# torchmd/torchmd-net

Measured on AMD Instinct MI355X. Metric: molecules/sec (64-atom molecules) TensorNet E+F, higher is better.
Workload: dtype f32; 1 GPU; BASELINE configs[1]: TensorNet F=128 L=2 K=32 rc=5.0, S-mol64 256 molecules x 64 atoms per GPU, energies + forces, random-init weights (seed 0); atoms_per_gpu=16384, pairs_per_gpu=193709, directed_edges_per_gpu=403802, parallelism=molecule-sharded x1, RCCL all-reduce of energies, rank_step=eager: tmdnet_build_graph (pair-count read-back) + tmdnet_energy_forces

## Files before the change

torchmd-net_amd/csrc/tn_api.hip:

```cpp
#include <hip/hip_runtime.h>

#include <algorithm>
#include <cmath>
#include <cstdio>
#include <cstdlib>
#include <cstring>
#include <map>
#include <unordered_map>
#include <string>
#include <vector>

#include "tn_chain.h"
#include "tn_heads.h"
#include "tn_model.h"
#include "tn_tlin9.h"
#include "tn_small.h"
#include "tn_interp.h"
#include "tn_virial.h"

using namespace tn;

static const char* kCatNames[CAT_COUNT] = {"graph", "gemm_edge", "gemm_node", "message", "pair_bwd", "embed_scatter", "elementwise", "edge_table"};

int fail(tmdnet_model* m, int code, const std::string& msg) {
// ... 52 lines not shown
  a.bias[0] = bias;
  a.C = C;
  a.C2 = C2;
  a.rowscale = rs;
  a.rowscale2 = rs2;
  a.lda = lda;
  a.ldw = K;
  a.ldc = ldc;
  a.M = M;
  a.N = N;
  a.K = K;
  a.groups = 1;
  a.m_dev = g_mdev;
  a.m_add = g_madd;
  const double bytes = 4.0 * (2.0 * M * K + (double)N * K + 2.0 * M * N);
  char lab[64];
  std::snprintf(lab, sizeof(lab), "gemm_dual<%d> %dx%dx%d", kind, M, N, K);
  ProfScope ps_(s, CAT_GEMM_EDGE, 4.0 * M * N * K, bytes, lab);
  launch_gemm_dual(a, kind, s);
}

namespace {

void build_specs(tmdnet_model* m) {
  const int F = m->hp.hidden_channels, K = m->hp.num_rbf, L = m->hp.num_layers, Z = m->hp.max_z, H = m->hp.head_hidden;
  auto& s = m->specs;
  const std::string R = "representation_model.", T = R + "tensor_embedding.";
  s.push_back({R + "distance_expansion.means", K, 1});
  s.push_back({R + "distance_expansion.betas", K, 1});
  for (int k = 1; k <= 3; ++k) {
    s.push_back({T + "distance_proj" + std::to_string(k) + ".weight", F, K});
    s.push_back({T + "distance_proj" + std::to_string(k) + ".bias", F, 1});
  }
  s.push_back({T + "emb.weight", Z, F});
  s.push_back({T + "emb2.weight", F, 2 * F});
  s.push_back({T + "emb2.bias", F, 1});
  for (int k = 0; k < 3; ++k) s.push_back({T + "linears_tensor." + std::to_string(k) + ".weight", F, F});
  s.push_back({T + "linears_scalar.0.weight", 2 * F, F});
  s.push_back({T + "linears_scalar.0.bias", 2 * F, 1});
  s.push_back({T + "linears_scalar.1.weight", 3 * F, 2 * F});
  s.push_back({T + "linears_scalar.1.bias", 3 * F, 1});
  s.push_back({T + "init_norm.weight", F, 1});
  s.push_back({T + "init_norm.bias", F, 1});
  for (int l = 0; l < L; ++l) {
    const std::string Lp = R + "layers." + std::to_string(l) + ".";
    const int64_t K1 = m->tn2 ? K + 2 * m->tn2->hp.q_dim : K;
    const int64_t dims[3][2] = {{F, K1}, {2 * F, F}, {3 * F, 2 * F}};
    for (int k = 0; k < 3; ++k) {
      s.push_back({Lp + "linears_scalar." + std::to_string(k) + ".weight", dims[k][0], dims[k][1]});
      s.push_back({Lp + "linears_scalar." + std::to_string(k) + ".bias", dims[k][0], 1});
    }
    for (int k = 0; k < 6; ++k) s.push_back({Lp + "linears_tensor." + std::to_string(k) + ".weight", F, F});
  }
  s.push_back({R + "linear.weight", F, 3 * F});
  s.push_back({R + "linear.bias", F, 1});
  s.push_back({R + "out_norm.weight", 3 * F, 1});
  s.push_back({R + "out_norm.bias", 3 * F, 1});
  const std::string O = "output_model.output_network.layers.";
  s.push_back({O + "0.weight", H, F});
  s.push_back({O + "0.bias", H, 1});
  s.push_back({O + "2.weight", 1, H});
  s.push_back({O + "2.bias", 1, 1});
  s.push_back({"mean", 1, 1});
  s.push_back({"std", 1, 1});
  if (m->hp.has_atomref) s.push_back({"atomref", Z, 1});
  if (m->tn2) {
    const int qd = m->tn2->hp.q_dim;
    for (int l = 0; l <= L; ++l) {
      const std::string Cp = R + (l == 0 ? std::string("charge_predict_0.") : "charge_predicts." + std::to_string(l - 1) + ".");
      s.push_back({Cp + "q_norm.weight", 3 * F, 1});
      s.push_back({Cp + "q_norm.bias", 3 * F, 1});
      s.push_back({Cp + "q_mlp.layers.0.weight", F, 3 * F});
      s.push_back({Cp + "q_mlp.layers.0.bias", F, 1});
      s.push_back({Cp + "q_mlp.layers.2.weight", F, F});
      s.push_back({Cp + "q_mlp.layers.2.bias", F, 1});
      s.push_back({Cp + "q_mlp.layers.4.weight", 2 * qd, F});
      s.push_back({Cp + "q_mlp.layers.4.bias", 2 * qd, 1});
    }
    s.push_back({"output_model.qweights", (int64_t)(L + 1) * qd, 1});
  }
}

}

void tensor_linear(hipStream_t s, const float* A, const float* const W3[3], float* C, int N, int F, int flags, float* pre,
                   const float* gates) {
  GemmArgs a{};
  a.A = A;
  a.C = C;
  a.pre = pre;
  a.aux = gates;
  a.lda = a.ldc = a.ldpre = 9 * (int64_t)F;
  a.ldaux = 3 * (int64_t)F;
  a.ldw = F;
  for (int c = 0; c < 9; ++c) {
    const int t = c == 0 ? 0 : (c < 4 ? 1 : 2);
    a.W[c] = W3[t];
    if (g_cur) {
      auto it = g_cur->sb_of.find(W3[t]);
      if (it != g_cur->sb_of.end()) a.Wsbg[c] = it->second;
    }
    a.bias[c] = nullptr;
    a.a_off[c] = a.c_off[c] = a.pre_off[c] = c * F;
    a.aux_off[c] = t * F;
  }
  a.M = N;
  a.N = F;
  a.K = F;
  a.groups = 9;
  a.flags = flags;
  const double bytes = 4.0 * (9.0 * N * F * (2 + (pre ? 1 : 0)) + (gates ? 3.0 * N * F : 0.0) + 3.0 * F * F);
  char lab[64];
  std::snprintf(lab, sizeof(lab), "tensor_linear 9x%dx%dx%d", N, F, F);
  ProfScope ps_(s, CAT_GEMM_NODE, 2.0 * 9 * N * (double)F * F, bytes, lab);
  launch_gemm(a, s);
}


void remember_graph(tmdnet_model* m, const void* graph_ws, int64_t n_atoms, int64_t n_mol) {
  if (m->graph_rec.size() >= 64 && !m->graph_rec.count(graph_ws)) m->graph_rec.clear();
  m->graph_rec[graph_ws] = tmdnet_model::GraphRecord{m->graph_is_cell, m->graph_cell_multi, m->graph_has_z, m->last_nt, m->lastE, m->graph_no_ghost_pairs, n_atoms, n_mol, m->graph_closed_tiles};
}
void recall_graph(tmdnet_model* m, const void* graph_ws) {
  auto it = m->graph_rec.find(graph_ws);
  if (it == m->graph_rec.end()) return;
  m->graph_is_cell = it->second.is_cell;
  m->graph_cell_multi = it->second.cell_multi;
  m->graph_has_z = it->second.has_z;
  m->last_nt = it->second.nt;
  m->lastE = it->second.lastE;
  m->graph_no_ghost_pairs = it->second.no_ghost_pairs;
  m->graph_closed_tiles = it->second.closed_tiles;
}

bool tlin9_images(const float* const W3[3]) {
  if (!g_cur) return false;
  for (int t = 0; t < 3; ++t)
    if (g_cur->fm_of.find(W3[t]) == g_cur->fm_of.end()) return false;
  return true;
}
void tlin9(hipStream_t s, int pro, int epi, const float* const W3[3], Tl9Args a, double tensors, const char* what) {
  for (int t = 0; t < 3; ++t) a.Wfm[t] = g_cur->fm_of.at(W3[t]);
  char lab[64];
  std::snprintf(lab, sizeof(lab), "tlin9 %s 9x%dx%dx%d", what, a.N, a.F, a.F);
  ProfScope ps_(s, CAT_GEMM_NODE, 2.0 * 9 * a.N * (double)a.F * a.F, 4.0 * (tensors * 9.0 * a.N * a.F + 3.0 * a.F * a.F), lab);
  launch_tlin9(a, pro, epi, s);
}

Graph carve_graph(void* ws, int64_t N, int64_t B, int64_t ecap, size_t* total) {
  Carver c(ws);
  Graph g{};
  const int64_t pcap = ecap / 2 + 1;
  g.small_mols = N <= 96 * (B > 0 ? B : 1) ? 1 : 0;
  g.counts = c.take<int>(8);
  g.mstart = c.take<int>(B);
  g.mend = c.take<int>(B);
  g.nlow = c.take<int>(N);
  g.ntot = c.take<int>(N);
  g.rowptr = c.take<int>(N + 1);
  g.pairptr = c.take<int>(N + 1);
  g.col = c.take<int>(ecap);
  g.epair = c.take<int>(ecap);
  g.esign = c.take<float>(ecap);
  g.pair_i = c.take<int>(pcap);
  g.pair_j = c.take<int>(pcap);
  g.pd = c.take<float>(pcap + 1);
  g.pdelta = c.take<float>(pcap * 3);
  g.prhat = c.take<float>(pcap * 3);
  g.ecap = ecap;
  g.pcap = pcap;
  g.perm = c.take<int>(N);
  g.iota = c.take<int>(N);
  g.cell_key = c.take<int>(N);
  g.cell_key_sorted = c.take<int>(N);
  g.cell_start = c.take<int>(8 * N + 2);
  g.pos_s = c.take<float>(3 * N);
  g.z_s = c.take<int64_t>(N);
  g.boxd = c.take<float>(12);
  g.cgrid = c.take<int>(4);
  g.bat_s = c.take<int>(N);
  g.bat_c = c.take<int64_t>(N);
  g.z_c = c.take<int64_t>(N);
  g.tix = c.take<int>(N);
  g.tz = c.take<int>(64);
  g.sort_tmp_bytes = cell_sort_temp_bytes(N);
  g.sort_tmp = c.take<char>((int64_t)g.sort_tmp_bytes);
  if (total) *total = c.off;
  return g;
}

namespace {
bool cell_applicable(const tmdnet_model* m, int64_t n_atoms, int64_t n_mol, int box_mode) {
  const int* n = m->cell_n;
  if (n_mol < 1 || box_mode == 2 || n_atoms < 1) return false;
  if (n[0] < 0) return true;
  if (n[0] < 1 || n[1] < 1 || n[2] < 1) return false;
  return (int64_t)n[0] * n[1] * n[2] <= 8 * n_atoms;
}
void set_cell(Graph& g, const tmdnet_model* m, bool on, int64_t n_mol = 1) {
  g.use_cell = on ? (n_mol > 1 ? 2 : 1) : 0;
  const bool explicit_grid = m->cell_n[0] > 0;
  g.ncx = explicit_grid ? m->cell_n[0] : 0;
  g.ncy = explicit_grid ? m->cell_n[1] : 0;
  g.ncz = explicit_grid ? m->cell_n[2] : 0;
}

}
int rb_ntp(const tmdnet_model* m, int64_t n_atoms, int64_t n_pairs) {
  if (!m->rb_fwd || m->et || m->train || n_pairs < 0 || n_atoms < m->rb_min_atoms) return 0;
  return embed_rb_ntp(m->last_nt);
}
namespace {

FwdBuffers carve_fwd(void* ws, const tmdnet_hparams& hp, int64_t N, int64_t B, int64_t P, bool bwd, size_t* total, int ntp = 0,
                     int lean = 0) {
  Carver c(ws);
  FwdBuffers b{};
  const int64_t F = hp.hidden_channels, K = hp.num_rbf, L = hp.num_layers, Z = hp.max_z, H = hp.head_hidden;
  const int64_t P1 = P + 1, N9 = N * 9 * F;
  b.phi = c.take<float>((lean & 1) ? 0 : P1 * K);
  b.dphi = c.take<float>((lean & 1) ? 0 : P1 * K);
  b.C = c.take<float>(P1);
  b.dC = c.take<float>(P1);
  b.Q = c.take<float>((lean & 2) ? 0 : P1 * 3 * F);
  b.u0 = c.take<float>(N9);
  b.s0n = c.take<float>(N * F);
  b.ln0 = c.take<float>(N * F);
  b.xh0 = c.take<float>(N * F);
  b.rstd0 = c.take<float>(N);
  b.a1 = c.take<float>(N * 2 * F);
  b.h1 = c.take<float>(N * 2 * F);
  b.a2 = c.take<float>(N * 3 * F);
  b.gates = c.take<float>(N * 3 * F);
  b.UX = c.take<float>(N9);
  for (int l = 0; l <= L; ++l) b.X.push_back(c.take<float>(N9));
  for (int l = 0; l < L; ++l) {
    b.w.push_back(c.take<float>((lean & 4) ? 0 : P1 * 3 * F));
    b.dw.push_back(c.take<float>(bwd && !(lean & 4) ? P1 * 3 * F : 0));
    b.Pn.push_back(c.take<float>(N9));
    b.Mi.push_back(c.take<float>(N9));
    b.D.push_back(c.take<float>(N9));
  }
  b.he1 = c.take<float>((lean & 1) ? 0 : P1 * F);
  b.he2 = c.take<float>((lean & 1) ? 0 : P1 * 2 * F);
  b.te1 = c.take<float>(bwd && !(lean & 1) ? P1 * F : 0);
  b.te2 = c.take<float>(bwd && !(lean & 1) ? P1 * 2 * F : 0);
  b.dQ = c.take<float>(bwd && !(lean & 2) ? P1 * 3 * F : 0);
  b.Xh = c.take<float>(N9);
  b.Ch = c.take<float>(N9);
  b.feat = c.take<float>(N * 3 * F);
  b.lnr = c.take<float>(N * 3 * F);
  b.xhr = c.take<float>(N * 3 * F);
  b.rstdr = c.take<float>(N);
  b.al = c.take<float>(N * F);
  b.x = c.take<float>(N * F);
  b.ao = c.take<float>(N * H);
  b.ea = c.take<float>(N);
  b.kap = c.take<float>(N);
  b.skeys_s = c.take<unsigned>(P1);
  b.svals_s = c.take<int>(P1);
  b.shist = c.take<int>(65536 + 2);
  if (bwd) {
    b.g_ao = c.take<float>(N * H);
    b.g_al = c.take<float>(N * F);
    b.g_ln = c.take<float>(N * 3 * F);
    b.g_feat = c.take<float>(N * 3 * F);
    b.G = c.take<float>(N9);
    b.gD = c.take<float>(N9);
    b.gCh = c.take<float>(N9);
    b.gMi = c.take<float>(N9);
    b.gPn = c.take<float>(N9);
    b.gXl = c.take<float>(N9);
    b.gd = c.take<float>(P1);
    b.gd_slots = c.take<float>(2 * P1 * (int64_t)L * ((F + 31) / 32));
    b.gUX = c.take<float>(N9);
    b.g_a2 = c.take<float>(N * 3 * F);
    b.g_a1 = c.take<float>(N * 2 * F);
    b.g_ln0 = c.take<float>(N * F);
    b.g_s0n = c.take<float>(N * F);
    b.g_u0l = c.take<float>(N9);
    b.gA = c.take<float>(N * 10 * F);
    b.g_rhat = c.take<float>(P1 * 3);
    b.g_delta = c.take<float>(P1 * 3);
  }
  b.mom = c.take<float>(ntp ? embed_rb_moment_elems(N, ntp, (int)K) : 0);
  b.gmom = c.take<float>(ntp && bwd ? embed_rb_gmoment_elems(N, ntp, (int)K) : 0);
  b.ps = c.take<float>(ntp ? P1 * 8 : 0);
  if (total) *total = c.off;
  return b;
}

}

void free_radial_tables(EdgeTables& t) {
  for (float* p : t.tab)
    if (p) (void)hipFree(p);
  t = EdgeTables{};
}

int build_radial_tables(tmdnet_model* m, EdgeTables& out, const std::vector<TableSpec>& specs, const float* means, const float* betas,
                        int K, double lo, double up) {
  free_radial_tables(out);
  const char* env = getenv("TMDNET_EDGE_TABLE");
  if (env && atoi(env) == 0) return TMDNET_OK;
  int Rmax = 0, Nmax = 0;
  for (const TableSpec& sp : specs) {
    const int R = sp.chain.back().N;
    if (R % 4 || R / 4 > 256) return TMDNET_OK;
    Rmax = std::max(Rmax, R);
    for (const TableLayer& l : sp.chain) Nmax = std::max(Nmax, l.N);
  }
  if (specs.empty()) return TMDNET_OK;
  const double tol_value = 5e-7, tol_slope = 2e-6;
  hipStream_t s = nullptr;
  const int ntab = (int)specs.size();
  for (int T = 8192; T <= 65536; T *= 2) {
    const int M = T + 2;
    std::vector<void*> tmp;
    bool alloc_ok = true;
    auto D_ = [&](int64_t n) {
      double* p = nullptr;
      alloc_ok = (hipMalloc(reinterpret_cast<void**>(&p), (size_t)n * sizeof(double)) == hipSuccess) && alloc_ok;
      tmp.push_back(p);
      return p;
    };
    auto F_ = [&](int64_t n) {
      float* p = nullptr;
      alloc_ok = (hipMalloc(reinterpret_cast<void**>(&p), (size_t)n * sizeof(float)) == hipSuccess) && alloc_ok;
      tmp.push_back(p);
      return p;
    };
    double *dist = D_(M), *phi = D_((int64_t)M * K), *dphi = D_((int64_t)M * K), *C = D_(M), *dC = D_(M);
    double* hv_[2] = {D_((int64_t)M * Nmax), D_((int64_t)M * Nmax)};
    double* hs_[2] = {D_((int64_t)M * Nmax), D_((int64_t)M * Nmax)};
    float *ip = F_((int64_t)T * Rmax), *dip = F_((int64_t)T * Rmax);
    std::vector<float*> tab(ntab, nullptr);
    for (int t = 0; t < ntab; ++t)
      alloc_ok = (hipMalloc(reinterpret_cast<void**>(&tab[t]), (size_t)M * 3 * specs[t].chain.back().N * sizeof(float)) == hipSuccess) &&
                 alloc_ok;
// ... 628 lines not shown
    }
    Packer pk;
    std::map<std::string, size_t> off;
    pack_tensornet_params(m, tags, pk, off);
    if (pk.buf.size() != m->packed_elems) return fail(m, TMDNET_ERR_STATE, "device-side parameter update: layout mismatch");
    std::vector<int32_t> tid(pk.buf.size(), -1), ofs(pk.buf.size(), 0);
    for (size_t i = 0; i < pk.buf.size(); ++i) {
      uint32_t tag;
      std::memcpy(&tag, &pk.buf[i], 4);
      if (!tag || (int64_t)tag > base[ns]) continue;
      const int64_t g = (int64_t)tag - 1;
      const size_t t = (size_t)(std::upper_bound(base.begin(), base.end(), g) - base.begin()) - 1;
      tid[i] = (int32_t)t;
      ofs[i] = (int32_t)(g - base[t]);
    }
    HIP_TRY(m, hipMalloc(reinterpret_cast<void**>(&m->upd_tid), tid.size() * sizeof(int32_t)));
    HIP_TRY(m, hipMalloc(reinterpret_cast<void**>(&m->upd_ofs), ofs.size() * sizeof(int32_t)));
    HIP_TRY(m, hipMalloc(reinterpret_cast<void**>(&m->upd_ptrs), ns * sizeof(float*)));
    HIP_TRY(m, hipMemcpy(m->upd_tid, tid.data(), tid.size() * sizeof(int32_t), hipMemcpyHostToDevice));
    HIP_TRY(m, hipMemcpy(m->upd_ofs, ofs.data(), ofs.size() * sizeof(int32_t), hipMemcpyHostToDevice));
    m->upd_ready = true;
  }
  std::vector<const float*> ptrs(ns, nullptr);
  for (int32_t c = 0; c < count; ++c) {
    size_t i = 0;
    for (; i < ns; ++i)
      if (m->specs[i].name == names[c]) break;
    if (i == ns) return fail(m, TMDNET_ERR_INVALID, std::string("unknown parameter: ") + names[c]);
    if (m->specs[i].name == "mean" || m->specs[i].name == "std")
      return fail(m, TMDNET_ERR_INVALID, "mean / std are kernel arguments read on the host: update them through tmdnet_set_param");
    ptrs[i] = dev_ptrs[c];
  }
  HIP_TRY(m, hipMemcpyAsync(m->upd_ptrs, ptrs.data(), ns * sizeof(float*), hipMemcpyHostToDevice, s));
  hipLaunchKernelGGL(k_param_gather, dim3((unsigned)((m->packed_elems + 255) / 256)), dim3(256), 0, s, m->dev, m->upd_tid, m->upd_ofs,
                     m->upd_ptrs, (int64_t)m->packed_elems);
  for (const auto& j : m->image_jobs) {
    if (j.fm) launch_split_weight_fm(m->dev + j.src_off, j.n, j.k, m->dev_sb + j.dst_off, s);
    else launch_split_weight_tiles(m->dev + j.src_off, j.n, j.k, m->dev_sb + j.dst_off, s);
  }
  const int F = m->hp.hidden_channels;
  launch_ztables(m->P.emb, m->P.emb2_waT, m->P.emb2_wbT, m->P.emb2_b, m->hp.max_z, F, const_cast<float*>(m->P.Utab),
                 const_cast<float*>(m->P.Vtab), s);
  m->tabs_pending = true;
  if (m->rb_fwd)
    launch_embed_rb_images(m->P.Wdp, m->P.bdp, F, m->hp.num_rbf, m->rb_img, m->rb_img + embed_rb_image_elems(F, m->hp.num_rbf, false), s);
  HIP_TRY(m, hipGetLastError());
  return TMDNET_OK;
}

int tmdnet_set_option(tmdnet_model* m, const char* name, double value) {
  if (!m || !name) return TMDNET_ERR_INVALID;
  const std::string n(name);
  if (n == "edge_table_min_pairs") {
    m->tab_min_pairs = value < 0 ? 0 : (int64_t)value;
    return TMDNET_OK;
  }
  if (n == "embed_rb_min_atoms") {
    m->rb_min_atoms = value < 0 ? 0 : (int64_t)value;
    return TMDNET_OK;
  }
  if (n == "chain_min_atoms") {
    m->chain_min_atoms = value < 0 ? 0 : (value > 9e18 ? INT64_MAX : (int64_t)value);
    return TMDNET_OK;
  }
  if (n == "chain_mask") {
    m->chain_mask = (int)value & 7;
    return TMDNET_OK;
  }
  if (n == "pair_rows_bf16") {
    if (!m->et) return fail(m, TMDNET_ERR_INVALID, "pair_rows_bf16 applies to the Equivariant Transformer handle only");
    m->pair_bf16 = value == 2.0 ? 2 : (value != 0.0 ? 1 : 0);
    return TMDNET_OK;
  }
  if (n == "recompute_pair_rows") {
    if (m->et || m->tn2) return fail(m, TMDNET_ERR_INVALID, "recompute_pair_rows applies to the TensorNet handle only");
    m->recompute_rows = value != 0.0;
    return TMDNET_OK;
  }
  if (n == "fold_node_adjoint") {
    if (m->et || m->tn2) return fail(m, TMDNET_ERR_INVALID, "fold_node_adjoint applies to the TensorNet handle only");
    m->fold_node_adjoint = value != 0.0;
    return TMDNET_OK;
  }
  return fail(m, TMDNET_ERR_INVALID, "unknown option: " + n);
}

int tmdnet_get_info(const tmdnet_model* m, const char* name, double* value) {
  if (!m || !name || !value) return TMDNET_ERR_INVALID;
  const std::string n(name);
  if (m->tabs_pending && n.rfind("edge_table_", 0) == 0 && n != "edge_table_min_pairs")
    if (const int rc = ensure_radial_tables(const_cast<tmdnet_model*>(m), nullptr)) return rc;
  if (n == "edge_table_T") *value = m->tabs.ok ? m->tabs.T : 0;
  else if (n == "edge_table_err_value") *value = m->tabs.err_value;
  else if (n == "edge_table_err_slope") *value = m->tabs.err_slope;
  else if (n == "edge_table_min_pairs") *value = (double)m->tab_min_pairs;
  else if (n == "pair_rows_bf16") *value = (double)m->pair_bf16;
  else if (n == "embed_rb_min_atoms") *value = (double)m->rb_min_atoms;
  else if (n == "chain_min_atoms") *value = (double)m->chain_min_atoms;
  else if (n == "chain_mask") *value = (double)m->chain_mask;
  else if (n == "chain_last") *value = (double)m->chain_last;
  else if (n == "recompute_pair_rows") *value = m->recompute_rows ? 1.0 : 0.0;
  else if (n == "embed_rb") *value = m->rb_fwd ? 1.0 : 0.0;
  else if (n == "species_last_build") *value = (double)m->last_nt;
  else if (n == "halo_active_first") *value = (double)m->halo_active[0];
  else if (n == "halo_active_rows") *value = (double)m->halo_active[1];
  else if (n == "message_route_last") *value = (double)m->msg_route_last[0];
  else if (n == "message_adjoint_route_last") *value = (double)m->msg_route_last[1];
  else if (n == "fold_node_adjoint") *value = m->fold_node_adjoint ? 1.0 : 0.0;
  else if (n == "message_adjoint_fold_last") *value = (double)m->msg_fold_last;
  else return TMDNET_ERR_INVALID;
  return TMDNET_OK;
}

int tmdnet_set_cell_grid(tmdnet_model* m, int32_t ncx, int32_t ncy, int32_t ncz) {
  if (!m) return TMDNET_ERR_INVALID;
  if (ncx < 0 || ncy < 0 || ncz < 0) ncx = ncy = ncz = -1;
  m->cell_n[0] = ncx;
  m->cell_n[1] = ncy;
  m->cell_n[2] = ncz;
  return TMDNET_OK;
}

int tmdnet_graph_workspace_bytes(const tmdnet_model* m, int64_t n_atoms, int64_t n_mol, size_t* bytes) {
  if (!m || !bytes || n_atoms < 0 || n_mol < 0) return TMDNET_ERR_INVALID;
  const int64_t ecap = (int64_t)m->hp.max_num_neighbors * n_atoms;
  carve_graph(nullptr, n_atoms, n_mol, ecap, bytes);
  return TMDNET_OK;
}

int tmdnet_build_graph(tmdnet_model* m, void* stream, void* graph_ws, size_t graph_ws_bytes, int64_t n_atoms, int64_t n_mol,
                       const float* pos, const int64_t* batch, const int64_t* z, const float* box, int32_t box_mode,
                       int64_t counts_host[8]) {
  if (!m || !graph_ws || !counts_host || n_atoms < 0 || n_mol < 0) return TMDNET_ERR_INVALID;
  if (n_atoms >= (int64_t)1 << 30) return fail(m, TMDNET_ERR_INVALID, "n_atoms too large for 32-bit indices");
  hipStream_t s = reinterpret_cast<hipStream_t>(stream);
  const int64_t ecap = (int64_t)m->hp.max_num_neighbors * n_atoms;
  size_t need = 0;
  Graph g = carve_graph(graph_ws, n_atoms, n_mol, ecap, &need);
  if (need > graph_ws_bytes) return fail(m, TMDNET_ERR_WORKSPACE, "graph workspace too small");
  if (box_mode != 0 && !box) return fail(m, TMDNET_ERR_INVALID, "box_mode != 0 needs a box");
  const bool cell = cell_applicable(m, n_atoms, n_mol, box_mode);
  set_cell(g, m, cell, n_mol);
  if (cell && m->halo_fn && m->atom_w && !m->et && !m->tn2) g.ghost_w = m->atom_w;
  m->graph_no_ghost_pairs = g.ghost_w != nullptr;
  m->graph_is_cell = cell;
  m->graph_cell_multi = cell && n_mol > 1;
  m->graph_has_z = z != nullptr;
  m->g_pos = pos;
  m->g_box = box;
  m->g_box_mode = box_mode;
  CurScope cur_(m);
  {
    ProfScope ps_(s, CAT_GRAPH, 0.0, (double)n_atoms * 20);
    if (cell) {
      launch_fill(reinterpret_cast<float*>(g.counts), 0.f, 8, s);
      launch_cell_phase1(g, pos, batch, box_mode == 1 ? box : nullptr, (int)n_atoms, m->hp.cutoff_lower, m->hp.cutoff_upper, true, s,
                         (int)n_mol);
      launch_scan_counts(g, (int)n_atoms, s);
    } else {
      launch_graph_build_phase1(g, pos, batch, box, box_mode, (int)n_atoms, (int)n_mol, m->hp.cutoff_lower, m->hp.cutoff_upper,
                                true, s);
    }
    if (z) launch_prepare_z(g, z, cell ? g.perm : nullptr, (int)n_atoms, m->hp.max_z, s);
    if (z && m->rb_fwd && n_atoms >= m->rb_min_atoms) launch_type_map(g, (int)n_atoms, m->hp.max_z, s);
  }
  int counts[8] = {0, 0, 0, 0, 0, 0, 0, 0};
  HIP_TRY(m, hipMemcpyAsync(counts, g.counts, sizeof(counts), hipMemcpyDeviceToHost, s));
  HIP_TRY(m, hipStreamSynchronize(s));
  for (int k = 0; k < 8; ++k) counts_host[k] = counts[k];
  m->last_nt = (z && m->rb_fwd && n_atoms >= m->rb_min_atoms) ? counts[6] : 0;
  m->lastE = counts[1];
  m->graph_closed_tiles = !cell && counts[3] == 0 && counts[5] == 0 && counts[7] == 0;
  remember_graph(m, graph_ws, n_atoms, n_mol);
  if (counts[5])
    return fail(m, TMDNET_ERR_INVALID, "batch index out of range: every entry must be in [0, " + std::to_string(n_mol) + ")");
  if (counts[4])
    return fail(m, TMDNET_ERR_INVALID, "atomic number out of range: every z must be in [0, max_z = " + std::to_string(m->hp.max_z) + ")");
  if (counts[2])
    return fail(m, TMDNET_ERR_OVERFLOW, "Found num_pairs > max_num_pairs, please increase max_num_pairs (found " +
                                            std::to_string(counts[1]) + " edges, capacity " + std::to_string(ecap) + ")");
  m->lastE = counts[1];
  {
    ProfScope ps_(s, CAT_GRAPH, 0.0, (double)counts[1] * 12 + (double)counts[0] * 40);
    if (cell) {
      launch_cell_phase2(g, (int)n_atoms, m->hp.cutoff_lower, m->hp.cutoff_upper, true, s);
      launch_nbr_link_wave(g, (int)n_atoms, s);
    } else {
      launch_graph_build_phase2(g, pos, batch, box, box_mode, (int)n_atoms, (int)n_mol, m->hp.cutoff_lower, m->hp.cutoff_upper, true,
                                s);
    }
  }
  HIP_TRY(m, hipGetLastError());
  return TMDNET_OK;
}

int tmdnet_build_graph_static(tmdnet_model* m, void* stream, void* graph_ws, size_t graph_ws_bytes, int64_t n_atoms, int64_t n_mol,
                              const float* pos, const int64_t* batch, const int64_t* z, const float* box, int32_t box_mode) {
  if (!m || !graph_ws || n_atoms < 0 || n_mol < 0) return TMDNET_ERR_INVALID;
  hipStream_t s = reinterpret_cast<hipStream_t>(stream);
  const int64_t ecap = (int64_t)m->hp.max_num_neighbors * n_atoms;
  size_t need = 0;
  Graph g = carve_graph(graph_ws, n_atoms, n_mol, ecap, &need);
  if (need > graph_ws_bytes) return fail(m, TMDNET_ERR_WORKSPACE, "graph workspace too small");
  if (box_mode != 0 && !box) return fail(m, TMDNET_ERR_INVALID, "box_mode != 0 needs a box");
  const bool cell = cell_applicable(m, n_atoms, n_mol, box_mode);
  set_cell(g, m, cell, n_mol);
  m->graph_no_ghost_pairs = false;
  m->graph_is_cell = cell;
  m->graph_cell_multi = cell && n_mol > 1;
  m->graph_has_z = z != nullptr;
  m->g_pos = pos;
  m->g_box = box;
  m->g_box_mode = box_mode;
  CurScope cur_(m);
  {
    ProfScope ps_(s, CAT_GRAPH, 0.0, (double)n_atoms * 20);
    if (cell) {
      launch_fill(reinterpret_cast<float*>(g.counts), 0.f, 8, s);
      launch_cell_phase1(g, pos, batch, box_mode == 1 ? box : nullptr, (int)n_atoms, m->hp.cutoff_lower, m->hp.cutoff_upper, true, s,
                         (int)n_mol);
      launch_scan_counts(g, (int)n_atoms, s);
      launch_cell_phase2(g, (int)n_atoms, m->hp.cutoff_lower, m->hp.cutoff_upper, true, s);
      launch_nbr_link_wave(g, (int)n_atoms, s);
    } else if (graph_small_ok((int)n_atoms)) {
      launch_graph_small(g, pos, batch, box, box_mode, (int)n_atoms, (int)n_mol, m->hp.cutoff_lower, m->hp.cutoff_upper, true, z,
                         m->hp.max_z, s);
    } else {
      launch_graph_build_phase1(g, pos, batch, box, box_mode, (int)n_atoms, (int)n_mol, m->hp.cutoff_lower, m->hp.cutoff_upper,
                                true, s);
      launch_graph_build_phase2(g, pos, batch, box, box_mode, (int)n_atoms, (int)n_mol, m->hp.cutoff_lower, m->hp.cutoff_upper, true,
                                s);
    }
    if (z && (cell || !graph_small_ok((int)n_atoms))) launch_prepare_z(g, z, cell ? g.perm : nullptr, (int)n_atoms, m->hp.max_z, s);
  }
  m->lastE = ecap;
  m->last_nt = 0;
  m->graph_closed_tiles = false;
  remember_graph(m, graph_ws, n_atoms, n_mol);
  HIP_TRY(m, hipGetLastError());
  return TMDNET_OK;
}

int tmdnet_graph_counts(tmdnet_model* m, void* stream, void* graph_ws, int64_t n_atoms, int64_t n_mol, int64_t counts_host[8]) {
  if (!m || !graph_ws || !counts_host) return TMDNET_ERR_INVALID;
  hipStream_t s = reinterpret_cast<hipStream_t>(stream);
  Graph g = carve_graph(graph_ws, n_atoms, n_mol, (int64_t)m->hp.max_num_neighbors * n_atoms, nullptr);
  int counts[8] = {0, 0, 0, 0, 0, 0, 0, 0};
  HIP_TRY(m, hipMemcpyAsync(counts, g.counts, sizeof(counts), hipMemcpyDeviceToHost, s));
  HIP_TRY(m, hipStreamSynchronize(s));
  for (int k = 0; k < 8; ++k) counts_host[k] = counts[k];
  if (counts[5]) return fail(m, TMDNET_ERR_INVALID, "batch index out of range: every entry must be in [0, " + std::to_string(n_mol) + ")");
  if (counts[4])
    return fail(m, TMDNET_ERR_INVALID, "atomic number out of range: every z must be in [0, max_z = " + std::to_string(m->hp.max_z) + ")");
  return counts[2] ? TMDNET_ERR_OVERFLOW : TMDNET_OK;
}

int tmdnet_set_atom_weights(tmdnet_model* m, const float* weights_dev) {
  if (!m) return TMDNET_ERR_INVALID;
  m->atom_w = weights_dev;
  return TMDNET_OK;
}

int tmdnet_set_halo_exchange(tmdnet_model* m, tmdnet_halo_exchange_fn fn, void* user) {
  if (!m) return TMDNET_ERR_INVALID;
  m->halo_fn = fn;
  m->halo_user = fn ? user : nullptr;
  if (fn && !m->halo_rng) HIP_TRY(m, hipMalloc(reinterpret_cast<void**>(&m->halo_rng), 4 * sizeof(int)));
  return TMDNET_OK;
}

int tmdnet_graph_cell_grid(tmdnet_model* m, void* stream, void* graph_ws, int64_t n_atoms, int64_t n_mol, int64_t grid_host[4]) {
  if (!m || !graph_ws || !grid_host) return TMDNET_ERR_INVALID;
  recall_graph(m, graph_ws);
  hipStream_t s = reinterpret_cast<hipStream_t>(stream);
  Graph g = carve_graph(graph_ws, n_atoms, n_mol, (int64_t)m->hp.max_num_neighbors * n_atoms, nullptr);
  int grid[4] = {0, 0, 0, 0};
  if (m->graph_is_cell) {
    HIP_TRY(m, hipMemcpyAsync(grid, g.cgrid, sizeof(grid), hipMemcpyDeviceToHost, s));
    HIP_TRY(m, hipStreamSynchronize(s));
  }
  for (int k = 0; k < 3; ++k) grid_host[k] = grid[k];
  grid_host[3] = m->graph_is_cell ? 1 : 0;
  return TMDNET_OK;
}

int tmdnet_forward_workspace_bytes(const tmdnet_model* m, int64_t n_atoms, int64_t n_mol, int64_t n_pairs, int64_t n_edges,
                                   int32_t want_forces, size_t* bytes) {
  if (!m || !bytes) return TMDNET_ERR_INVALID;
  (void)n_edges;
  if (n_pairs < 0) n_pairs = ((int64_t)m->hp.max_num_neighbors * n_atoms) / 2 + 1;
  if (m->et) return et_forward_workspace_bytes(m, n_atoms, n_mol, n_pairs, want_forces, bytes);
  if (m->tn2) return tn2_forward_workspace_bytes(m, n_atoms, n_mol, n_pairs, n_edges, want_forces, bytes);
  const bool rb_possible = m->rb_fwd && !m->et && !m->train && n_pairs >= 0 && n_atoms >= m->rb_min_atoms;
  carve_fwd(nullptr, m->hp, n_atoms, n_mol, n_pairs, want_forces != 0, bytes, rb_possible ? 8 : 0,
            m->recompute_rows ? (rb_possible && rb_ntp(m, n_atoms, n_pairs) > 0 ? 7 : 5) : 0);
  if (m->head_kind) {
    size_t hb = 0;
    carve_heads(nullptr, n_atoms, n_mol, &hb);
    *bytes = ((*bytes + 255) & ~size_t(255)) + hb;
  }
  return TMDNET_OK;
}

int tmdnet_energy_forces(tmdnet_model* m, void* stream, void* graph_ws, void* ws, size_t ws_bytes, int64_t n_atoms,
                         int64_t n_mol, int64_t n_pairs, const int64_t* z, const int64_t* batch, const float* q,
                         int32_t want_forces, float* energy, float* forces) {
  if (!m || !graph_ws || !ws || !energy) return TMDNET_ERR_INVALID;
  if (!m->finalized) return fail(m, TMDNET_ERR_STATE, "parameters not finalised");
  if (want_forces && !forces) return TMDNET_ERR_INVALID;
  recall_graph(m, graph_ws);
  hipStream_t s = reinterpret_cast<hipStream_t>(stream);
  const tmdnet_hparams& hp = m->hp;
  const int F = hp.hidden_channels, K = hp.num_rbf, L = hp.num_layers, Z = hp.max_z, H = hp.head_hidden;
  const int N = (int)n_atoms, B = (int)n_mol;
  const int64_t ecap = (int64_t)hp.max_num_neighbors * n_atoms;
  Graph g = carve_graph(graph_ws, n_atoms, n_mol, ecap, nullptr);
  if (n_pairs > g.pcap) return fail(m, TMDNET_ERR_INVALID, "n_pairs out of range");
  if (!m->train && (n_pairs >= 0 ? n_pairs : g.pcap) + 1 >= m->tab_min_pairs)
    if (const int rc_tab = ensure_radial_tables(m, s)) return rc_tab;
  if (m->graph_is_cell && m->graph_cell_multi) batch = g.bat_c;
  if (m->atom_w && (m->et || m->tn2 || m->train))
    return fail(m, TMDNET_ERR_INVALID, "atom weights (tmdnet_set_atom_weights) are implemented for TensorNet inference only");
  if (m->halo_fn && (m->et || m->tn2 || m->train || n_pairs < 0))
    return fail(m, TMDNET_ERR_INVALID, "the halo exchange (tmdnet_set_halo_exchange) is implemented for TensorNet inference with the "
                                       "exact pair count (tmdnet_build_graph, not the static mode)");
  if (m->et) {
    if (q) return fail(m, TMDNET_ERR_INVALID, "the Equivariant Transformer takes no total charge (reference torchmd_et.py:188-196)");
    CurScope cur_(m);
    if (m->graph_has_z) {
      z = g.z_c;
    } else if (m->graph_is_cell) {
      set_cell(g, m, true, n_mol);
      launch_permute_z(g, z, (int)n_atoms, s);
      z = g.z_s;
    }
    if (!z) return fail(m, TMDNET_ERR_INVALID, "z is required (here or in tmdnet_build_graph)");
    return et_energy_forces(m, s, g, ws, ws_bytes, n_atoms, n_mol, n_pairs, z, batch, want_forces, energy, forces);
  }
  if (m->tn2) {
    CurScope cur_(m);
    if (m->graph_has_z) {
      z = g.z_c;
    } else if (m->graph_is_cell) {
      set_cell(g, m, true, n_mol);
      launch_permute_z(g, z, (int)n_atoms, s);
      z = g.z_s;
    }
    if (!z) return fail(m, TMDNET_ERR_INVALID, "z is required (here or in tmdnet_build_graph)");
    if (m->graph_is_cell) set_cell(g, m, true, n_mol);
    return tn2_energy_forces(m, s, g, ws, ws_bytes, n_atoms, n_mol, n_pairs, z, batch, q, want_forces, energy, forces);
  }
  const int P = n_pairs >= 0 ? (int)n_pairs : (int)g.pcap, P1 = P + 1;
  size_t need = 0;
  const int ntp = rb_ntp(m, n_atoms, n_pairs);
  const bool recompute = m->recompute_rows;
  FwdBuffers b = carve_fwd(ws, hp, n_atoms, n_mol, P, want_forces != 0, &need, ntp, recompute ? (ntp ? 7 : 5) : 0);
  HeadBuffers hbuf{};
  if (m->head_kind) {
    if (m->train) return fail(m, TMDNET_ERR_INVALID, "the property heads (tmdnet_set_output_head) have no parameter-gradient pass");
    if (m->atom_w || m->halo_fn)
      return fail(m, TMDNET_ERR_INVALID, "the property heads (tmdnet_set_output_head) take neither atom weights nor the halo exchange");
    if (!m->g_pos) return fail(m, TMDNET_ERR_STATE, "the property heads read the positions of tmdnet_build_graph: build the graph first");
    need = (need + 255) & ~size_t(255);
    size_t hb = 0;
    hbuf = carve_heads(static_cast<char*>(ws) + need, n_atoms, n_mol, &hb);
    need += hb;
  }
  if (need > ws_bytes) return fail(m, TMDNET_ERR_WORKSPACE, "forward workspace too small: need " + std::to_string(need));
  const DevParams& W = m->P;
  const int o3 = hp.group_o3;

  CurScope cur_(m);
  const int* perm = nullptr;
  if (m->graph_is_cell) {
    set_cell(g, m, true, n_mol);
    if (!m->graph_has_z) {
      launch_permute_z(g, z, N, s);
      z = g.z_s;
    }
    perm = g.perm;
  }
  if (m->graph_has_z) z = g.z_c;
  if (!z) return fail(m, TMDNET_ERR_INVALID, "z is required (here or in tmdnet_build_graph)");
  HeadArgs heads{};
  if (m->head_kind) {
    heads.kind = m->head_kind; heads.N = N; heads.B = B; heads.pos = m->g_pos; heads.perm = perm; heads.z = z; heads.batch = batch;
    heads.mass = W.mass; heads.n_mass = TMDNET_MASS_TABLE_SIZE; heads.q = b.ea; heads.mean = W.mean; heads.y = energy;
  }
  const int64_t* batch_k = batch;
  if (q) {
    launch_kappa(q, batch, N, B, b.kap, s);
    q = b.kap;
    batch_k = nullptr;
  }
  const double E_ = (double)m->lastE, Nd = N, Pd = P, Fd = F;
  const double nodeB = Nd * 9 * Fd * 4;
  const double wB = (Pd + 1) * 12 * Fd, idxB = E_ * 12;
  auto EDGE = [&](int add) { g_gemm_cat = CAT_GEMM_EDGE; g_mdev = g.counts; g_madd = add; };
  auto NODE = [&]() { g_gemm_cat = CAT_GEMM_NODE; g_mdev = nullptr; g_madd = 0; };

  TrainCtx* const tc = m->train;
  const bool use_tab = !tc && m->tabs.ok && (int64_t)P1 >= m->tab_min_pairs && (int)m->tabs.tab.size() == 1 + L && L + 1 <= 8;
  hipStream_t es = s;
  const RadialParams rbp{W.means, W.betas, K, hp.cutoff_lower, hp.cutoff_upper};
  const double momB = (double)embed_rb_moment_elems(N, ntp ? ntp : 4, K) * 4;
  const bool run_fwd = !tc || tc->phase != 2, run_bwd = !tc || tc->phase != 1;
  if (recompute && (!use_tab || (want_forces && !(message_adjoint_gd_ok(N, F) && !getenv("TMDNET_SEPARATE_PAIR_GD")))))
    return fail(m, TMDNET_ERR_STATE, "option recompute_pair_rows needs the radial tables (verified, not switched off) and the merged "
                                     "distance gradient; TensorNet inference only");
  PairRowTable rts[8];
  for (int l = 0; l < L && recompute; ++l) {
    const float h_ = (hp.cutoff_upper - hp.cutoff_lower) / (float)m->tabs.T;
    rts[l] = PairRowTable{m->tabs.tab[1 + l], g.pd, g.counts, hp.cutoff_lower, h_, 1.0f / h_, m->tabs.T};
  }
  const bool use_mid = !small_fused_ok(N, F, H, L);
  auto HALO = [&](int stage, float* rows, int row_floats) -> int {
    if (!m->halo_fn) return 0;
    return m->halo_fn(m->halo_user, stage, rows, (int64_t)N, (int64_t)row_floats, perm, (void*)s);
  };
#define HALO_TRY(stage, rows, row_floats) \
  do { if (HALO(stage, rows, row_floats)) return fail(m, TMDNET_ERR_STATE, "halo exchange callback failed at stage " + std::to_string(stage)); } while (0)
  int a0 = 0, Na = N;
  if (m->halo_fn && m->halo_rng && m->atom_w && m->graph_is_cell && want_forces && !tc && (int64_t)N > 256 * (int64_t)B) {
    int h[4] = {0, 0, 0, 0};
    launch_owned_range(m->atom_w, perm, N, m->halo_rng, s);
    HIP_TRY(m, hipMemcpyAsync(h, m->halo_rng, sizeof(h), hipMemcpyDeviceToHost, s));
    HIP_TRY(m, hipStreamSynchronize(s));
    const bool images = tlin9_images(W.Ue) && tlin9_images(W.UeT) && L > 0 && tlin9_images(W.layer[0].V) && tlin9_images(W.layer[0].VT);
    if (h[2] > 0 && h[2] < N && h[1] - h[0] + 1 == h[2] && images && tlin9_ok(h[2], F, true)) {
      a0 = h[0];
      Na = h[2];
    }
  }
  const bool rng = Na != N;
  const bool t9 = !tc && tlin9_ok(Na, F, rng) && tlin9_images(W.Ue) && tlin9_images(W.UeT) && (L == 0 || tlin9_images(W.layer[0].V));
  const bool t9r = !tc && L > 0 && tlin9_ok(Na, F, rng) && tlin9_images(W.UeT) && tlin9_images(W.layer[0].VT);
  m->halo_active[0] = a0;
  m->halo_active[1] = Na;
  const int64_t o1_ = a0, oF = (int64_t)a0 * F, o2F = 2 * oF, o3F = 3 * oF, o9F = 9 * oF, oH = (int64_t)a0 * H;
  const float* const q_a = q ? q + o1_ : nullptr;
  const int64_t* const batch_a = batch_k ? batch_k + o1_ : nullptr;
  const bool fused_small = !tc && !ntp && !recompute && !m->halo_fn && !m->head_kind && (small_fused_ok(N, F, H, L) || mid_fused_ok(N, F, H, L)) &&
                           (!want_forces || (message_adjoint_gd_ok(N, F) && !getenv("TMDNET_SEPARATE_PAIR_GD")));
  auto fm_image = [&](const float* w) -> const uint16_t* {
    auto it = m->fm_of.find(w);
    return it == m->fm_of.end() ? nullptr : it->second;
  };
  const bool chain_any = !tc && !m->head_kind && !m->halo_fn && Na == N && !fused_small && (int64_t)N >= m->chain_min_atoms;
  const bool chain_ro = chain_any && (m->chain_mask & 1) && want_forces && run_fwd && run_bwd && chain_readout_shape_ok(F, H) &&
                        fm_image(W.Lin) && fm_image(W.LinT) && fm_image(W.O1) && fm_image(W.O1T);
  const bool chain_gate = chain_any && want_forces && run_fwd && run_bwd && chain_gate_shape_ok(F);
  const bool chain_gf = chain_gate && (m->chain_mask & 2) && fm_image(W.L1) && fm_image(W.L2);
  const bool chain_gb = chain_gate && (m->chain_mask & 4) && fm_image(W.L2T) && fm_image(W.L1T);
  m->chain_last = (chain_ro ? 1 : 0) | (chain_gf ? 2 : 0) | (chain_gb ? 4 : 0);
  m->msg_fold_last = 0;
  if (run_fwd) {
    if (use_tab) {
      const float* tabs[8];
      float* outs[8];
      float* douts[8];
      int nt_ = 0;
      if (!ntp) {
        tabs[nt_] = m->tabs.tab[0];
        outs[nt_] = b.Q;
        douts[nt_++] = want_forces ? b.dQ : nullptr;
      }
      for (int l = 0; l < L && !recompute; ++l) {
        tabs[nt_] = m->tabs.tab[1 + l];
        outs[nt_] = b.w[l];
        douts[nt_++] = want_forces ? b.dw[l] : nullptr;
      }
      const double rowB = 12.0 * Fd;
      if (nt_ > 0)
        KR(CAT_EDGE_TABLE, (Pd + 1) * (rowB * nt_ * (want_forces ? 2 : 1) + 24) + (double)(m->tabs.T + 2) * 2 * rowB * nt_,
           (launch_pair_buckets(g, P, hp.cutoff_lower, hp.cutoff_upper, m->tabs.T, b.C, b.dC, b.shist, b.skeys_s, b.svals_s, s),
            launch_edge_interp(g, P, hp.cutoff_lower, hp.cutoff_upper, m->tabs.T, 3 * F, nt_, tabs, outs, douts, b.skeys_s, b.svals_s, s, b.C,
                               b.dC)));
    } else {
      RadialParams rp{W.means, W.betas, K, hp.cutoff_lower, hp.cutoff_upper};
      KR(CAT_ELEMENTWISE, Pd * (2 * K + 3) * 4, launch_radial(g, P, rp, b.phi, b.dphi, b.C, b.dC, s));
      es = (m->side && L > 0 && P >= 16384 && !tc) ? m->side : s;
      if (es != s) {
        HIP_TRY(m, hipEventRecord(m->ev_fork, s));
        HIP_TRY(m, hipStreamWaitEvent(es, m->ev_fork, 0));
      }
      for (int l = 0; l < L; ++l) {
        const LayerP& q_ = W.layer[l];
        EDGE(1);
        if (tc) {
          gemm(es, b.phi, K, q_.M1, K, q_.b1, tc->he1[l], F, P1, F, K, GEMM_ACT_SILU, tc->pre1[l], F);
          gemm(es, tc->he1[l], F, q_.M2, F, q_.b2, tc->he2[l], 2 * F, P1, 2 * F, F, GEMM_ACT_SILU, tc->pre2[l], 2 * F);
          gemm(es, tc->he2[l], 2 * F, q_.M3, 2 * F, q_.b3, b.w[l], 3 * F, P1, 3 * F, 2 * F, GEMM_ACT_SILU | GEMM_ROWSCALE, tc->pre3[l], 3 * F,
               nullptr, 0, b.C);
        } else if (want_forces) {
          gemm_dual(es, 1, b.phi, b.dphi, K, q_.M1, q_.b1, b.he1, b.te1, F, P1, F, K, nullptr, nullptr, q_.M_sb[0]);
          gemm_dual(es, 1, b.he1, b.te1, F, q_.M2, q_.b2, b.he2, b.te2, 2 * F, P1, 2 * F, F, nullptr, nullptr, q_.M_sb[1]);
          gemm_dual(es, 2, b.he2, b.te2, 2 * F, q_.M3, q_.b3, b.w[l], b.dw[l], 3 * F, P1, 3 * F, 2 * F, b.C, b.dC, q_.M_sb[2]);
        } else {
          gemm(es, b.phi, K, q_.M1, K, q_.b1, b.he1, F, P1, F, K, GEMM_ACT_SILU);
          gemm(es, b.he1, F, q_.M2, F, q_.b2, b.he2, 2 * F, P1, 2 * F, F, GEMM_ACT_SILU);
          gemm(es, b.he2, 2 * F, q_.M3, 2 * F, q_.b3, b.w[l], 3 * F, P1, 3 * F, 2 * F, GEMM_ACT_SILU | GEMM_ROWSCALE, nullptr, 0, nullptr, 0,
               b.C);
        }
        if (es != s) HIP_TRY(m, hipEventRecord(m->ev_join[l], es));
      }
      EDGE(1);
      if (ntp) {
      } else if (tc) gemm(s, b.phi, K, W.Wdp, K, W.bdp, b.Q, 3 * F, P1, 3 * F, K);
      else if (want_forces) gemm_dual(s, 0, b.phi, b.dphi, K, W.Wdp, W.bdp, b.Q, b.dQ, 3 * F, P1, 3 * F, K, nullptr, nullptr, W.Wdp_sb);
      else gemm(s, b.phi, K, W.Wdp, K, W.bdp, b.Q, 3 * F, P1, 3 * F, K);
    }
    if (fused_small) {
      SmallEmbedArgs ea{};
      ea.g = g; ea.N = N; ea.F = F; ea.L = L; ea.z = z;
      ea.Utab = W.Utab; ea.Vtab = W.Vtab; ea.Q = b.Q; ea.C = b.C;
      ea.ln0_w = W.ln0_w; ea.ln0_b = W.ln0_b; ea.L1T = W.L1T; ea.bL1 = W.bL1; ea.L2T = W.L2T; ea.bL2 = W.bL2;
      for (int t = 0; t < 3; ++t) {
        ea.UeT[t] = W.UeT[t];
        ea.V0T[t] = W.layer[0].VT[t];
      }
      ea.u0 = b.u0; ea.xh0 = b.xh0; ea.rstd0 = b.rstd0; ea.a1 = b.a1; ea.a2 = b.a2; ea.gates = b.gates; ea.UX = b.UX; ea.X0 = b.X[0];
      ea.Pn0 = b.Pn[0];
      KR(CAT_SCATTER, Pd * 12 * Fd + E_ * 12 + 5 * nodeB, (use_mid ? launch_mid_embed(ea, s) : launch_small_embed(ea, s)));
      for (int l = 0; l < L; ++l) {
        const LayerP& q_ = W.layer[l];
        const bool last = l + 1 == L;
        SmallLayerArgs la{};
        la.g = g; la.N = N; la.F = F; la.H = H; la.o3 = o3; la.want_forces = want_forces ? 1 : 0; la.z = z; la.kap = q; la.atom_w = m->atom_w; la.perm = perm;
        la.w = b.w[l]; la.Pn = b.Pn[l]; la.X = b.X[l]; la.Mi = b.Mi[l]; la.D = b.D[l]; la.Xn = b.X[l + 1];
        for (int t = 0; t < 3; ++t) {
          la.VbT[t] = q_.VT[3 + t];
          la.Vb[t] = q_.V[3 + t];
          if (!last) la.VnT[t] = W.layer[l + 1].VT[t];
        }
        if (!last) la.Pn_next = b.Pn[l + 1];
        la.lnr_w = W.lnr_w; la.lnr_b = W.lnr_b; la.LinT = W.LinT; la.bLin = W.bLin; la.O1T = W.O1T; la.bO1 = W.bO1; la.O2 = W.O2;
        la.bO2 = W.bO2; la.atomref = W.atomref; la.Lin = W.Lin; la.O1 = W.O1; la.std_ = W.std;
        la.xhr = b.xhr; la.rstdr = b.rstdr; la.al = b.al; la.x = b.x; la.ea = b.ea;
        if (want_forces) { la.G = b.G; la.gMi = b.gMi; la.gPn = b.gPn; }
        KR(CAT_MESSAGE, wB + idxB + 6 * nodeB, (use_mid ? launch_mid_layer(la, last, s) : launch_small_layer(la, last, s)));
      }
      if (!want_forces) KR(CAT_ELEMENTWISE, Nd * 4, launch_mol_sum(g, b.ea, batch, N, B, W.mean, energy, s));
    } else {
    if (ntp) {
      KR(CAT_SCATTER, E_ * 12 + Pd * 48 + momB,
         (launch_pair_scalars(g, P, hp.cutoff_lower, hp.cutoff_upper, b.ps, s), launch_embed_moments(g, N, rbp, ntp, b.ps, b.mom, s)));
      KR(CAT_SCATTER, momB + Nd * 10 * Fd * 4, launch_embed_combine(g, N, F, K, ntp, z, W.Utab, W.Vtab, m->rb_fwd, b.mom, b.u0, b.s0n, s));
    } else {
      KR(CAT_SCATTER, Pd * 12 * Fd + E_ * 12 + Nd * 10 * Fd * 4,
         launch_embed_scatter(g, N, F, z, W.Utab, W.Vtab, b.Q, b.C, b.u0, b.s0n, s));
    }
    NODE();
    if (chain_gf) {
      ChainGateFwdArgs ca{};
      ca.s0n = b.s0n; ca.xh0 = b.xh0; ca.rstd0 = b.rstd0; ca.a1 = b.a1; ca.a2 = b.a2; ca.gates = b.gates;
      ca.ln_w = W.ln0_w; ca.ln_b = W.ln0_b; ca.bL1 = W.bL1; ca.bL2 = W.bL2; ca.L1_fm = fm_image(W.L1); ca.L2_fm = fm_image(W.L2); ca.N = N;
      char lab[64];
      std::snprintf(lab, sizeof(lab), "chain gate_fwd %dx%d", N, F);
      ProfScope ps_(s, CAT_GEMM_NODE, 2.0 * Nd * 8.0 * Fd * Fd, Nd * 10 * Fd * 4 + Nd * 4 + 4.0 * 8.0 * Fd * Fd, lab);
      if (launch_chain_gate_fwd(ca, F, s)) return fail(m, TMDNET_ERR_HIP, "launch_chain_gate_fwd");
    } else {
    KR(CAT_ELEMENTWISE, Nd * Fd * 12,
       launch_layernorm_fwd(b.s0n + oF, W.ln0_w, W.ln0_b, Na, F, b.ln0 + oF, b.xh0 + oF, b.rstd0 + o1_, s));
    gemm(s, b.ln0 + oF, F, W.L1, F, W.bL1, b.h1 + o2F, 2 * F, Na, 2 * F, F, GEMM_ACT_SILU, b.a1 + o2F, 2 * F);
    gemm(s, b.h1 + o2F, 2 * F, W.L2, 2 * F, W.bL2, b.gates + o3F, 3 * F, Na, 3 * F, 2 * F, GEMM_ACT_SILU, b.a2 + o3F, 3 * F);
    }
    if (t9) {
      Tl9Args ta{};
      ta.A = b.u0 + o9F; ta.C = b.X[0] + o9F; ta.o1 = b.UX + o9F; ta.e3 = b.gates + o3F; ta.N = Na; ta.F = F;
      tlin9(s, TL9_PRO_PLAIN, TL9_EPI_MULGATE, W.Ue, ta, 3.0 + 1.0 / 3.0, "gate");
    } else
      tensor_linear(s, b.u0, W.Ue, b.X[0], N, F, GEMM_MUL_AUX, b.UX, b.gates);
    for (int l = 0; l < L; ++l) {
      const LayerP& q_ = W.layer[l];
      if (es != s) HIP_TRY(m, hipStreamWaitEvent(s, m->ev_join[l], 0));
      float* const Xh_l = tc ? tc->Xh[l] : b.Xh;
      float* const Ch_l = tc ? tc->Ch[l] : b.Ch;
      float* const Xh_n = tc && l + 1 < L ? tc->Xh[l + 1] : b.Xh;
      if (t9) {
        Tl9Args ta{};
        ta.A = b.X[l] + o9F; ta.C = b.Pn[l] + o9F; ta.N = Na; ta.F = F;
        tlin9(s, TL9_PRO_NORM, TL9_EPI_PLAIN, q_.V, ta, 2.0, "norm");
        HALO_TRY(l, b.Pn[l], 9 * F);
        m->msg_route_last[0] = message_route(g, N, F, recompute, a0, rng ? Na : -1);
        KR(CAT_MESSAGE, wB + idxB + nodeB * (1.0 + 2.0 * Na / Nd),
           launch_message(g, N, F, b.w[l], b.Pn[l], q, batch_k, o3, b.Mi[l], Ch_l, s, recompute ? &rts[l] : nullptr, a0, rng ? Na : -1));
        Tl9Args tb{};
        tb.A = Ch_l + o9F; tb.C = b.D[l] + o9F; tb.e0 = b.X[l] + o9F; tb.o1 = b.X[l + 1] + o9F; tb.o2 = b.feat + o3F;
        tb.want_feat = l + 1 == L; tb.kap = q_a;
        tb.N = Na; tb.F = F;
        tlin9(s, TL9_PRO_PLAIN, TL9_EPI_UPDATE, q_.V + 3, tb, 4.0 + (l + 1 == L ? 1.0 / 3.0 : 0.0), "update");
        continue;
      }
      if (l == 0) KR(CAT_ELEMENTWISE, 2 * nodeB, launch_norm_x(b.X[l], Xh_l, N, F, s));
      tensor_linear(s, Xh_l, q_.V, b.Pn[l], N, F);
      HALO_TRY(l, b.Pn[l], 9 * F);
      m->msg_route_last[0] = message_route(g, N, F, recompute);
      KR(CAT_MESSAGE, wB + idxB + 3 * nodeB, launch_message(g, N, F, b.w[l], b.Pn[l], q, batch_k, o3, b.Mi[l], Ch_l, s, recompute ? &rts[l] : nullptr));
      tensor_linear(s, Ch_l, q_.V + 3, b.D[l], N, F);
      KR(CAT_ELEMENTWISE, 4 * nodeB, launch_layer_update(Xh_l, b.D[l], q, batch_k, N, F, b.X[l + 1], l + 1 < L ? 1 : 2,
                                                         l + 1 < L ? Xh_n : b.feat, s));
    }
    if (L == 0) KR(CAT_ELEMENTWISE, nodeB + Nd * 3 * Fd * 4, launch_readout_feat(b.X[L] + o9F, Na, F, b.feat + o3F, s));
    if (chain_ro) {
      ChainReadoutArgs ca{};
      ca.feat = b.feat; ca.X = b.X[L]; ca.G = b.G; ca.x = b.x; ca.ea = b.ea;
      ca.lnr_w = W.lnr_w; ca.lnr_b = W.lnr_b; ca.bLin = W.bLin; ca.bO1 = W.bO1; ca.O2 = W.O2; ca.bO2 = W.bO2;
      ca.Lin_fm = fm_image(W.Lin); ca.LinT_fm = fm_image(W.LinT); ca.O1_fm = fm_image(W.O1); ca.O1T_fm = fm_image(W.O1T);
      ca.atomref = W.atomref; ca.z = z; ca.aw = m->atom_w; ca.perm = perm; ca.std_ = W.std; ca.N = N;
      {
        char lab[64];
        std::snprintf(lab, sizeof(lab), "chain readout_fb %dx%dx%d", N, F, H);
        ProfScope ps_(s, CAT_GEMM_NODE, 2.0 * Nd * (2.0 * 3 * Fd * Fd + 2.0 * Fd * H),
                      2 * nodeB + Nd * 4 * Fd * 4 + Nd * 4 + 4.0 * (2.0 * 3 * Fd * Fd + 2.0 * Fd * H), lab);
        if (launch_chain_readout_fb(ca, F, H, s)) return fail(m, TMDNET_ERR_HIP, "launch_chain_readout_fb");
      }
      KR(CAT_ELEMENTWISE, Nd * 4, launch_mol_sum(g, b.ea, batch, N, B, W.mean, energy, s));
    } else {
    KR(CAT_ELEMENTWISE, Nd * 3 * Fd * 12,
       launch_layernorm_fwd(b.feat + o3F, W.lnr_w, W.lnr_b, Na, 3 * F, b.lnr + o3F, b.xhr + o3F, b.rstdr + o1_, s));
    NODE();
    gemm(s, b.lnr + o3F, 3 * F, W.Lin, 3 * F, W.bLin, b.x + oF, F, Na, F, 3 * F, GEMM_ACT_SILU, b.al + oF, F);
    gemm(s, b.x + oF, F, W.O1, F, W.bO1, b.ao + oH, H, Na, H, F);
    if (m->head_kind) {
      KR(CAT_ELEMENTWISE, Nd * H * 4,
         launch_head_energy(b.ao, W.O2, W.bO2, N, H, W.std, nullptr, z, b.ea, s, want_forces ? b.g_ao : nullptr));
      heads.state = want_forces ? hbuf.state : nullptr;
      KR(CAT_ELEMENTWISE, Nd * 32, launch_heads_reduce(g, heads, hbuf, s));
    } else if ((int64_t)N <= 256 * (int64_t)B) {
      KR(CAT_ELEMENTWISE, Nd * H * 4, launch_head_mol_sum(g, b.ao, W.O2, W.bO2, N, B, H, W.std, W.atomref, z, batch, W.mean, energy, s,
                                                          want_forces ? b.g_ao : nullptr, m->atom_w, perm));
    } else {
      if (Na != N) launch_fill(b.ea, 0.f, N, s);
      KR(CAT_ELEMENTWISE, Nd * H * 4,
         launch_head_energy(b.ao + oH, W.O2, W.bO2, Na, H, W.std, W.atomref, z + o1_, b.ea + o1_, s, want_forces ? b.g_ao + oH : nullptr,
                            perm ? m->atom_w : (m->atom_w ? m->atom_w + o1_ : nullptr), perm ? perm + o1_ : nullptr));
      KR(CAT_ELEMENTWISE, Nd * 4, launch_mol_sum(g, b.ea, batch, N, B, W.mean, energy, s));
    }
    }
    }
  }
  if (m->head_kind && want_forces && run_bwd)
    KR(CAT_ELEMENTWISE, Nd * (8 * H + 40), launch_heads_seed(heads, H, b.g_ao, hbuf.direct, s));

  if (want_forces && run_bwd && fused_small) {
    const int gd_nw = message_adjoint_gd_waves(g, N, F, recompute);
    const int64_t gd_stride = 2 * (int64_t)P1;
    for (int l = L - 1; l >= 0; --l) {
      const LayerP& q_ = W.layer[l];
      float* const gMi_in = ((L - 1 - l) & 1) ? b.gCh : b.gMi;
      float* const gMi_out = ((L - 1 - l) & 1) ? b.gMi : b.gCh;
      SmallRevArgs ra{};
      ra.g = g; ra.N = N; ra.F = F; ra.B = B; ra.o3 = o3; ra.first = l == 0; ra.kap = q;
      ra.w = b.w[l]; ra.dw = b.dw[l]; ra.gMi_in = gMi_in; ra.Pn = b.Pn[l]; ra.X = b.X[l];
      ra.gPn = b.gPn; ra.G = b.G; ra.slots = b.gd_slots + (int64_t)l * gd_nw * gd_stride; ra.slot_stride = gd_stride;
      for (int t = 0; t < 3; ++t) {
        ra.Va[t] = q_.V[t];
        ra.Ue[t] = W.Ue[t];
        if (l > 0) ra.Vb_prev[t] = W.layer[l - 1].V[3 + t];
      }
      if (l > 0) { ra.D_prev = b.D[l - 1]; ra.Pn_prev = b.Pn[l - 1]; ra.Mi_prev = b.Mi[l - 1]; ra.gMi_out = gMi_out; }
      ra.UX = b.UX; ra.gates = b.gates; ra.a2 = b.a2; ra.a1 = b.a1; ra.L2 = W.L2; ra.L1 = W.L1; ra.xh0 = b.xh0; ra.rstd0 = b.rstd0;
      ra.ln0_w = W.ln0_w; ra.u0 = b.u0; ra.gA = b.gA;
      if (l == L - 1) { ra.ea = b.ea; ra.batch = batch; ra.mean = W.mean; ra.energy = energy; }
      KR(CAT_MESSAGE, 2 * wB + idxB + 6 * nodeB + 8 * (Pd + 1) * gd_nw, (use_mid ? launch_mid_rev(ra, s) : launch_small_rev(ra, s)));
    }
    KR(CAT_PAIR, Pd * (24 * Fd + 24) + Nd * 10 * Fd * 4,
       launch_embed_pair_gd(g, P, F, z, W.Utab, W.Vtab, b.Q, b.dQ, b.C, b.dC, b.gA, b.gd, b.g_rhat, s, b.g_delta, b.gd_slots, L * gd_nw,
                            gd_stride));
    if (m->virial_out)
      KR(CAT_ELEMENTWISE, E_ * 8 + Nd * 84 + Pd * 12, launch_force_virial(g, N, B, b.g_delta, perm, batch, forces, m->virial_out, m->virial_ws, s));
    else
      KR(CAT_ELEMENTWISE, E_ * 8 + Nd * 12, launch_force_gather(g, N, b.g_delta, perm, forces, s));
  } else if (want_forces && run_bwd) {
    NODE();
    const RowMap rH = rows_plain(H), rF = rows_plain(F), r2F = rows_plain(2 * F), r3F = rows_plain(3 * F), rK = rows_plain(K);
    const RowMap rc_[3] = {rows_comp(F, 1), rows_comp(F, 3), rows_comp(F, 5)};
    const int c0_[3] = {0, 1, 4}, nc_[3] = {1, 3, 5};
    auto tensor_linear_grad = [&](const float* gOut, const float* In, const std::string& key) {
      for (int t = 0; t < 3; ++t)
        launch_tn_gemm(s, gOut + (int64_t)c0_[t] * F, rc_[t], In + (int64_t)c0_[t] * F, rc_[t], nullptr, nullptr, N * nc_[t], F, F,
                       tc->at(key + std::to_string(t)), false, tc->part);
    };
    if (tc) {
      launch_train_seed(b.ao, tc->gE, batch, N, H, W.std, b.g_ao, tc->head, s);
      launch_colsum(s, tc->head, rows_plain(H + 1), nullptr, rH, nullptr, nullptr, N, H, tc->at("O2"), false, tc->part);
      launch_colsum(s, tc->head + H, rows_plain(H + 1), nullptr, rH, nullptr, nullptr, N, 1, tc->at("bO2"), false, tc->part);
      launch_tn_gemm(s, b.g_ao, rH, b.x, rF, nullptr, nullptr, N, H, F, tc->at("O1"), false, tc->part);
      launch_colsum(s, b.g_ao, rH, nullptr, rH, nullptr, nullptr, N, H, tc->at("bO1"), false, tc->part);
    }
    if (!chain_ro) gemm(s, b.g_ao + oH, H, W.O1T, H, nullptr, b.g_al + oF, F, Na, F, H, GEMM_MUL_DSILU_AUX, nullptr, 0, b.al + oF, F);
    if (!chain_ro) gemm(s, b.g_al + oF, F, W.LinT, F, nullptr, b.g_ln + o3F, 3 * F, Na, 3 * F, F);
    if (tc) {
      launch_tn_gemm(s, b.g_al, rF, b.lnr, r3F, nullptr, nullptr, N, F, 3 * F, tc->at("Lin"), false, tc->part);
      launch_colsum(s, b.g_al, rF, nullptr, rF, nullptr, nullptr, N, F, tc->at("bLin"), false, tc->part);
      launch_colsum(s, b.g_ln, r3F, b.xhr, r3F, nullptr, nullptr, N, 3 * F, tc->at("lnr_w"), false, tc->part);
      launch_colsum(s, b.g_ln, r3F, nullptr, r3F, nullptr, nullptr, N, 3 * F, tc->at("lnr_b"), false, tc->part);
    }
    if (chain_ro) {
// ... 287 lines not shown
  float* e_out = energy ? energy : tc.forces;
  const int rc = tmdnet_energy_forces(m, stream, graph_ws, ws, ws_bytes, n_atoms, n_mol, n_pairs, z, batch, q, 1, e_out, tc.forces);
  m->train = nullptr;
  return rc;
}

int tmdnet_neighbor_workspace_bytes(int64_t n_atoms, int64_t n_mol, int64_t max_num_pairs, size_t* bytes) {
  if (!bytes || n_atoms < 0 || n_mol < 0 || max_num_pairs < 0) return TMDNET_ERR_INVALID;
  const int64_t ecap = 2 * max_num_pairs + n_atoms + 2;
  carve_graph(nullptr, n_atoms, n_mol, ecap, bytes);
  return TMDNET_OK;
}

int tmdnet_neighbor_pairs(void* stream, void* ws, size_t ws_bytes, int64_t n_atoms, int64_t n_mol, const float* pos,
                          const int64_t* batch, const float* box, int32_t box_mode, float cutoff_lower, float cutoff_upper,
                          int64_t max_num_pairs, int32_t loop, int32_t include_transpose, int32_t strategy, int64_t* neighbors,
                          float* deltas, float* distances, int32_t* num_pairs) {
  if (!ws || !neighbors || !deltas || !distances || !num_pairs) return TMDNET_ERR_INVALID;
  hipStream_t s = reinterpret_cast<hipStream_t>(stream);
  const int64_t ecap = 2 * max_num_pairs + n_atoms + 2;
  size_t need = 0;
  Graph g = carve_graph(ws, n_atoms, n_mol, ecap, &need);
  if (need > ws_bytes) return TMDNET_ERR_WORKSPACE;
  const bool cell = strategy == 1 && box_mode != 2 && n_atoms > 0;
  if (cell) {
    g.use_cell = n_mol > 1 ? 2 : 1;
    g.ncx = g.ncy = g.ncz = 0;
    launch_fill(reinterpret_cast<float*>(g.counts), 0.f, 8, s);
    launch_cell_phase1(g, pos, batch, box_mode == 1 ? box : nullptr, (int)n_atoms, cutoff_lower, cutoff_upper, true, s);
    launch_scan_counts(g, (int)n_atoms, s);
    launch_cell_phase2(g, (int)n_atoms, cutoff_lower, cutoff_upper, true, s);
    launch_nbr_link_wave(g, (int)n_atoms, s);
  } else {
    launch_graph_build_phase1(g, pos, batch, box, box_mode, (int)n_atoms, (int)n_mol, cutoff_lower, cutoff_upper, true, s);
    launch_graph_build_phase2(g, pos, batch, box, box_mode, (int)n_atoms, (int)n_mol, cutoff_lower, cutoff_upper, true, s);
  }
  launch_export_pairs(g, (int)n_atoms, include_transpose != 0, loop != 0, max_num_pairs, cell ? g.perm : nullptr, neighbors, deltas,
                      distances, num_pairs, s);
  return hipGetLastError() == hipSuccess ? TMDNET_OK : TMDNET_ERR_HIP;
}

int tmdnet_neighbor_grad(void* stream, const int64_t* neighbors, const float* deltas, const float* distances,
                         const float* grad_deltas, const float* grad_distances, int64_t num_entries, int64_t n_atoms,
                         float* grad_positions) {
  if (!neighbors || !deltas || !distances || !grad_positions || num_entries < 0 || n_atoms < 0) return TMDNET_ERR_INVALID;
  launch_neighbor_grad(neighbors, deltas, distances, grad_deltas, grad_distances, num_entries, (int)n_atoms, grad_positions,
                       reinterpret_cast<hipStream_t>(stream));
  return hipGetLastError() == hipSuccess ? TMDNET_OK : TMDNET_ERR_HIP;
}

int tmdnet_profile_begin(tmdnet_model* m, uint32_t category_mask) {
  if (!m) return TMDNET_ERR_INVALID;
  m->prof.on = true;
  m->prof.mask = category_mask;
  m->prof.recs.clear();
  m->prof.used = 0;
  return TMDNET_OK;
}

int tmdnet_profile_end(tmdnet_model* m, void* stream, double* ms, double* flops, double* bytes, int64_t* launches) {
  if (!m || !ms || !flops || !bytes || !launches) return TMDNET_ERR_INVALID;
  HIP_TRY(m, hipStreamSynchronize(reinterpret_cast<hipStream_t>(stream)));
  for (int c = 0; c < CAT_COUNT; ++c) ms[c] = flops[c] = bytes[c] = 0.0, launches[c] = 0;
  for (const ProfRec& r : m->prof.recs) {
    float t = 0.f;
    HIP_TRY(m, hipEventElapsedTime(&t, r.a, r.b));
    ms[r.cat] += t;
    flops[r.cat] += r.flops;
    bytes[r.cat] += r.bytes;
    launches[r.cat] += 1;
  }
  m->prof.on = false;
  m->prof.recs.clear();
  m->prof.used = 0;
  return TMDNET_OK;
}

int tmdnet_profile_end_records(tmdnet_model* m, void* stream, int64_t cap, int32_t* cat, double* ms, double* flops, double* bytes,
                               char* labels, int64_t* n_out) {
  if (!m || !cat || !ms || !flops || !bytes || !n_out || cap < 0) return TMDNET_ERR_INVALID;
  HIP_TRY(m, hipStreamSynchronize(reinterpret_cast<hipStream_t>(stream)));
  int64_t n = 0;
  for (const ProfRec& r : m->prof.recs) {
    if (n >= cap) break;
    float t = 0.f;
    HIP_TRY(m, hipEventElapsedTime(&t, r.a, r.b));
    cat[n] = r.cat;
    ms[n] = t;
    flops[n] = r.flops;
    bytes[n] = r.bytes;
    if (labels) std::memcpy(labels + 64 * n, r.label, 64);
    ++n;
  }
  *n_out = (int64_t)m->prof.recs.size();
  m->prof.on = false;
  m->prof.recs.clear();
  m->prof.used = 0;
  return TMDNET_OK;
}

int tmdnet_profile_num_categories(void) { return CAT_COUNT; }
const char* tmdnet_profile_category_name(int idx) { return idx >= 0 && idx < CAT_COUNT ? kCatNames[idx] : nullptr; }

int tmdnet_debug_tensor(tmdnet_model* m, void* stream, const char* name, float* out, int64_t numel) {
  if (m && m->et) return et_debug_tensor(m, reinterpret_cast<hipStream_t>(stream), name, out, numel);
  if (!m || !name || !out || !m->has_last) return TMDNET_ERR_STATE;
  hipStream_t s = reinterpret_cast<hipStream_t>(stream);
  const int64_t F = m->hp.hidden_channels, K = m->hp.num_rbf, N = m->lastN, P1 = m->lastP + 1;
  const FwdBuffers& b = m->last;
  const float* src = nullptr;
  int64_t n = 0;
  std::string nm(name);
  if (nm == "X_embed") { src = b.X[0]; n = N * 9 * F; }
  else if (nm.rfind("X_layer", 0) == 0) {
    int l = std::atoi(nm.c_str() + 7);
    if (l < 0 || l >= m->hp.num_layers) return TMDNET_ERR_INVALID;
    src = b.X[l + 1]; n = N * 9 * F;
  }
  else if (nm.rfind("Pn", 0) == 0 || nm.rfind("Mi", 0) == 0 || (nm.rfind("D", 0) == 0 && nm.size() == 2)) {
    const int l = std::atoi(nm.c_str() + (nm[0] == 'D' ? 1 : 2));
    if (l < 0 || l >= m->hp.num_layers) return TMDNET_ERR_INVALID;
    src = nm[0] == 'P' ? b.Pn[l] : (nm[0] == 'M' ? b.Mi[l] : b.D[l]);
    n = N * 9 * F;
  }
  else if (nm == "x") { src = b.x; n = N * F; }
  else if (nm == "phi") { src = b.phi; n = P1 * K; }
  else if (nm == "Q") { src = b.Q; n = P1 * 3 * F; }
  else if (nm == "u0") { src = b.u0; n = N * 9 * F; }
  else if (nm == "G_embed") { src = b.G; n = N * 9 * F; }
  else if (nm == "charges" && m->tn2) { src = m->tn2_last_chg; n = N * (int64_t)(m->hp.num_layers + 1) * m->tn2->hp.q_dim; }
  else return fail(m, TMDNET_ERR_INVALID, "unknown debug tensor");
  if (!src || numel != n) return fail(m, TMDNET_ERR_INVALID, "debug tensor size mismatch: expected " + std::to_string(n));
  HIP_TRY(m, hipMemcpyAsync(out, src, sizeof(float) * n, hipMemcpyDeviceToDevice, s));
  return TMDNET_OK;
}

int tmdnet_debug_graph(tmdnet_model* m, void* stream, const void* graph_ws, int64_t n_atoms, int64_t n_mol, const char* name,
                       void* out, int64_t bytes) {
  if (!m || !graph_ws || !name || !out || n_atoms < 0 || n_mol < 0) return TMDNET_ERR_INVALID;
  const auto it = m->graph_rec.find(graph_ws);
  if (it == m->graph_rec.end()) return fail(m, TMDNET_ERR_STATE, "no graph was built on this workspace");
  if (it->second.n_atoms != n_atoms || it->second.n_mol != n_mol)
    return fail(m, TMDNET_ERR_INVALID, "debug graph: the last build on this workspace had other n_atoms / n_mol");
  const int64_t N = n_atoms, B = n_mol;
  const Graph g = carve_graph(const_cast<void*>(graph_ws), N, B, (int64_t)m->hp.max_num_neighbors * N, nullptr);
  const struct { const char* name; const void* ptr; int64_t bytes; } arrays[] = {
      {"counts", g.counts, 8 * 4},          {"mstart", g.mstart, B * 4},          {"mend", g.mend, B * 4},
      {"nlow", g.nlow, N * 4},              {"ntot", g.ntot, N * 4},              {"rowptr", g.rowptr, (N + 1) * 4},
      {"pairptr", g.pairptr, (N + 1) * 4},  {"col", g.col, g.ecap * 4},           {"epair", g.epair, g.ecap * 4},
      {"esign", g.esign, g.ecap * 4},       {"pair_i", g.pair_i, g.pcap * 4},     {"pair_j", g.pair_j, g.pcap * 4},
      {"pd", g.pd, (g.pcap + 1) * 4},       {"pdelta", g.pdelta, g.pcap * 12},    {"prhat", g.prhat, g.pcap * 12},
      {"perm", g.perm, N * 4},              {"z_c", g.z_c, N * 8},                {"bat_c", g.bat_c, N * 8},
      {"cgrid", g.cgrid, 4 * 4},            {"boxd", g.boxd, 12 * 4},             {"cell_key_sorted", g.cell_key_sorted, N * 4},
      {"cell_start", g.cell_start, (8 * N + 2) * 4}};
  for (const auto& a : arrays) {
    if (std::strcmp(a.name, name)) continue;
    if (bytes != a.bytes) return fail(m, TMDNET_ERR_INVALID, "debug graph size mismatch: expected " + std::to_string(a.bytes) + " bytes");
    if (a.bytes > 0) HIP_TRY(m, hipMemcpyAsync(out, a.ptr, (size_t)a.bytes, hipMemcpyDeviceToDevice, reinterpret_cast<hipStream_t>(stream)));
    return TMDNET_OK;
  }
  return fail(m, TMDNET_ERR_INVALID, std::string("unknown graph array: ") + name);
}

int tmdnet_debug_gemm_dual(void* stream, const float* A, const float* A2, const float* W, const float* bias, float* C, float* C2,
                           int64_t M, int64_t N, int64_t K, int32_t kind, const float* rs, const float* rs2, const uint16_t* Wsb) {
  g_mdev = nullptr;
  gemm_dual(reinterpret_cast<hipStream_t>(stream), kind, A, A2, K, W, bias, C, C2, N, (int)M, (int)N, (int)K, rs, rs2, Wsb);
  return hipGetLastError() == hipSuccess ? TMDNET_OK : TMDNET_ERR_HIP;
}

int64_t tmdnet_debug_split_weight(const float* W_host, int64_t N, int64_t K, uint16_t* out_host) {
  if (out_host) split_weight_tiles(W_host, N, K, out_host);
  return (int64_t)split_weight_elems(N, K);
}

int tmdnet_debug_gemm(void* stream, const float* A, const float* W, const float* bias, float* C, int64_t M, int64_t N,
                      int64_t K, int32_t silu_, const uint16_t* Wsb) {
  g_mdev = nullptr;
  g_wsb_debug = Wsb;
  gemm(reinterpret_cast<hipStream_t>(stream), A, K, W, K, bias, C, N, (int)M, (int)N, (int)K, silu_ ? GEMM_ACT_SILU : 0);
  g_wsb_debug = nullptr;
  return hipGetLastError() == hipSuccess ? TMDNET_OK : TMDNET_ERR_HIP;
}

static_assert(TMDNET_GEMM_MAX_GROUPS == GEMM_MAX_GROUPS, "group count of the diagnostic struct");
static_assert(TMDNET_GEMM_ACT_SILU == GEMM_ACT_SILU && TMDNET_GEMM_MUL_AUX == GEMM_MUL_AUX && TMDNET_GEMM_MUL_DSILU_AUX == GEMM_MUL_DSILU_AUX &&
                  TMDNET_GEMM_ACCUM == GEMM_ACCUM && TMDNET_GEMM_ROWSCALE == GEMM_ROWSCALE, "flag values of the diagnostic struct");
static_assert(TMDNET_GEMM_ROUTE_NONE == GEMM_ROUTE_NONE && TMDNET_GEMM_ROUTE_SKINNY4 == GEMM_ROUTE_SKINNY4 &&
                  TMDNET_GEMM_ROUTE_SKINNY8 == GEMM_ROUTE_SKINNY8 && TMDNET_GEMM_ROUTE_TILES_128X128 == GEMM_ROUTE_TILES_128x128 &&
                  TMDNET_GEMM_ROUTE_TILES_128X64 == GEMM_ROUTE_TILES_128x64 && TMDNET_GEMM_ROUTE_TILES_128X32 == GEMM_ROUTE_TILES_128x32 &&
                  TMDNET_GEMM_ROUTE_SB1_128 == GEMM_ROUTE_SB1_128 && TMDNET_GEMM_ROUTE_SB1_64 == GEMM_ROUTE_SB1_64, "route values of the header");

int tmdnet_debug_gemm_ex(void* stream, const tmdnet_gemm_ex_args* x, int32_t* route_out) {
  if (!x) return TMDNET_ERR_INVALID;
  const int all_flags = GEMM_ACT_SILU | GEMM_MUL_AUX | GEMM_MUL_DSILU_AUX | GEMM_ACCUM | GEMM_ROWSCALE;
  if (x->N < 1 || x->K < 1 || x->M < 0 || x->groups < 1 || x->groups > GEMM_MAX_GROUPS || (x->flags & ~all_flags)) return TMDNET_ERR_INVALID;
  if (!x->A || !x->C || x->lda < x->K || x->ldw < x->K || x->ldc < x->N) return TMDNET_ERR_INVALID;
  if ((x->flags & GEMM_ROWSCALE) && !x->rowscale) return TMDNET_ERR_INVALID;
  if ((x->flags & (GEMM_MUL_AUX | GEMM_MUL_DSILU_AUX)) && !x->aux) return TMDNET_ERR_INVALID;
  if (x->pre && x->ldpre < x->N) return TMDNET_ERR_INVALID;
  if (x->aux && x->ldaux < x->N) return TMDNET_ERR_INVALID;
  GemmArgs a{};
  for (int g = 0; g < x->groups; ++g) {
    if (!x->W[g] || x->a_off[g] < 0 || x->c_off[g] < 0 || (x->pre && x->pre_off[g] < 0) || (x->aux && x->aux_off[g] < 0)) return TMDNET_ERR_INVALID;
    a.W[g] = x->W[g];
    a.bias[g] = x->bias[g];
    a.Wsbg[g] = x->Wsbg[g];
    a.a_off[g] = x->a_off[g];
    a.c_off[g] = x->c_off[g];
    a.pre_off[g] = x->pre_off[g];
    a.aux_off[g] = x->aux_off[g];
  }
  a.A = x->A;
  a.C = x->C;
  a.pre = x->pre;
  a.aux = x->aux;
  a.rowscale = x->rowscale;
  a.lda = x->lda;
  a.ldw = x->ldw;
  a.ldc = x->ldc;
  a.ldpre = x->ldpre;
  a.ldaux = x->ldaux;
  a.M = x->M;
  a.N = x->N;
  a.K = x->K;
  a.groups = x->groups;
  a.flags = x->flags;
  a.m_dev = x->m_dev;
  a.m_add = x->m_add;
  if (route_out) *route_out = gemm_route(a);
  return launch_gemm(a, reinterpret_cast<hipStream_t>(stream)) == (int)hipSuccess ? TMDNET_OK : TMDNET_ERR_HIP;
}

int tmdnet_debug_tlin9(void* stream, int32_t pro, int32_t epi, int64_t N, int64_t F, const float* A, const float* A2, float* C,
                       const float* e0, const float* e1, const float* e2, const float* e3, const float* e4, float* o1, float* o2,
                       const float* kap, int32_t want_feat, const float* W_I, const float* W_A, const float* W_S,
                       uint16_t* scratch, int64_t* scratch_elems) {
  if (!scratch_elems || F < 128 || F % 128 || F > (1 << 14)) return TMDNET_ERR_INVALID;
  const int64_t one = (int64_t)split_weight_fm_elems(F, F);
  if (!scratch) {
    *scratch_elems = 3 * one;
    return TMDNET_OK;
  }
  if (*scratch_elems < 3 * one || N < 1 || N > (1 << 26)) return TMDNET_ERR_INVALID;
  auto bad = [](const void* p, uintptr_t al) { return !p || (reinterpret_cast<uintptr_t>(p) & (al - 1)); };
  bool inv = bad(A, 8) || bad(W_I, 16) || bad(W_A, 16) || bad(W_S, 16) || bad(scratch, 16) || (kap && bad(kap, 4));
  if (pro == TL9_PRO_PLAIN) {
    switch (epi) {
      case TL9_EPI_PLAIN: inv = inv || bad(C, 8); break;
      case TL9_EPI_MULGATE: inv = inv || bad(C, 8) || bad(e3, 8) || bad(o1, 8); break;
      case TL9_EPI_UPDATE: inv = inv || bad(C, 8) || bad(e0, 8) || bad(o1, 8) || (want_feat && bad(o2, 8)); break;
      case TL9_EPI_NORMBWD: inv = inv || bad(C, 8) || bad(e0, 8) || bad(e1, 8); break;
      case TL9_EPI_NORMBWD_GATE:
        inv = inv || bad(C, 8) || bad(e0, 8) || bad(e1, 8) || bad(e2, 8) || bad(e3, 8) || bad(e4, 8) || bad(o1, 8);
        break;
      case TL9_EPI_EMBBWD: inv = inv || bad(e0, 8) || bad(e1, 8) || bad(o1, 8); break;
      default: inv = true;
    }
  } else if (pro == TL9_PRO_NORM && epi == TL9_EPI_PLAIN) {
    inv = inv || bad(C, 8);
  } else if (pro == TL9_PRO_UPDBWD && epi == TL9_EPI_PLAIN) {
    inv = inv || bad(C, 8) || bad(A2, 8);
  } else {
    inv = true;
  }
  if (inv) return TMDNET_ERR_INVALID;
  hipStream_t s = reinterpret_cast<hipStream_t>(stream);
  const float* W3[3] = {W_I, W_A, W_S};
  Tl9Args a{};
  for (int t = 0; t < 3; ++t) {
    launch_split_weight_fm(W3[t], F, F, scratch + t * one, s);
    a.Wfm[t] = scratch + t * one;
  }
  a.A = A;
  a.A2 = A2;
  a.C = C;
  a.e0 = e0;
  a.e1 = e1;
  a.e2 = e2;
  a.e3 = e3;
  a.e4 = e4;
  a.o1 = o1;
  a.o2 = o2;
  a.kap = kap;
  a.N = (int)N;
  a.F = (int)F;
  a.want_feat = want_feat ? 1 : 0;
  if (hipGetLastError() != hipSuccess) return TMDNET_ERR_HIP;
  return launch_tlin9(a, pro, epi, s) == (int)hipSuccess ? TMDNET_OK : TMDNET_ERR_HIP;
}

static_assert(TMDNET_MSG_FWD_ROW == MSG_FWD_ROW && TMDNET_MSG_FWD_SPLIT == MSG_FWD_SPLIT && TMDNET_MSG_FWD_TILE == MSG_FWD_TILE &&
                  TMDNET_MSG_ADJ_ROW == MSG_ADJ_ROW && TMDNET_MSG_ADJ_SPLIT == MSG_ADJ_SPLIT && TMDNET_MSG_GD_ROW == MSG_GD_ROW &&
                  TMDNET_MSG_GD_SPLIT == MSG_GD_SPLIT && TMDNET_MSG_GD_TILE == MSG_GD_TILE && TMDNET_MSG_DUAL == MSG_DUAL &&
                  TMDNET_MSG_DUAL_ACC == MSG_DUAL_ACC && TMDNET_MSG_DUAL_SPLIT3 == MSG_DUAL_SPLIT3 && TMDNET_MSG_AUTO == MSG_NONE,
              "route values of the header");

int tmdnet_debug_message(void* stream, const tmdnet_message_args* x, int32_t* route_out, int32_t* slot_arrays_out) {
  if (!x) return TMDNET_ERR_INVALID;
  const int N = x->N, F = x->F;
  if (N < 1 || F < 1 || x->P < 0 || x->op < TMDNET_MSG_OP_FWD || x->op > TMDNET_MSG_OP_DUAL) return TMDNET_ERR_INVALID;
  if (!x->rowptr || !x->col || !x->epair || !x->esign || !x->counts) return TMDNET_ERR_INVALID;
  Graph g{};
  g.rowptr = const_cast<int*>(x->rowptr);
  g.col = const_cast<int*>(x->col);
  g.epair = const_cast<int*>(x->epair);
  g.esign = const_cast<float*>(x->esign);
// ... 105 lines not shown
```

torchmd-net_amd/csrc/tn_cell.hip:

```cpp
#include <cstring>

#include <hip/hip_runtime.h>

#include "tn_common.h"
#include "tn_kernels.h"

namespace tn {

static inline int cdivc(int64_t a, int64_t b) { return (int)((a + b - 1) / b); }

size_t cell_sort_temp_bytes(int64_t n) { return (size_t)(8 * (n > 0 ? n : 1) + 2) * sizeof(int); }

__global__ void k_cell_assign(const float* __restrict__ pos, const float* __restrict__ box, int N, const int* __restrict__ cgrid,
                              int* __restrict__ key, int* __restrict__ hist) {
  int i = blockIdx.x * blockDim.x + threadIdx.x;
  if (i >= N) return;
  const int ncx = cgrid[0], ncy = cgrid[1], ncz = cgrid[2];
  const float x = pos[i * 3], y = pos[i * 3 + 1], zc = pos[i * 3 + 2];
  float fz = zc / box[8];
  float fy = (y - fz * box[7]) / box[4];
  float fx = (x - fy * box[3] - fz * box[6]) / box[0];
  fx -= floorf(fx);
  fy -= floorf(fy);
  fz -= floorf(fz);
  int cx = min((int)(fx * ncx), ncx - 1), cy = min((int)(fy * ncy), ncy - 1), cz = min((int)(fz * ncz), ncz - 1);
  const int c = (cx * ncy + cy) * ncz + cz;
  key[i] = c;
  atomicAdd(&hist[c], 1);
}

__global__ void k_fill_cells(const int* __restrict__ cgrid, int* __restrict__ hist) {
  const int64_t c = (int64_t)blockIdx.x * blockDim.x + threadIdx.x;
  if (c <= cgrid[3]) hist[c] = 0;
}
__global__ __launch_bounds__(1024) void k_cell_scan(const int* __restrict__ cgrid, int* __restrict__ hist_cursor,
                                                   int* __restrict__ cell_start, int N) {
  __shared__ int wsum[16];
  __shared__ int carry_s;
  const int ncells = cgrid[3];
  const int tid = threadIdx.x, lane = tid & 63, wave = tid >> 6;
  if (tid == 0) carry_s = 0;
  __syncthreads();
  for (int base = 0; base < ncells; base += 1024) {
    const int c = base + tid;
    const int v = c < ncells ? hist_cursor[c] : 0;
    int x = v;
#pragma unroll
    for (int off = 1; off < 64; off <<= 1) {
      const int y = __shfl_up(x, off, 64);
      if (lane >= off) x += y;
    }
    if (lane == 63) wsum[wave] = x;
    __syncthreads();
    int woff = 0;
    for (int w = 0; w < wave; ++w) woff += wsum[w];
    const int excl = carry_s + woff + x - v;
    if (c < ncells) {
      cell_start[c] = excl;
      hist_cursor[c] = excl;
    }
    __syncthreads();
    if (tid == 1023) carry_s = excl + v;
    __syncthreads();
  }
  if (tid == 0) cell_start[ncells] = N;
}
__global__ void k_cell_place(const int* __restrict__ key, int N, int* __restrict__ cursor, int* __restrict__ slot_atom) {
  int i = blockIdx.x * blockDim.x + threadIdx.x;
  if (i >= N) return;
  slot_atom[atomicAdd(&cursor[key[i]], 1)] = i;
}
__global__ __launch_bounds__(256) void k_cell_rank(const int* __restrict__ cgrid, const int* __restrict__ cell_start,
                                                   const int* __restrict__ slot_atom, int* __restrict__ perm,
                                                   int* __restrict__ key_sorted) {
  const int ncells = cgrid[3];
  const int lane = threadIdx.x & 63;
  for (int c = blockIdx.x * 4 + (threadIdx.x >> 6); c < ncells; c += gridDim.x * 4) {
    const int s0 = cell_start[c], n = cell_start[c + 1] - s0;
    for (int a0 = 0; a0 < n; a0 += 64) {
      const int a = a0 + lane;
      const int mine = a < n ? slot_atom[s0 + a] : 0x7fffffff;
      int rank = 0;
      for (int b0 = 0; b0 < n; b0 += 64) {
        const int other = b0 + lane < n ? slot_atom[s0 + b0 + lane] : 0x7fffffff;
        const int m = n - b0 < 64 ? n - b0 : 64;
        for (int k = 0; k < m; ++k) rank += __shfl(other, k, 64) < mine ? 1 : 0;
      }
      if (a < n) {
        perm[s0 + rank] = mine;
        key_sorted[s0 + rank] = c;
      }
    }
  }
}

__global__ void k_permute_pos(const float* __restrict__ pos, const int64_t* __restrict__ batch, const int* __restrict__ perm, int N,
                              int B, float* __restrict__ pos_s, int* __restrict__ bat_s, int64_t* __restrict__ bat_c,
                              int* __restrict__ counts) {
  int i = blockIdx.x * blockDim.x + threadIdx.x;
  if (i >= N) return;
  const int o = perm[i];
  pos_s[i * 3] = pos[o * 3];
  pos_s[i * 3 + 1] = pos[o * 3 + 1];
  pos_s[i * 3 + 2] = pos[o * 3 + 2];
  if (batch) {
    int64_t b = batch[o];
    if (B > 0 && (b < 0 || b >= B)) {
      counts[5] = 1;
      b = b < 0 ? 0 : B - 1;
    }
    bat_s[i] = (int)b;
    bat_c[i] = b;
    if (i == 0) counts[3] = 1;
  }
}
__global__ void k_permute_z(const int64_t* __restrict__ z, const int* __restrict__ perm, int N, int64_t* __restrict__ z_s) {
  int i = blockIdx.x * blockDim.x + threadIdx.x;
  if (i < N) z_s[i] = z[perm[i]];
}
void launch_permute_z(const Graph& g, const int64_t* z, int N, hipStream_t s) {
  hipLaunchKernelGGL(k_permute_z, dim3(cdivc(N, 256)), dim3(256), 0, s, z, g.perm, N, g.z_s);
}
__global__ void k_prepare_z(const int64_t* __restrict__ z, const int* __restrict__ perm, int N, int max_z, int64_t* __restrict__ z_c,
                            int* __restrict__ counts) {
  int i = blockIdx.x * blockDim.x + threadIdx.x;
  if (i >= N) return;
  int64_t v = z[perm ? perm[i] : i];
  if (v < 0 || v >= max_z) {
    counts[4] = 1;
    v = v < 0 ? 0 : max_z - 1;
  }
  z_c[i] = v;
}
void launch_prepare_z(const Graph& g, const int64_t* z, const int* perm, int N, int max_z, hipStream_t s) {
  if (N <= 0) return;
  hipLaunchKernelGGL(k_prepare_z, dim3(cdivc(N, 256)), dim3(256), 0, s, z, perm, N, max_z, g.z_c, g.counts);
}

__device__ __forceinline__ float cell_d2(const float* __restrict__ pos, int hi, int lo, const float* __restrict__ box, float& dx,
                                         float& dy, float& dz) {
  return pair_geometry(pos, hi, lo, box, dx, dy, dz);
}

template <bool FILL>
__global__ __launch_bounds__(256) void k_nbr_cell(Graph g, int N, float lo2, float up2, int loop) {
  const int i = blockIdx.x * 4 + (threadIdx.x >> 6);
  const int lane = threadIdx.x & 63;
  if (i >= N) return;
  if (FILL && g.counts[2]) return;
  const float* __restrict__ pos = g.pos_s;
  const float* __restrict__ box = g.boxd;
  const int* __restrict__ bat = g.use_cell > 1 ? g.bat_s : nullptr;
  const int ncx = g.cgrid[0], ncy = g.cgrid[1], ncz = g.cgrid[2];
  const int ci = g.cell_key_sorted[i];
  const int bi = bat ? bat[i] : 0;
  const float* __restrict__ gw = g.ghost_w;
  const bool ghost_i = gw && gw[g.perm[i]] == 0.f;
  const int cz = ci % ncz, cy = (ci / ncz) % ncy, cx = ci / (ncz * ncy);
  int nid = 0x7fffffff;
  if (lane < 27) {
    const int dx = lane / 9 - 1, dy = (lane / 3) % 3 - 1, dz = lane % 3 - 1;
    const int x = (cx + dx + ncx) % ncx, y = (cy + dy + ncy) % ncy, zc = (cz + dz + ncz) % ncz;
    nid = (x * ncy + y) * ncz + zc;
  }
#pragma unroll
  for (int k = 2; k <= 32; k <<= 1)
#pragma unroll
    for (int j = k >> 1; j > 0; j >>= 1) {
      const int other = __shfl_xor(nid, j, 64);
      const bool up = ((lane & k) == 0);
      const bool lower = ((lane & j) == 0);
      nid = (lower == up) ? min(nid, other) : max(nid, other);
    }
  const int P = FILL ? g.counts[0] : 0;
  int e = FILL ? g.rowptr[i] : 0, p = FILL ? g.pairptr[i] : 0;
  int nl = 0, nt = 0;
  const unsigned long long lt = lane == 0 ? 0ull : (~0ull >> (64 - lane));
  int t = 0;
  while (t < 27) {
    int c0 = __shfl(nid, t, 64), c1 = c0;
    ++t;
    while (t < 27) {
      const int cn = __shfl(nid, t, 64);
      if (cn != c1 && cn != c1 + 1) break;
      c1 = cn;
      ++t;
    }
    const int j0 = g.cell_start[c0], j1 = g.cell_start[c1 + 1];
    for (int base = j0; base < j1; base += 64) {
      const int j = base + lane;
      bool hit = false, self = false;
      float dx = 0.f, dy = 0.f, dz = 0.f, d2 = 0.f;
      if (j < j1) {
        if (j == i) {
          hit = loop != 0;
          self = true;
        } else if ((!bat || bat[j] == bi) && !(ghost_i && gw[g.perm[j]] == 0.f)) {
          d2 = (j < i) ? cell_d2(pos, i, j, box, dx, dy, dz) : cell_d2(pos, j, i, box, dx, dy, dz);
          hit = d2 < up2 && d2 >= lo2;
        }
      }
      const unsigned long long mall = __ballot(hit);
      const unsigned long long mlow = __ballot(hit && j < i);
      if (FILL) {
        if (hit) {
          const int ee = e + __popcll(mall & lt);
          g.col[ee] = j;
          if (self) {
            g.epair[ee] = P;
            g.esign[ee] = 0.f;
          } else if (j < i) {
            const int pp = p + __popcll(mlow & lt);
            const float d = sqrtf(d2);
            const float inv = d > 0.f ? 1.0f / d : 0.f;
            g.pair_i[pp] = i;
            g.pair_j[pp] = j;
            g.pd[pp] = d;
            g.pdelta[pp * 3 + 0] = dx; g.pdelta[pp * 3 + 1] = dy; g.pdelta[pp * 3 + 2] = dz;
            g.prhat[pp * 3 + 0] = dx * inv; g.prhat[pp * 3 + 1] = dy * inv; g.prhat[pp * 3 + 2] = dz * inv;
            g.epair[ee] = pp;
            g.esign[ee] = 1.f;
          } else {
            g.epair[ee] = -1;
            g.esign[ee] = -1.f;
          }
        }
        e += __popcll(mall);
        p += __popcll(mlow);
      } else {
        nt += __popcll(mall);
        nl += __popcll(mlow);
      }
    }
  }
  if (!FILL && lane == 0) {
    g.nlow[i] = nl;
    g.ntot[i] = nt;
  }
  if (FILL && i == 0 && lane == 0) g.pd[P] = 0.f;
}

__global__ __launch_bounds__(1024) void k_cell_setup(const float* __restrict__ box, const float* __restrict__ pos, int N, float rc,
                                                    int ncap, int ex, int ey, int ez, float* __restrict__ boxd,
                                                    int* __restrict__ cgrid, int* mstart, int* mend, int one_mol) {
  __shared__ float red[6][16];
  const int tid = threadIdx.x, lane = tid & 63, wave = tid >> 6;
  float w[3];
  if (box) {
    if (tid == 0) {
      for (int k = 0; k < 9; ++k) boxd[k] = box[k];
      const float ax = box[0], bx = box[3], by = box[4], cx = box[6], cy = box[7], cz = box[8];
      const float vol = fabsf(ax * by * cz);
      const float bcx = by * cz, bcy = -bx * cz, bcz = bx * cy - by * cx;
      w[0] = vol / sqrtf(bcx * bcx + bcy * bcy + bcz * bcz);
      w[1] = vol / (fabsf(ax) * sqrtf(cz * cz + cy * cy));
      w[2] = fabsf(cz);
    }
  } else {
    float mn[3] = {3.0e38f, 3.0e38f, 3.0e38f}, mx[3] = {-3.0e38f, -3.0e38f, -3.0e38f};
    for (int i = tid; i < N; i += 1024)
      for (int a = 0; a < 3; ++a) {
        const float v = pos[i * 3 + a];
        mn[a] = fminf(mn[a], v);
        mx[a] = fmaxf(mx[a], v);
      }
    for (int a = 0; a < 3; ++a) {
      for (int off = 32; off >= 1; off >>= 1) {
        mn[a] = fminf(mn[a], __shfl_xor(mn[a], off, 64));
        mx[a] = fmaxf(mx[a], __shfl_xor(mx[a], off, 64));
      }
      if (lane == 0) {
        red[a][wave] = mn[a];
        red[3 + a][wave] = mx[a];
      }
    }
    __syncthreads();
    if (tid == 0) {
      for (int k = 0; k < 9; ++k) boxd[k] = 0.f;
      for (int a = 0; a < 3; ++a) {
        float lo = red[a][0], hi = red[3 + a][0];
        for (int k = 1; k < 16; ++k) {
          lo = fminf(lo, red[a][k]);
          hi = fmaxf(hi, red[3 + a][k]);
        }
        const float ext = N > 0 ? hi - lo : 0.f;
        w[a] = fmaxf(ext + 1.01f * rc + 1e-3f * ext, 3.0f * rc);
        boxd[a * 4] = w[a];
      }
    }
// ... 40 lines not shown
```

torchmd-net_amd/csrc/tn_common.h:

```cpp
#pragma once
#include <hip/hip_runtime.h>
#include <stdint.h>

#define TN_WAVE 64

namespace tn {

struct M3 {
  float a[3][3];
};

__device__ __forceinline__ float pair_geometry(const float* __restrict__ pos, int hi, int lo, const float* __restrict__ box, float& dx,
                                               float& dy, float& dz) {
#pragma clang fp contract(off)
  dx = pos[hi * 3 + 0] - pos[lo * 3 + 0];
  dy = pos[hi * 3 + 1] - pos[lo * 3 + 1];
  dz = pos[hi * 3 + 2] - pos[lo * 3 + 2];
  if (box) {
    const float s3 = -roundf(dz / box[8]);
    dx = __builtin_fmaf(s3, box[6], dx);
    dy = __builtin_fmaf(s3, box[7], dy);
    dz = __builtin_fmaf(s3, box[8], dz);
    const float s2 = -roundf(dy / box[4]);
    dx = __builtin_fmaf(s2, box[3], dx);
// ... 102 lines not shown
__device__ __forceinline__ M3 add(const M3& x, const M3& y) {
  M3 r;
#pragma unroll
  for (int i = 0; i < 3; ++i)
#pragma unroll
    for (int j = 0; j < 3; ++j) r.a[i][j] = x.a[i][j] + y.a[i][j];
  return r;
}
__device__ __forceinline__ M3 scale(const M3& x, float s) {
  M3 r;
#pragma unroll
  for (int i = 0; i < 3; ++i)
#pragma unroll
    for (int j = 0; j < 3; ++j) r.a[i][j] = x.a[i][j] * s;
  return r;
}
__device__ __forceinline__ float frob2(const M3& x) {
  float s = 0.f;
#pragma unroll
  for (int i = 0; i < 3; ++i)
#pragma unroll
    for (int j = 0; j < 3; ++j) s += x.a[i][j] * x.a[i][j];
  return s;
}

__device__ __forceinline__ float kappa_of(const float* __restrict__ q, const int64_t* __restrict__ batch, int n) {
  return q ? (batch ? __builtin_fmaf(0.1f, q[batch[n]], 1.0f) : q[n]) : 1.0f;
}

__device__ __forceinline__ M3 xm_matmul(const M3& x, const M3& y) {
#pragma clang fp contract(off)
  M3 r;
#pragma unroll
  for (int i = 0; i < 3; ++i)
#pragma unroll
    for (int j = 0; j < 3; ++j)
      r.a[i][j] = __builtin_fmaf(x.a[i][2], y.a[2][j], __builtin_fmaf(x.a[i][1], y.a[1][j], x.a[i][0] * y.a[0][j]));
  return r;
}
__device__ __forceinline__ M3 xm_add_scaled(const M3& x, const M3& y, float s) {
#pragma clang fp contract(off)
  M3 r;
#pragma unroll
  for (int i = 0; i < 3; ++i)
#pragma unroll
    for (int j = 0; j < 3; ++j) r.a[i][j] = (x.a[i][j] + y.a[i][j]) * s;
  return r;
}
__device__ __forceinline__ M3 xm_scale(const M3& x, float s) {
#pragma clang fp contract(off)
  M3 r;
#pragma unroll
  for (int i = 0; i < 3; ++i)
#pragma unroll
    for (int j = 0; j < 3; ++j) r.a[i][j] = x.a[i][j] * s;
  return r;
}
__device__ __forceinline__ void group_product_adjoint(const float gc[9], const float y[9], const float m[9], float kap, int o3,
                                                      float gm[9], float gy[9]) {
#pragma clang fp contract(off)
  const M3 Y = compose(y), M = compose(m);
  const M3 Cm = o3 ? xm_add_scaled(xm_matmul(Y, M), xm_matmul(M, Y), kap) : xm_scale(xm_matmul(Y, M), 2.0f);
  const float tr3 = (Cm.a[0][0] + Cm.a[1][1] + Cm.a[2][2]) * (1.0f / 3.0f);
  const float uc[9] = {tr3,
                       0.5f * (Cm.a[2][1] - Cm.a[1][2]),
                       0.5f * (Cm.a[0][2] - Cm.a[2][0]),
                       0.5f * (Cm.a[1][0] - Cm.a[0][1]),
                       Cm.a[0][0] - tr3,
                       0.5f * (Cm.a[0][1] + Cm.a[1][0]),
                       0.5f * (Cm.a[0][2] + Cm.a[2][0]),
                       Cm.a[1][1] - tr3,
                       0.5f * (Cm.a[1][2] + Cm.a[2][1])};
  float f2 = 0.f;
#pragma unroll
  for (int i = 0; i < 3; ++i)
#pragma unroll
    for (int j = 0; j < 3; ++j) f2 = __builtin_fmaf(Cm.a[i][j], Cm.a[i][j], f2);
  const float inv = 1.0f / (f2 + 1.0f);
  float dot = 0.f, g[9];
#pragma unroll
  for (int c = 0; c < 9; ++c) {
    dot = __builtin_fmaf(gc[c], uc[c], dot);
    g[c] = gc[c] * inv;
  }
  const float g2 = 2.0f * (-dot * inv * inv);
  const float t = (g[0] - g[4] - g[7]) * (1.0f / 3.0f);
  M3 D;
  D.a[0][0] = t + g[4];
  D.a[0][1] = 0.5f * (g[5] - g[3]);
  D.a[0][2] = 0.5f * (g[6] + g[2]);
  D.a[1][0] = 0.5f * (g[5] + g[3]);
  D.a[1][1] = t + g[7];
  D.a[1][2] = 0.5f * (g[8] - g[1]);
  D.a[2][0] = 0.5f * (g[6] - g[2]);
  D.a[2][1] = 0.5f * (g[8] + g[1]);
  D.a[2][2] = t;
  M3 gCm;
#pragma unroll
  for (int i = 0; i < 3; ++i)
#pragma unroll
    for (int j = 0; j < 3; ++j) gCm.a[i][j] = __builtin_fmaf(Cm.a[i][j], g2, D.a[i][j]);
  const M3 Yt = transpose(Y), Mt = transpose(M);
  M3 gY, gM;
  if (o3) {
    gY = xm_add_scaled(xm_matmul(gCm, Mt), xm_matmul(Mt, gCm), kap);
    gM = xm_add_scaled(xm_matmul(Yt, gCm), xm_matmul(gCm, Yt), kap);
  } else {
    gY = xm_scale(xm_matmul(gCm, Mt), 2.0f);
    gM = xm_scale(xm_matmul(Yt, gCm), 2.0f);
  }
  compose_T(gM, gm);
  compose_T(gY, gy);
}

__device__ __forceinline__ int type_of(int c) { return c == 0 ? 0 : (c < 4 ? 1 : 2); }

__device__ __forceinline__ int xcd_chunk(int b, int n) {
  const int q = n >> 3, r = n & 7, x = b & 7, k = b >> 3;
  return (x < r ? x * (q + 1) : r * (q + 1) + (x - r) * q) + k;
}

__device__ __forceinline__ int xcd_chunk_act(int b, int n_act) {
  const int q = n_act >> 3, r = n_act & 7, x = b & 7, k = b >> 3;
  if (k >= q + (x < r ? 1 : 0)) return -1;
  return (x < r ? x * (q + 1) : r * (q + 1) + (x - r) * q) + k;
}

__device__ __forceinline__ float row_sum(float v, int n) {
  if (n >= 2) v = v + __int_as_float(__builtin_amdgcn_update_dpp(0, __float_as_int(v), 0xB1, 0xF, 0xF, true));
  if (n >= 4) v = v + __int_as_float(__builtin_amdgcn_update_dpp(0, __float_as_int(v), 0x4E, 0xF, 0xF, true));
  if (n >= 8) v = v + __int_as_float(__builtin_amdgcn_update_dpp(0, __float_as_int(v), 0x141, 0xF, 0xF, true));
  if (n >= 16) v = v + __int_as_float(__builtin_amdgcn_update_dpp(0, __float_as_int(v), 0x140, 0xF, 0xF, true));
  return v;
}
__device__ __forceinline__ float wave_sum(float v) {
  v = row_sum(v, 16);
  v += __shfl_xor(v, 16, 64);
  v += __shfl_xor(v, 32, 64);
  return v;
}

__device__ __forceinline__ float wave_sum4(float a, float b, float c, float d, int lane) {
  const bool hi = lane & 32;
  float k0 = hi ? c : a, k1 = hi ? d : b;
  const float s0 = hi ? a : c, s1 = hi ? b : d;
  k0 += __shfl_xor(s0, 32, 64);
  k1 += __shfl_xor(s1, 32, 64);
  const bool q = lane & 16;
  float v = q ? k1 : k0;
  v += __shfl_xor(q ? k0 : k1, 16, 64);
  return row_sum(v, 16);
}

__device__ __forceinline__ void cosine_cutoff(float d, float lo, float up, float& c, float& dc) {
  const float PI = 3.14159265358979323846f;
  if (lo > 0.f) {
    float k = 2.0f * PI / (up - lo);
    float arg = PI * (2.0f * (d - lo) / (up - lo) + 1.0f);
    bool in = (d < up) && (d > lo);
    c = in ? 0.5f * (cosf(arg) + 1.0f) : 0.f;
    dc = in ? -0.5f * sinf(arg) * k : 0.f;
  } else {
    float k = PI / up;
    bool in = d < up;
    c = in ? 0.5f * (cosf(d * k) + 1.0f) : 0.f;
    dc = in ? -0.5f * sinf(d * k) * k : 0.f;
  }
}

}
```

torchmd-net_amd/csrc/tn_edge_table.hip:

```cpp
#include <hip/hip_runtime.h>

#include <cstdlib>

#include "tn_common.h"
#include "tn_kernels.h"
#include "tn_interp.h"

namespace tn {

static inline int cdive(int64_t a, int64_t b) { return (int)((a + b - 1) / b); }

__device__ __forceinline__ double grid_d(int k, double lo, double h, int T, int mid) {
  if (mid) return lo + ((double)k + 0.5) * h;
  return k <= T ? lo + (double)k * h : 0.0;
}
__device__ __forceinline__ void cosine_cutoff_f64(double d, double lo, double up, double& c, double& dc) {
  const double PI = 3.14159265358979323846;
  if (lo > 0.0) {
    const double k = 2.0 * PI / (up - lo), arg = PI * (2.0 * (d - lo) / (up - lo) + 1.0);
    const bool in = (d < up) && (d > lo);
    c = in ? 0.5 * (cos(arg) + 1.0) : 0.0;
    dc = in ? -0.5 * sin(arg) * k : 0.0;
  } else {
    const double k = PI / up;
    const bool in = d < up;
    c = in ? 0.5 * (cos(d * k) + 1.0) : 0.0;
    dc = in ? -0.5 * sin(d * k) * k : 0.0;
  }
}
__global__ void k_radial_f64(int rows, double lo, double up, double h, int T, int mid, const float* __restrict__ means,
                             const float* __restrict__ betas, int K, double* __restrict__ dist, double* __restrict__ phi,
                             double* __restrict__ dphi, double* __restrict__ C, double* __restrict__ dC) {
  const int64_t idx = (int64_t)blockIdx.x * blockDim.x + threadIdx.x;
  if (idx >= (int64_t)rows * K) return;
  const int p = (int)(idx / K), k = (int)(idx - (int64_t)p * K);
  const double d = grid_d(p, lo, h, T, mid);
  double c0, dc0;
  cosine_cutoff_f64(d, 0.0, up, c0, dc0);
  const double alpha = 5.0 / (up - lo);
  const double u = exp(-alpha * (d - lo));
  const double mu = means[k], beta = betas[k];
  const double gk = exp(-beta * (u - mu) * (u - mu));
  phi[idx] = c0 * gk;
  dphi[idx] = dc0 * gk + c0 * gk * (-2.0 * beta * (u - mu)) * (-alpha * u);
  if (k == 0) {
    double c, dc;
    cosine_cutoff_f64(d, lo, up, c, dc);
    C[p] = c;
    dC[p] = dc;
    dist[p] = d;
  }
}
__global__ void k_dense_f64(const double* __restrict__ A, const double* __restrict__ A2, int lda, const float* __restrict__ W,
                            const float* __restrict__ bias, int M, int N, int K, int kind, const double* __restrict__ rs,
                            const double* __restrict__ rs2, double* __restrict__ C, double* __restrict__ C2, int ldc) {
  const int64_t idx = (int64_t)blockIdx.x * blockDim.x + threadIdx.x;
  if (idx >= (int64_t)M * N) return;
  const int m = (int)(idx / N), n = (int)(idx - (int64_t)m * N);
  const double* a = A + (int64_t)m * lda;
  const double* a2 = A2 + (int64_t)m * lda;
  const float* w = W + (int64_t)n * K;
  double e = bias ? (double)bias[n] : 0.0, r = 0.0;
  for (int k = 0; k < K; ++k) {
    const double wk = w[k];
    e += a[k] * wk;
    r += a2[k] * wk;
  }
  if (kind == 3) {
    const double e0 = e;
    e = e0 * rs[m];
    r = r * rs[m] + e0 * rs2[m];
  } else if (kind != 0) {
    const double sg = 1.0 / (1.0 + exp(-e));
    const double f = e * sg, df = sg * (1.0 + e * (1.0 - sg));
    if (kind == 1) {
      e = f;
      r = df * r;
    } else {
      e = f * rs[m];
      r = df * r * rs[m] + f * rs2[m];
    }
  }
  C[(int64_t)m * ldc + n] = e;
  C2[(int64_t)m * ldc + n] = r;
}
__global__ void k_table_pack(const double* __restrict__ f, const double* __restrict__ sl, int T, int R, double h, float* __restrict__ tab) {
  const int64_t idx = (int64_t)blockIdx.x * blockDim.x + threadIdx.x;
  if (idx >= (int64_t)(T + 2) * R) return;
  const int k = (int)(idx / R), c = (int)(idx - (int64_t)k * R);
  const double v = f[idx];
  float* row = tab + (int64_t)k * 3 * R + c;
  row[0] = (float)v;
  row[R] = (float)sl[idx];
  row[2 * R] = k < T ? (float)((f[idx + R] - v) / h) : 0.f;
}
void launch_radial_f64(int rows, double lo, double up, int T, bool mid, const float* means, const float* betas, int K, double* dist,
                       double* phi, double* dphi, double* C, double* dC, hipStream_t s) {
  hipLaunchKernelGGL(k_radial_f64, dim3(cdive((int64_t)rows * K, 256)), dim3(256), 0, s, rows, lo, up, (up - lo) / (double)T, T,
                     mid ? 1 : 0, means, betas, K, dist, phi, dphi, C, dC);
}
void launch_dense_f64(const double* A, const double* A2, int lda, const float* W, const float* bias, int M, int N, int K, int kind,
                      const double* rs, const double* rs2, double* C, double* C2, int ldc, hipStream_t s) {
  hipLaunchKernelGGL(k_dense_f64, dim3(cdive((int64_t)M * N, 256)), dim3(256), 0, s, A, A2, lda, W, bias, M, N, K, kind, rs, rs2, C, C2,
                     ldc);
}
void launch_table_pack(const double* f, const double* sl, int T, int R, double h, float* tab, hipStream_t s) {
  hipLaunchKernelGGL(k_table_pack, dim3(cdive((int64_t)(T + 2) * R, 256)), dim3(256), 0, s, f, sl, T, R, h, tab);
}

__device__ __forceinline__ int interval_of(float d, float lo, float inv_h, int T) {
  const int k = (int)((d - lo) * inv_h);
  return k < 0 ? 0 : (k > T - 1 ? T - 1 : k);
}
constexpr int BK_SLOTS = 2048, BK_THREADS = 1024;
struct BucketAgg {
  int key[BK_SLOTS], cnt[BK_SLOTS], base[BK_SLOTS];
};
__device__ __forceinline__ void bucket_agg_init(BucketAgg& A) {
  for (int i = threadIdx.x; i < BK_SLOTS; i += blockDim.x) {
    A.key[i] = -1;
    A.cnt[i] = 0;
  }
  __syncthreads();
}
__device__ __forceinline__ int bucket_agg_add(BucketAgg& A, int bucket) {
  const int sl = bucket & (BK_SLOTS - 1);
  const int prev = atomicCAS(&A.key[sl], -1, bucket);
  if (prev != -1 && prev != bucket) return -1;
  return atomicAdd(&A.cnt[sl], 1);
}

__global__ __launch_bounds__(BK_THREADS) void k_pair_cutoff_hist(Graph g, int Pcap, float lo, float up, float inv_h, int T,
                                                                float* __restrict__ C, float* __restrict__ dC, int* __restrict__ hist) {
  __shared__ BucketAgg A;
  bucket_agg_init(A);
  const int p = blockIdx.x * blockDim.x + threadIdx.x;
  const int P = g.counts[0];
  if (p <= Pcap && p <= P && !g.counts[2]) {
    const float d = p < P ? g.pd[p] : 0.f;
    float c, dc;
    cosine_cutoff(d, lo, up, c, dc);
    C[p] = c;
    dC[p] = dc;
    const int b = p < P ? interval_of(d, lo, inv_h, T) : T;
    if (bucket_agg_add(A, b) < 0) atomicAdd(hist + b, 1);
  }
  __syncthreads();
  for (int i = threadIdx.x; i < BK_SLOTS; i += blockDim.x)
    if (A.cnt[i] > 0) atomicAdd(hist + A.key[i], A.cnt[i]);
}
__global__ __launch_bounds__(1024) void k_bucket_scan(int* __restrict__ hist, int nb) {
  constexpr int PER = 8, TILE = 1024 * PER;
  __shared__ int wsum[16];
  __shared__ int carry;
  const int tid = threadIdx.x, lane = tid & 63, wave = tid >> 6;
  if (tid == 0) carry = 0;
  __syncthreads();
  for (int base = 0; base < nb; base += TILE) {
    int v[PER], sum = 0;
#pragma unroll
    for (int r = 0; r < PER; ++r) {
      const int i = base + tid * PER + r;
      v[r] = i < nb ? hist[i] : 0;
      sum += v[r];
    }
    int inc = sum;
#pragma unroll
    for (int off = 1; off < 64; off <<= 1) {
      const int t = __shfl_up(inc, off, 64);
      if (lane >= off) inc += t;
    }
    if (lane == 63) wsum[wave] = inc;
    __syncthreads();
    int pre = carry + inc - sum;
    for (int w = 0; w < wave; ++w) pre += wsum[w];
#pragma unroll
    for (int r = 0; r < PER; ++r) {
      const int i = base + tid * PER + r;
      if (i < nb) hist[i] = pre;
      pre += v[r];
    }
    __syncthreads();
    if (tid == 1023) carry = pre;
    __syncthreads();
  }
  if (tid == 0) hist[nb] = carry;
}
__global__ __launch_bounds__(BK_THREADS) void k_bucket_scatter(Graph g, int Pcap, float lo, float inv_h, int T, int* __restrict__ cursor,
                                                              unsigned* __restrict__ keys_s, int* __restrict__ vals_s) {
  __shared__ BucketAgg A;
  bucket_agg_init(A);
  const int p = blockIdx.x * blockDim.x + threadIdx.x;
  const int P = g.counts[0];
  const bool in_cap = p <= Pcap, valid = in_cap && p <= P && !g.counts[2];
  float d = 0.f;
  int b = 0, rank = -1, slot = -1;
  if (valid) {
    d = p < P ? g.pd[p] : 0.f;
    b = p < P ? interval_of(d, lo, inv_h, T) : T;
    rank = bucket_agg_add(A, b);
    if (rank < 0) slot = atomicAdd(cursor + b, 1);
  } else if (in_cap) {
    keys_s[p] = 0xFFFFFFFFu;
  }
  __syncthreads();
  for (int i = threadIdx.x; i < BK_SLOTS; i += blockDim.x)
    if (A.cnt[i] > 0) A.base[i] = atomicAdd(cursor + A.key[i], A.cnt[i]);
  __syncthreads();
  if (valid) {
    if (rank >= 0) slot = A.base[b & (BK_SLOTS - 1)] + rank;
    keys_s[slot] = __float_as_uint(d);
    vals_s[slot] = p;
  }
}

__global__ void k_fill_int(int* p, int v, int n) {
  const int i = blockIdx.x * blockDim.x + threadIdx.x;
  if (i < n) p[i] = v;
}

struct InterpArgs {
  const float* tab[8];
  float* out[8];
  float* dout[8];
  int ntab;
  int out_bf16;
};

__device__ __forceinline__ void store_piece(float* base, int64_t elem, float x, float y, float z, float w, int bf16) {
  if (bf16) {
    typedef __bf16 b2 __attribute__((ext_vector_type(2)));
    typedef float f2 __attribute__((ext_vector_type(2)));
    union { b2 v; uint32_t u; } lo, hi;
    lo.v = __builtin_convertvector((f2){x, y}, b2);
    hi.v = __builtin_convertvector((f2){z, w}, b2);
    if (bf16 == 2)
      *reinterpret_cast<float4*>(base + elem) = make_float4(__uint_as_float(lo.u << 16), __uint_as_float(lo.u & 0xFFFF0000u),
                                                            __uint_as_float(hi.u << 16), __uint_as_float(hi.u & 0xFFFF0000u));
    else
      *reinterpret_cast<uint2*>(reinterpret_cast<uint16_t*>(base) + elem) = make_uint2(lo.u, hi.u);
  } else {
    *reinterpret_cast<float4*>(base + elem) = make_float4(x, y, z, w);
  }
}

constexpr int EI_RUN = 8;
template <int NT>
__global__ __launch_bounds__(256) void k_edge_interp(Graph g, int Pcap, const unsigned* __restrict__ keys_sorted,
                                                    const int* __restrict__ vals_sorted, InterpArgs a, int R4, int T, float lo,
                                                    float h, float inv_h, int run) {
  typedef float f4 __attribute__((ext_vector_type(4)));
  const int groups = blockDim.x / R4;
  const int grp = threadIdx.x / R4, c4 = threadIdx.x - grp * R4;
  if (grp >= groups) return;
  const int R = 4 * R4;
  const int P = g.counts[0];
  const int s0 = (blockIdx.x * groups + grp) * run;
  int kcur = -1;
  f4 f0[NT], sl0[NT], D[NT], sl1[NT];
  for (int s = s0; s < s0 + run && s <= Pcap; ++s) {
    const unsigned key = keys_sorted[s];
    if (key == 0xFFFFFFFFu) break;
    const int p = vals_sorted[s];
    if (p == P) {
#pragma unroll
      for (int t = 0; t < NT; ++t) {
        const float* row = a.tab[t] + (int64_t)(T + 1) * 3 * R + 4 * c4;
        const f4 v0 = *reinterpret_cast<const f4*>(row);
        store_piece(a.out[t], (int64_t)p * R + 4 * c4, v0.x, v0.y, v0.z, v0.w, a.out_bf16);
        if (a.dout[t]) {
          const f4 v1 = *reinterpret_cast<const f4*>(row + R);
          store_piece(a.dout[t], (int64_t)p * R + 4 * c4, v1.x, v1.y, v1.z, v1.w, a.out_bf16);
        }
      }
      continue;
    }
    const float d = __uint_as_float(key);
    const InterpCoef ic = interp_coef(d, lo, h, inv_h, T);
    const int k = ic.k;
    if (k != kcur) {
      kcur = k;
#pragma unroll
      for (int t = 0; t < NT; ++t) {
        const float* row = a.tab[t] + (int64_t)k * 3 * R + 4 * c4;
        f0[t] = *reinterpret_cast<const f4*>(row);
        sl0[t] = *reinterpret_cast<const f4*>(row + R);
        D[t] = *reinterpret_cast<const f4*>(row + 2 * R);
        sl1[t] = *reinterpret_cast<const f4*>(row + 4 * R);
      }
    }
#pragma unroll
    for (int tb = 0; tb < NT; ++tb) {
      f4 v0, v1;
#pragma unroll
      for (int j = 0; j < 4; ++j) {
        v0[j] = interp_value(f0[tb][j], sl0[tb][j], D[tb][j], sl1[tb][j], ic);
        v1[j] = interp_slope(sl0[tb][j], D[tb][j], sl1[tb][j], ic);
      }
      store_piece(a.out[tb], (int64_t)p * R + 4 * c4, v0.x, v0.y, v0.z, v0.w, a.out_bf16);
      if (a.dout[tb]) store_piece(a.dout[tb], (int64_t)p * R + 4 * c4, v1.x, v1.y, v1.z, v1.w, a.out_bf16);
    }
  }
}

template <int NT>
__global__ __launch_bounds__(256) void k_edge_interp_direct(Graph g, int Pcap, InterpArgs a, int R4, int T, float lo, float up, float h,
                                                           float inv_h, float* __restrict__ C, float* __restrict__ dC) {
  typedef float f4 __attribute__((ext_vector_type(4)));
  const int groups = blockDim.x / R4;
  const int grp = threadIdx.x / R4, c4 = threadIdx.x - grp * R4;
  if (grp >= groups) return;
  const int p = blockIdx.x * groups + grp;
  if (p > Pcap) return;
  const int P = g.counts[0];
  if (p > P || g.counts[2]) return;
  const int R = 4 * R4;
  const float d = p < P ? g.pd[p] : 0.f;
  if (C && c4 == 0) {
    float c, dc;
    cosine_cutoff(d, lo, up, c, dc);
    C[p] = c;
    dC[p] = dc;
  }
  if (p == P) {
#pragma unroll
    for (int t = 0; t < NT; ++t) {
      const float* row = a.tab[t] + (int64_t)(T + 1) * 3 * R + 4 * c4;
      const f4 v0 = *reinterpret_cast<const f4*>(row);
      store_piece(a.out[t], (int64_t)p * R + 4 * c4, v0.x, v0.y, v0.z, v0.w, a.out_bf16);
      if (a.dout[t]) {
        const f4 v1 = *reinterpret_cast<const f4*>(row + R);
        store_piece(a.dout[t], (int64_t)p * R + 4 * c4, v1.x, v1.y, v1.z, v1.w, a.out_bf16);
      }
    }
    return;
  }
  const InterpCoef ic = interp_coef(d, lo, h, inv_h, T);
#pragma unroll
  for (int tb = 0; tb < NT; ++tb) {
    const float* row = a.tab[tb] + (int64_t)ic.k * 3 * R + 4 * c4;
    const f4 f0 = *reinterpret_cast<const f4*>(row), sl0 = *reinterpret_cast<const f4*>(row + R);
    const f4 D = *reinterpret_cast<const f4*>(row + 2 * R), sl1 = *reinterpret_cast<const f4*>(row + 4 * R);
    f4 v0, v1;
#pragma unroll
    for (int j = 0; j < 4; ++j) {
      v0[j] = interp_value(f0[j], sl0[j], D[j], sl1[j], ic);
      v1[j] = interp_slope(sl0[j], D[j], sl1[j], ic);
    }
    store_piece(a.out[tb], (int64_t)p * R + 4 * c4, v0.x, v0.y, v0.z, v0.w, a.out_bf16);
    if (a.dout[tb]) store_piece(a.dout[tb], (int64_t)p * R + 4 * c4, v1.x, v1.y, v1.z, v1.w, a.out_bf16);
  }
}

bool edge_interp_direct(int Pcap) {
  static const int lim = [] {
    const char* e = getenv("TMDNET_EDGE_DIRECT_MAX");
    return e ? atoi(e) : 16384;
  }();
  return Pcap + 1 <= lim;
}

void launch_pair_buckets(const Graph& g, int Pcap, float lo, float up, int T, float* C, float* dC, int* hist, unsigned* keys_s,
                         int* vals_s, hipStream_t s) {
  const int n = Pcap + 1;
  if (edge_interp_direct(Pcap)) return;
  const float h0 = (up - lo) / (float)T, inv_h0 = 1.0f / h0;
  hipLaunchKernelGGL(k_fill_int, dim3(cdive(T + 2, 256)), dim3(256), 0, s, hist, 0, T + 2);
  hipLaunchKernelGGL(k_pair_cutoff_hist, dim3(cdive(n, BK_THREADS)), dim3(BK_THREADS), 0, s, g, Pcap, lo, up, inv_h0, T, C, dC, hist);
  hipLaunchKernelGGL(k_bucket_scan, dim3(1), dim3(1024), 0, s, hist, T + 1);
  hipLaunchKernelGGL(k_bucket_scatter, dim3(cdive(n, BK_THREADS)), dim3(BK_THREADS), 0, s, g, Pcap, lo, inv_h0, T, hist, keys_s, vals_s);
}

void launch_edge_interp(const Graph& g, int Pcap, float lo, float up, int T, int R, int ntab, const float* const* tabs,
                        float* const* outs, float* const* douts, const unsigned* keys_s, const int* vals_s, hipStream_t s, float* C,
                        float* dC, int out_bf16) {
  const int n = Pcap + 1;
  InterpArgs a{};
  const float h = (up - lo) / (float)T;
  const int R4 = R / 4;
  const int groups = R4 >= 256 ? 1 : 256 / R4;
  const bool direct = edge_interp_direct(Pcap);
  static const int run_env = getenv("TMDNET_EI_RUN") ? atoi(getenv("TMDNET_EI_RUN")) : 0;
  const int run = run_env > 0 ? run_env : (n / 4096 < 4 ? 4 : (n / 4096 > EI_RUN ? EI_RUN : n / 4096));
  const dim3 grid(direct ? cdive(n, groups) : cdive(n, groups * run)), block(groups * R4);
#define EI_LAUNCH(NT)                                                                                                          \
  if (direct) {                                                                                                                \
    hipLaunchKernelGGL((k_edge_interp_direct<NT>), grid, block, 0, s, g, Pcap, a, R4, T, lo, up, h, 1.0f / h, C, dC);          \
    C = dC = nullptr;                                                                                         \
  } else                                                                                                                       \
    hipLaunchKernelGGL((k_edge_interp<NT>), grid, block, 0, s, g, Pcap, keys_s, vals_s, a, R4, T, lo, h, 1.0f / h, run)
  for (int t0 = 0; t0 < ntab; t0 += 4) {
    a = InterpArgs{};
    a.ntab = ntab - t0 < 4 ? ntab - t0 : 4;
    a.out_bf16 = out_bf16;
    for (int t = 0; t < a.ntab; ++t) {
      a.tab[t] = tabs[t0 + t];
      a.out[t] = outs[t0 + t];
      a.dout[t] = douts ? douts[t0 + t] : nullptr;
    }
    switch (a.ntab) {
      case 1: EI_LAUNCH(1); break;
      case 2: EI_LAUNCH(2); break;
      case 3: EI_LAUNCH(3); break;
      default: EI_LAUNCH(4); break;
    }
  }
#undef EI_LAUNCH
}

__global__ void k_interp_list(const float* __restrict__ tab, const double* __restrict__ dist, int M, int R, int T, float lo, float h,
                              float inv_h, float* __restrict__ out, float* __restrict__ dout) {
  const int64_t idx = (int64_t)blockIdx.x * blockDim.x + threadIdx.x;
  if (idx >= (int64_t)M * R) return;
  const int m = (int)(idx / R), c = (int)(idx - (int64_t)m * R);
  const InterpCoef ic = interp_coef((float)dist[m], lo, h, inv_h, T);
  const float* row = tab + (int64_t)ic.k * 3 * R + c;
  const float f0 = row[0], s0 = row[R], D = row[2 * R], s1 = row[4 * R];
  out[idx] = interp_value(f0, s0, D, s1, ic);
  dout[idx] = interp_slope(s0, D, s1, ic);
}
void launch_interp_list(const float* tab, const double* dist, int M, int R, int T, float lo, float up, float* out, float* dout,
                        hipStream_t s) {
  const float h = (up - lo) / (float)T;
  hipLaunchKernelGGL(k_interp_list, dim3(cdive((int64_t)M * R, 256)), dim3(256), 0, s, tab, dist, M, R, T, lo, h, 1.0f / h, out, dout);
}

}
```

torchmd-net_amd/csrc/tn_embed_rb.hip:

```cpp
#include <cstdlib>
#include <cstring>

#include "tn_common.h"
#include "tn_gemm_sb.h"
#include "tn_kernels.h"

namespace tn {

static inline int cdivr(int64_t a, int64_t b) { return (int)((a + b - 1) / b); }

__host__ __device__ __forceinline__ int64_t mom_off(int64_t R, int g, int k, int nksb) {
  return (R >> 5) * (10 * (int64_t)nksb * 512) + ((int64_t)(g * nksb + (k >> 4)) * 2 + ((k >> 3) & 1)) * 256 + (R & 31) * 8 + (k & 7);
}

__global__ __launch_bounds__(1024) void k_type_map(const int64_t* __restrict__ z_c, int N, int max_z, int* __restrict__ tix,
                                                  int* __restrict__ tz, int* __restrict__ counts) {
  __shared__ int flag[2048];
  const int tid = threadIdx.x;
  if (max_z > 2048) {
    if (tid == 0) counts[6] = 1 << 20;
    return;
  }
  for (int k = tid; k < max_z; k += 1024) flag[k] = 0;
  if (tid < 64) tz[tid] = 0;
  __syncthreads();
  for (int i = tid; i < N; i += 1024) flag[(int)z_c[i]] = 1;
  __syncthreads();
  if (tid == 0) {
    int nt = 0;
    for (int k = 0; k < max_z; ++k)
      if (flag[k]) {
        if (nt < 64) tz[nt] = k;
        flag[k] = nt + 1;
        ++nt;
      }
    counts[6] = nt;
  }
  __syncthreads();
  for (int i = tid; i < N; i += 1024) tix[i] = flag[(int)z_c[i]] - 1;
}
void launch_type_map(const Graph& g, int N, int max_z, hipStream_t s) {
  if (N <= 0) return;
  hipLaunchKernelGGL(k_type_map, dim3(1), dim3(1024), 0, s, g.z_c, N, max_z, g.tix, g.tz, g.counts);
}

__global__ void k_pair_scalars(Graph g, int Pcap, float lo, float up, float* __restrict__ ps) {
  const int p = blockIdx.x * blockDim.x + threadIdx.x;
  if (p > Pcap || g.counts[2]) return;
  const int P = g.counts[0];
  if (p > P) return;
  const float d = p < P ? g.pd[p] : 0.f;
  float c, dc, c0, dc0;
  cosine_cutoff(d, lo, up, c, dc);
  cosine_cutoff(d, 0.f, up, c0, dc0);
  const float alpha = 5.0f / (up - lo);
  *reinterpret_cast<float4*>(ps + (int64_t)p * 8) = make_float4(c, dc, c0, dc0);
  *reinterpret_cast<float4*>(ps + (int64_t)p * 8 + 4) = make_float4(expf(-alpha * (d - lo)), 0.f, 0.f, 0.f);
}
void launch_pair_scalars(const Graph& g, int Pcap, float lo, float up, float* ps, hipStream_t s) {
  hipLaunchKernelGGL(k_pair_scalars, dim3(cdivr(Pcap + 1, 256)), dim3(256), 0, s, g, Pcap, lo, up, ps);
}

__device__ __forceinline__ float rlane(float v, int l) { return __int_as_float(__builtin_amdgcn_readlane(__float_as_int(v), l)); }
template <int NTP, int KS>
__global__ __launch_bounds__(256) void k_embed_moments(Graph g, int N, RadialParams rp, const float* __restrict__ ps,
                                                       float* __restrict__ m) {
  const int i = __builtin_amdgcn_readfirstlane(blockIdx.x * 4 + (threadIdx.x >> 6));
  const int lane = threadIdx.x & 63, kk = lane & 31, half = lane >> 5;
  if (i >= N || g.counts[2]) return;
  const int K = rp.K;
  const int e0 = __builtin_amdgcn_readfirstlane(g.rowptr[i]), e1 = __builtin_amdgcn_readfirstlane(g.rowptr[i + 1]);
  const int P = __builtin_amdgcn_readfirstlane(g.counts[0]);
  float acc[KS][NTP][5], accb[NTP][5];
#pragma unroll
  for (int t = 0; t < NTP; ++t)
#pragma unroll
    for (int q = 0; q < 5; ++q) {
      accb[t][q] = 0.f;
#pragma unroll
      for (int s = 0; s < KS; ++s) acc[s][t][q] = 0.f;
    }
  float mu[KS], beta[KS];
#pragma unroll
  for (int s = 0; s < KS; ++s) {
    mu[s] = rp.means[kk + 32 * s];
    beta[s] = rp.betas[kk + 32 * s];
  }
  for (int base = e0; base < e1; base += 64) {
    const int n = e1 - base < 64 ? e1 - base : 64;
    int lt = 0;
    float lc = 0.f, lc0 = 0.f, lu = 0.f, lx = 0.f, ly = 0.f, lz = 0.f;
    if (lane < n) {
      const int e = base + lane;
      const int j = g.col[e], p = g.epair[e];
      const float sg = g.esign[e];
      lt = g.tix[j];
      const int pp = sg != 0.f ? p : P;
      const float4 a = *reinterpret_cast<const float4*>(ps + (int64_t)pp * 8);
      lc = a.x;
      lc0 = a.z;
      lu = ps[(int64_t)pp * 8 + 4];
      if (sg != 0.f) {
        lx = sg * g.prhat[p * 3];
        ly = sg * g.prhat[p * 3 + 1];
        lz = sg * g.prhat[p * 3 + 2];
      }
    }
    for (int q_ = 0; q_ < n; ++q_) {
      const int t = __builtin_amdgcn_readlane(lt, q_);
      const float c = rlane(lc, q_), c0 = rlane(lc0, q_), u = rlane(lu, q_);
      const float rx = rlane(lx, q_), ry = rlane(ly, q_), rz = rlane(lz, q_);
      float ge[5];
      if (half == 0) {
        ge[0] = 1.f; ge[1] = rx; ge[2] = ry; ge[3] = rz; ge[4] = rx * rx;
      } else {
        ge[0] = rx * ry; ge[1] = rx * rz; ge[2] = ry * ry; ge[3] = ry * rz; ge[4] = rz * rz;
      }
      const float cc0 = c * c0;
      float psi[KS];
#pragma unroll
      for (int s = 0; s < KS; ++s) psi[s] = cc0 * __expf(-beta[s] * (u - mu[s]) * (u - mu[s]));
#pragma unroll
      for (int tt = 0; tt < NTP; ++tt)
        if (tt == t) {
#pragma unroll
          for (int q = 0; q < 5; ++q) {
#pragma unroll
            for (int s = 0; s < KS; ++s) acc[s][tt][q] += psi[s] * ge[q];
            accb[tt][q] += c * ge[q];
          }
        }
    }
  }
  const int nksb = K / 16 + 1;
#pragma unroll
  for (int t = 0; t < NTP; ++t)
#pragma unroll
    for (int q = 0; q < 5; ++q) {
      const int64_t R = (int64_t)i * NTP + t;
      const int gq = half * 5 + q;
#pragma unroll
      for (int s = 0; s < KS; ++s) m[mom_off(R, gq, kk + 32 * s, nksb)] = acc[s][t][q];
      if (kk == 0) m[mom_off(R, gq, K, nksb)] = accb[t][q];
    }
}

struct Frag3 {
  bf16x8 p[3];
};
__device__ __forceinline__ Frag3 frag_split(const float4& a, const float4& b) {
  uint4 h, m, l;
  split8(a, b, h, m, l);
  Frag3 f;
  f.p[0] = *reinterpret_cast<bf16x8*>(&h);
  f.p[1] = *reinterpret_cast<bf16x8*>(&m);
  f.p[2] = *reinterpret_cast<bf16x8*>(&l);
  return f;
}
__device__ __forceinline__ void mma6(const Frag3& a, const Frag3& b, floatx16& acc) {
  acc = __builtin_amdgcn_mfma_f32_32x32x16_bf16(a.p[0], b.p[2], acc, 0, 0, 0);
  acc = __builtin_amdgcn_mfma_f32_32x32x16_bf16(a.p[2], b.p[0], acc, 0, 0, 0);
  acc = __builtin_amdgcn_mfma_f32_32x32x16_bf16(a.p[1], b.p[1], acc, 0, 0, 0);
  acc = __builtin_amdgcn_mfma_f32_32x32x16_bf16(a.p[0], b.p[1], acc, 0, 0, 0);
  acc = __builtin_amdgcn_mfma_f32_32x32x16_bf16(a.p[1], b.p[0], acc, 0, 0, 0);
  acc = __builtin_amdgcn_mfma_f32_32x32x16_bf16(a.p[0], b.p[0], acc, 0, 0, 0);
}
__device__ __forceinline__ Frag3 frag_load(const uint4* img) {
  Frag3 f;
#pragma unroll
  for (int p = 0; p < 3; ++p) {
    const uint4 v = img[p * 64];
    f.p[p] = *reinterpret_cast<const bf16x8*>(&v);
  }
  return f;
}
__device__ __forceinline__ int rb_type_of(int g) { return g == 0 ? 0 : (g < 4 ? 1 : 2); }

template <int NKS>
struct ARow {
  float4 x[NKS][2];
  float b;
};
template <int NKS>
__device__ __forceinline__ void arow_load(const float* __restrict__ base, bool val, int half, ARow<NKS>& a) {
  (void)val;
#pragma unroll
  for (int s = 0; s < NKS; ++s) {
    a.x[s][0] = *reinterpret_cast<const float4*>(base + 512 * s);
    a.x[s][1] = *reinterpret_cast<const float4*>(base + 512 * s + 4);
  }
  const float bv = base[512 * NKS - 256 * half];
  a.b = half == 0 ? bv : 0.f;
}
template <int NTP, int NKS>
__global__ __launch_bounds__(256) void k_embed_combine(int N, int F, const int64_t* __restrict__ z, const int* __restrict__ tz,
                                                       const float* __restrict__ Utab, const float* __restrict__ Vtab,
// ... 260 lines not shown
```

torchmd-net_amd/csrc/tn_graph_wave.hip:

```cpp
#include <cstdlib>

#include "tn_common.h"
#include "tn_kernels.h"

namespace tn {

static inline int cdivw(int64_t a, int64_t b) { return (int)((a + b - 1) / b); }

__device__ __forceinline__ float pair_d2(const float* __restrict__ pos, int hi, int lo, const float* __restrict__ box, float& dx,
                                         float& dy, float& dz) {
  return pair_geometry(pos, hi, lo, box, dx, dy, dz);
}

template <bool FILL>
__device__ __forceinline__ void nbr_wave_row(const Graph& g, const float* __restrict__ pos, const int64_t* __restrict__ batch,
                                             const float* __restrict__ box, int box_mode, int N, int B, float lo2, float up2, int loop,
                                             int i, int lane) {
  int64_t b = batch[i];
  int j0 = 0, j1 = N;
  if (b < 0 || b >= B) {
    b = 0;
    j1 = 0;
  } else if (!g.counts[3]) {
    j0 = g.mstart[b];
    j1 = g.mend[b];
  }
  const float* bx = box_mode == 0 ? nullptr : (box_mode == 1 ? box : box + b * 9);
  const int P = FILL ? g.counts[0] : 0;
  int e = FILL ? g.rowptr[i] : 0, p = FILL ? g.pairptr[i] : 0;
  int nl = 0, nt = 0;
  const unsigned long long lt = lane == 0 ? 0ull : (~0ull >> (64 - lane));
  for (int base = j0; base < j1; base += 64) {
    const int j = base + lane;
    bool hit = false, self = false;
    float dx = 0.f, dy = 0.f, dz = 0.f, d2 = 0.f;
    if (j < j1) {
      if (j == i) {
        hit = loop != 0;
        self = true;
      } else if (batch[j] == b) {
        d2 = (j < i) ? pair_d2(pos, i, j, bx, dx, dy, dz) : pair_d2(pos, j, i, bx, dx, dy, dz);
        hit = d2 < up2 && d2 >= lo2;
      }
    }
    const unsigned long long mall = __ballot(hit);
    const unsigned long long mlow = __ballot(hit && j < i);
    if (FILL) {
      if (hit) {
        const int ee = e + __popcll(mall & lt);
        g.col[ee] = j;
        if (self) {
          g.epair[ee] = P;
          g.esign[ee] = 0.f;
        } else if (j < i) {
          const int pp = p + __popcll(mlow & lt);
          const float d = sqrtf(d2);
          const float inv = d > 0.f ? 1.0f / d : 0.f;
          g.pair_i[pp] = i;
          g.pair_j[pp] = j;
          g.pd[pp] = d;
          g.pdelta[pp * 3 + 0] = dx; g.pdelta[pp * 3 + 1] = dy; g.pdelta[pp * 3 + 2] = dz;
          g.prhat[pp * 3 + 0] = dx * inv; g.prhat[pp * 3 + 1] = dy * inv; g.prhat[pp * 3 + 2] = dz * inv;
          g.epair[ee] = pp;
          g.esign[ee] = 1.f;
        } else {
          g.epair[ee] = -1;
          g.esign[ee] = -1.f;
        }
      }
      e += __popcll(mall);
      p += __popcll(mlow);
    } else {
      nt += __popcll(mall);
      nl += __popcll(mlow);
    }
  }
  if (!FILL && lane == 0) {
    g.nlow[i] = nl;
    g.ntot[i] = nt;
  }
  if (FILL && i == 0 && lane == 0) g.pd[P] = 0.f;
}

template <bool FILL>
__global__ __launch_bounds__(256) void k_nbr_wave(Graph g, const float* __restrict__ pos, const int64_t* __restrict__ batch,
                                                  const float* __restrict__ box, int box_mode, int N, int B, float lo2, float up2,
                                                  int loop) {
  const int i = blockIdx.x * 4 + (threadIdx.x >> 6);
  const int lane = threadIdx.x & 63;
  if (i >= N) return;
  if (FILL && g.counts[2]) return;
  nbr_wave_row<FILL>(g, pos, batch, box, box_mode, N, B, lo2, up2, loop, i, lane);
}

__device__ __forceinline__ void nbr_link_row(const Graph& g, int i, int lane) {
  const int e0 = g.rowptr[i], e1 = g.rowptr[i + 1];
  for (int e = e0 + lane; e < e1; e += 64) {
    const int j = g.col[e];
    if (j <= i) continue;
    int lo = g.rowptr[j], hi = lo + g.nlow[j] - 1;
    const int base = lo;
    while (lo < hi) {
      const int mid = (lo + hi) >> 1;
      if (g.col[mid] < i) lo = mid + 1; else hi = mid;
    }
    g.epair[e] = g.pairptr[j] + (lo - base);
  }
}
__global__ __launch_bounds__(256) void k_nbr_link_wave(Graph g, int N) {
  const int i = blockIdx.x * 4 + (threadIdx.x >> 6);
  const int lane = threadIdx.x & 63;
  if (i >= N || g.counts[2]) return;
  nbr_link_row(g, i, lane);
}

constexpr int GS_MAX_ATOMS = 256;
constexpr int GS_ECAP = 16384;
__global__ __launch_bounds__(1024) void k_graph_small(Graph g, const float* __restrict__ pos, const int64_t* __restrict__ batch,
                                                      const float* __restrict__ box, int box_mode, int N, int B, float lo2, float up2,
                                                      int loop, const int64_t* __restrict__ z, int max_z) {
  __shared__ int s_mstart[GS_MAX_ATOMS], s_mend[GS_MAX_ATOMS], s_nlow[GS_MAX_ATOMS], s_ntot[GS_MAX_ATOMS];
  __shared__ int s_rowptr[GS_MAX_ATOMS + 1], s_pairptr[GS_MAX_ATOMS + 1], s_counts[8], c_low[4], c_tot[4];
  __shared__ float s_pos[3 * GS_MAX_ATOMS];
  __shared__ int64_t s_batch[GS_MAX_ATOMS];
  __shared__ int s_col[GS_ECAP];
  const bool col_lds = g.ecap <= GS_ECAP;
  const int tid = threadIdx.x, lane = tid & 63, wave = tid >> 6;
  const bool mol_lds = B <= GS_MAX_ATOMS;
  Graph gl = g;
  gl.nlow = s_nlow;
  gl.ntot = s_ntot;
  gl.rowptr = s_rowptr;
  gl.pairptr = s_pairptr;
  gl.counts = s_counts;
  if (mol_lds) {
    gl.mstart = s_mstart;
    gl.mend = s_mend;
  }
  if (col_lds) gl.col = s_col;
  for (int k = tid; k < 3 * N; k += 1024) s_pos[k] = pos[k];
  if (tid < N) s_batch[tid] = batch[tid];
  for (int i = tid; i < B; i += 1024) gl.mstart[i] = gl.mend[i] = 0;
  if (tid < 8) s_counts[tid] = 0;
  __syncthreads();
  if (tid < N) {
    const int i = tid;
    const int64_t b = s_batch[i];
    if (b < 0 || b >= B) {
      s_counts[3] = 1;
      s_counts[5] = 1;
    } else {
      if (i > 0) {
        const int64_t bp = s_batch[i - 1];
        if (bp > b) s_counts[3] = 1;
        if (bp != b) gl.mstart[b] = i;
        else if ((i & 63) == 0) s_counts[7] = 1;
      } else {
        gl.mstart[b] = 0;
      }
      if (i == N - 1 || s_batch[i + 1] != b) gl.mend[b] = i + 1;
    }
    if (z) {
      int64_t v = z[i];
      if (v < 0 || v >= max_z) {
        s_counts[4] = 1;
        v = v < 0 ? 0 : max_z - 1;
      }
      g.z_c[i] = v;
    }
  }
  __syncthreads();
  for (int i = wave; i < N; i += 16) nbr_wave_row<false>(gl, s_pos, s_batch, box, box_mode, N, B, lo2, up2, loop, i, lane);
  __syncthreads();
  {
    int a = 0, b = 0;
    if (tid < GS_MAX_ATOMS) {
      a = tid < N ? s_nlow[tid] : 0;
      b = tid < N ? s_ntot[tid] : 0;
#pragma unroll
      for (int off = 1; off < 64; off <<= 1) {
        const int ta = __shfl_up(a, off, 64), tb = __shfl_up(b, off, 64);
        if (lane >= off) {
          a += ta;
          b += tb;
        }
      }
      if (lane == 63) {
        c_low[wave] = a;
        c_tot[wave] = b;
      }
    }
    __syncthreads();
    if (tid < GS_MAX_ATOMS) {
      for (int w = 0; w < wave; ++w) {
        a += c_low[w];
        b += c_tot[w];
      }
      if (tid < N) {
        s_pairptr[tid + 1] = a;
        s_rowptr[tid + 1] = b;
      }
      if (tid == 0) s_pairptr[0] = s_rowptr[0] = 0;
    }
    __syncthreads();
  }
  if (tid == 0) {
    const int P = s_pairptr[N], E = s_rowptr[N];
    s_counts[0] = P;
    s_counts[1] = E;
    s_counts[2] = (E > g.ecap || P > g.pcap || s_counts[5]) ? 1 : 0;
  }
  __syncthreads();
  if (!s_counts[2]) {
    for (int i = wave; i < N; i += 16) nbr_wave_row<true>(gl, s_pos, s_batch, box, box_mode, N, B, lo2, up2, loop, i, lane);
    __syncthreads();
    for (int i = wave; i < N; i += 16) nbr_link_row(gl, i, lane);
    if (col_lds) {
      __syncthreads();
      const int E = s_counts[1];
      for (int e = tid; e < E; e += 1024) g.col[e] = s_col[e];
    }
  }
  if (tid <= N) {
    g.rowptr[tid] = s_rowptr[tid];
    g.pairptr[tid] = s_pairptr[tid];
  }
  if (tid < N) {
    g.nlow[tid] = s_nlow[tid];
    g.ntot[tid] = s_ntot[tid];
  }
  if (mol_lds && tid < B) {
    g.mstart[tid] = s_mstart[tid];
    g.mend[tid] = s_mend[tid];
  }
  if (tid < 8) g.counts[tid] = s_counts[tid];
}
bool graph_small_ok(int N) {
  static const bool off = getenv("TMDNET_NO_GRAPH_SMALL") != nullptr;
  return !off && N > 0 && N <= GS_MAX_ATOMS;
}
void launch_graph_small(const Graph& g, const float* pos, const int64_t* batch, const float* box, int box_mode, int N, int B, float lo,
                        float up, bool loop, const int64_t* z, int max_z, hipStream_t s) {
  hipLaunchKernelGGL(k_graph_small, dim3(1), dim3(1024), 0, s, g, pos, batch, box, box_mode, N, B, lo * lo, up * up, (int)loop, z, max_z);
}

void launch_nbr_count_wave(const Graph& g, const float* pos, const int64_t* batch, const float* box, int box_mode, int N, int B,
                           float lo, float up, bool loop, hipStream_t s) {
  hipLaunchKernelGGL(k_nbr_wave<false>, dim3(cdivw(N, 4)), dim3(256), 0, s, g, pos, batch, box, box_mode, N, B, lo * lo, up * up,
                     (int)loop);
}
void launch_nbr_fill_link_wave(const Graph& g, const float* pos, const int64_t* batch, const float* box, int box_mode, int N, int B,
                               float lo, float up, bool loop, hipStream_t s) {
  hipLaunchKernelGGL(k_nbr_wave<true>, dim3(cdivw(N, 4)), dim3(256), 0, s, g, pos, batch, box, box_mode, N, B, lo * lo, up * up,
                     (int)loop);
  hipLaunchKernelGGL(k_nbr_link_wave, dim3(cdivw(N, 4)), dim3(256), 0, s, g, N);
}
void launch_nbr_link_wave(const Graph& g, int N, hipStream_t s) {
  hipLaunchKernelGGL(k_nbr_link_wave, dim3(cdivw(N, 4)), dim3(256), 0, s, g, N);
}

}
```

torchmd-net_amd/csrc/tn_kernels.h:

```cpp
#pragma once
#include <hip/hip_runtime.h>
#include <stdint.h>

namespace tn {

struct Graph {
  int* mstart;
  int* mend;
  int* nlow;
  int* ntot;
  int* rowptr;
  int* pairptr;
  int* col;
  int* epair;
  float* esign;
  int* pair_i;
  int* pair_j;
  float* pd;
  float* pdelta;
  float* prhat;
  int* counts;
  int* tix;
  int* tz;
  int64_t ecap, pcap;
  int* perm;
  int* iota;
  int* cell_key;
  int* cell_key_sorted;
  int* cell_start;
  float* pos_s;
  int64_t* z_s;
  float* boxd;
  int* cgrid;
  int* bat_s;
  int64_t* bat_c;
  int64_t* z_c;
  void* sort_tmp;
  size_t sort_tmp_bytes;
  int ncx, ncy, ncz;
  int use_cell;
  const float* ghost_w;
  int max_z;
  int small_mols;
};

struct RadialParams {
  const float* means;
  const float* betas;
  int K;
  float lo, up;
};

void launch_graph_build_phase1(const Graph& g, const float* pos, const int64_t* batch, const float* box, int box_mode, int N,
                               int B, float lo, float up, bool loop, hipStream_t s);
void launch_graph_build_phase2(const Graph& g, const float* pos, const int64_t* batch, const float* box, int box_mode, int N,
                               int B, float lo, float up, bool loop, hipStream_t s);
void launch_export_pairs(const Graph& g, int N, bool include_transpose, bool loop, int64_t max_pairs, const int* perm,
                         int64_t* neighbors, float* deltas, float* distances, int* num_pairs, hipStream_t s);

void launch_neighbor_grad(const int64_t* nb, const float* deltas, const float* dist, const float* g_delta, const float* g_dist,
                          int64_t M, int N, float* out, hipStream_t s);

void launch_radial(const Graph& g, int P, RadialParams rp, float* phi, float* dphi, float* C, float* dC, hipStream_t s);

void launch_ztables(const float* emb, const float* WaT, const float* WbT, const float* b2, int Z, int F, float* Utab, float* Vtab,
                    hipStream_t s);
void launch_embed_scatter(const Graph& g, int N, int F, const int64_t* z, const float* Utab, const float* Vtab, const float* Q,
                          const float* C, float* u0, float* s0n, hipStream_t s);
void launch_layernorm_fwd(const float* x, const float* w, const float* b, int rows, int R, float* y, float* xhat, float* rstd,
                          hipStream_t s);
void launch_layernorm_bwd(const float* g, const float* xhat, const float* rstd, const float* w, int rows, int R, float* gx,
                          hipStream_t s);
void launch_norm_x(const float* X, float* Xh, int N, int F, hipStream_t s);
struct PairRowTable;
enum MsgRoute {
  MSG_NONE = 0,
  MSG_FWD_ROW = 1,
  MSG_FWD_SPLIT = 2,
  MSG_FWD_TILE = 3,
  MSG_ADJ_ROW = 4,
  MSG_ADJ_SPLIT = 5,
  MSG_GD_ROW = 6,
  MSG_GD_SPLIT = 7,
  MSG_GD_TILE = 8,
  MSG_DUAL = 9,
  MSG_DUAL_ACC = 10,
  MSG_FWD_ROW_TABLE = 11,
  MSG_FWD_ROW_RANGE = 12,
  MSG_GD_ROW_TABLE = 13,
  MSG_GD_ROW_OWNED = 14,
  MSG_GD_ROW_TWO = 15,
  MSG_DUAL_SPLIT3 = 16,
};
MsgRoute message_route(const Graph& g, int N, int F, bool rows_from_table = false, int row0 = 0, int nrows = -1);
MsgRoute message_adjoint_route(int N, int F);
MsgRoute message_adjoint_gd_route(const Graph& g, int N, int F, bool rows_from_table = false, int own0 = 0, int own1 = -1,
                                  bool narrow = true);
MsgRoute message_dual_route(int N, int F, bool accumulate);
bool launch_message_as(MsgRoute r, const Graph& g, int N, int F, const float* w, const float* src, const float* q,
                       const int64_t* batch, int o3, float* Mi, float* Ch, hipStream_t s, const PairRowTable* rt = nullptr,
                       int row0 = 0, int nrows = -1, int balance = -1);
bool launch_message_adjoint_as(MsgRoute r, const Graph& g, int N, int F, const float* w, const float* gMi, float* gPn, hipStream_t s);
bool launch_message_adjoint_gd_as(MsgRoute r, const Graph& g, int N, int F, const float* w, const float* dw, const float* gMi,
                                  const float* Pn, float* gPn, float* slots, int64_t slot_stride, hipStream_t s,
                                  const PairRowTable* rt = nullptr, int own0 = 0, int own1 = -1, bool narrow = true);
bool launch_message_dual_as(MsgRoute r, const Graph& g, int N, int F, const float* w, const float* w_t, const float* src,
                            const float* src_t, float* out, float* out_t, hipStream_t s);
void launch_message_dual(const Graph& g, int N, int F, const float* w, const float* w_t, const float* src, const float* src_t,
                         float* out, float* out_t, bool accumulate, hipStream_t s);
void launch_message(const Graph& g, int N, int F, const float* w, const float* src, const float* q, const int64_t* batch, int o3,
                    float* Mi, float* Ch, hipStream_t s, const PairRowTable* rt = nullptr, int row0 = 0, int nrows = -1);
void launch_message_adjoint(const Graph& g, int N, int F, const float* w, const float* gMi, float* gPn, hipStream_t s);
bool message_adjoint_gd_ok(int N, int F);
int message_adjoint_gd_waves(const Graph& g, int N, int F, bool rows_from_table = false);
bool message_adjoint_pair_ok(const Graph& g, int N, int F);
struct NodeAdjointFold {
  const float* gCh;
  const float* Mi;
  const float* q;
  const int64_t* batch;
  int o3;
};
void launch_message_adjoint_pair(const Graph& g, int N, int F, const float* w, const float* dw, const float* gMi, const float* Pn,
                                 float* gPn, float* slots, int64_t slot_stride, hipStream_t s, const NodeAdjointFold* fold = nullptr);
void launch_message_adjoint_gd(const Graph& g, int N, int F, const float* w, const float* dw, const float* gMi, const float* Pn,
                               float* gPn, float* slots, int64_t slot_stride, hipStream_t s, const PairRowTable* rt = nullptr, int own0 = 0,
                               int own1 = -1, bool narrow = true,
                               const NodeAdjointFold* fold = nullptr);
void launch_layer_update(const float* Xh, const float* D, const float* q, const int64_t* batch, int N, int F, float* Xn, int next,
                         float* nxt, hipStream_t s);
void launch_readout_feat(const float* X, int N, int F, float* feat, hipStream_t s);
void launch_head_energy(const float* ao, const float* O2, const float* bO2, int N, int H, float std, const float* atomref,
                        const int64_t* z, float* ea, hipStream_t s, float* g_ao = nullptr,
                        const float* atom_w = nullptr, const int* perm = nullptr);
void launch_mol_sum(const Graph& g, const float* ea, const int64_t* batch, int N, int B, float mean, float* energy, hipStream_t s);

void launch_head_bwd(const float* ao, const float* O2, int N, int H, float std, float* g_ao, hipStream_t s);
void launch_readout_bwd(const float* X, const float* g_feat, int N, int F, float* G, hipStream_t s);
void launch_update_bwd(const float* G, const float* D, const float* q, const int64_t* batch, int N, int F, float* gD,
                       hipStream_t s);
void launch_message_bwd_node(const float* gCh, const float* Pn, const float* Mi, const float* q, const int64_t* batch, int o3, int N,
                             int F, float* gMi, float* gPn, hipStream_t s);
void launch_norm_bwd(const float* X, const float* gXh_lin, int N, int F, float* G, hipStream_t s);
void launch_norm_bwd_update_bwd(const float* X, const float* gXh_lin, int N, int F, float* G, const float* Dn, const float* q,
                                const int64_t* batch, float* gD, hipStream_t s);
void launch_norm_bwd_gate_bwd(const float* X, const float* gXh_lin, int N, int F, float* G, const float* UX, const float* gates,
                              const float* a2, float* gUX, float* g_a2, hipStream_t s);
void launch_lnbwd_readout_bwd(const float* g, const float* xhat, const float* rstd, const float* w, int N, int F, const float* X,
                              float* G, hipStream_t s);
void launch_head_mol_sum(const Graph& g, const float* ao, const float* O2, const float* bO2, int N, int B, int H, float std,
                         const float* atomref, const int64_t* z, const int64_t* batch, float mean, float* energy, hipStream_t s,
                         float* g_ao = nullptr, const float* atom_w = nullptr, const int* perm = nullptr);
void launch_embed_gate_bwd(const float* G, const float* UX, const float* gates, const float* a2, int N, int F, float* gUX, float* g_a2,
                           hipStream_t s);
void launch_owned_range(const float* aw, const int* perm, int N, int* out, hipStream_t s);
void launch_embed_bwd_atom(const float* g_u0_lin, const float* u0, const float* g_s0n, int N, int F, float* gA, hipStream_t s);
void launch_force_gather(const Graph& g, int N, const float* g_delta, const int* perm, float* forces, hipStream_t s,
                         const float* direct = nullptr);
void launch_fill(float* p, float v, int64_t n, hipStream_t s);
void launch_kappa(const float* q, const int64_t* batch, int N, int B, float* kap, hipStream_t s);

void launch_nbr_count_wave(const Graph& g, const float* pos, const int64_t* batch, const float* box, int box_mode, int N, int B,
                           float lo, float up, bool loop, hipStream_t s);
void launch_nbr_fill_link_wave(const Graph& g, const float* pos, const int64_t* batch, const float* box, int box_mode, int N, int B,
                               float lo, float up, bool loop, hipStream_t s);

void launch_nbr_link_wave(const Graph& g, int N, hipStream_t s);
bool graph_small_ok(int N);
void launch_graph_small(const Graph& g, const float* pos, const int64_t* batch, const float* box, int box_mode, int N, int B, float lo,
                        float up, bool loop, const int64_t* z, int max_z, hipStream_t s);
void launch_scan_counts(const Graph& g, int N, hipStream_t s);

size_t cell_sort_temp_bytes(int64_t n);
void launch_cell_phase1(const Graph& g, const float* pos, const int64_t* batch, const float* box, int N, float lo, float up, bool loop,
                        hipStream_t s, int B = 0);
void launch_cell_phase2(const Graph& g, int N, float lo, float up, bool loop, hipStream_t s);
void launch_permute_z(const Graph& g, const int64_t* z, int N, hipStream_t s);
void launch_prepare_z(const Graph& g, const int64_t* z, const int* perm, int N, int max_z, hipStream_t s);

void launch_pair_gd(const Graph& g, int Pcap, int F, const float* gMi, const float* Pn, const float* dw, float* gd, hipStream_t s);
void launch_embed_pair_gd(const Graph& g, int Pcap, int F, const int64_t* z, const float* Utab, const float* Vtab, const float* Q,
                          const float* dQ, const float* C, const float* dC, const float* gA, float* gd, float* g_rhat, hipStream_t s,
                          float* g_delta = nullptr, const float* slots = nullptr, int n_slots = 0, int64_t slot_stride = 0);
void launch_geom_gd(const Graph& g, int Pcap, const float* gd, const float* g_rhat, float* g_delta, hipStream_t s,
                    const float* slots = nullptr, int n_slots = 0, int64_t slot_stride = 0);

void launch_radial_f64(int rows, double lo, double up, int T, bool mid, const float* means, const float* betas, int K, double* dist,
                       double* phi, double* dphi, double* C, double* dC, hipStream_t s);
void launch_dense_f64(const double* A, const double* A2, int lda, const float* W, const float* bias, int M, int N, int K, int kind,
                      const double* rs, const double* rs2, double* C, double* C2, int ldc, hipStream_t s);
void launch_table_pack(const double* f, const double* sl, int T, int R, double h, float* tab, hipStream_t s);
void launch_pair_buckets(const Graph& g, int Pcap, float lo, float up, int T, float* C, float* dC, int* hist, unsigned* keys_s,
                         int* vals_s, hipStream_t s);
bool edge_interp_direct(int Pcap);
void launch_edge_interp(const Graph& g, int Pcap, float lo, float up, int T, int R, int ntab, const float* const* tabs,
                        float* const* outs, float* const* douts, const unsigned* keys_s, const int* vals_s, hipStream_t s, float* C,
                        float* dC, int out_bf16 = 0);
void launch_type_map(const Graph& g, int N, int max_z, hipStream_t s);
bool embed_rb_shape_ok(int F, int K);
int embed_rb_ntp(int nt);
int64_t embed_rb_moment_elems(int64_t N, int ntp, int K);
int64_t embed_rb_gmoment_elems(int64_t N, int ntp, int K);
size_t embed_rb_image_elems(int F, int K, bool reverse);
void launch_embed_rb_images(const float* Wdp_dev, const float* bdp_dev, int F, int K, uint16_t* fwd_dev, uint16_t* rev_dev, hipStream_t s);
void launch_pair_scalars(const Graph& g, int Pcap, float lo, float up, float* ps, hipStream_t s);
void launch_embed_moments(const Graph& g, int N, RadialParams rp, int ntp, const float* ps, float* m, hipStream_t s);
void launch_embed_combine(const Graph& g, int N, int F, int K, int ntp, const int64_t* z, const float* Utab, const float* Vtab,
                          const uint16_t* Bimg, const float* m, float* u0, float* s0n, hipStream_t s);
void launch_embed_gm(const Graph& g, int N, int F, int K, int ntp, const int64_t* z, const float* Utab, const float* Vtab,
                     const uint16_t* B2img, const float* bdp, const float* gA, float* gm, hipStream_t s);
void launch_embed_pair_rb(const Graph& g, int Pcap, int N, RadialParams rp, int ntp, const float* ps, const float* gm, float* gd,
                          float* g_rhat, hipStream_t s, float* g_delta, const float* slots, int n_slots, int64_t slot_stride);
void launch_interp_list(const float* tab, const double* dist, int M, int R, int T, float lo, float up, float* out, float* dout,
                        hipStream_t s);

bool message_pair_ok(int N, int F);
void launch_message_pair(const Graph& g, int N, int F, const float* w, const float* src, const float* q, const int64_t* batch,
                         int o3, float* Mi, float* Ch, hipStream_t s, int balance = -1);

bool gather_v4_ok(int F);

}
```

torchmd-net_amd/csrc/tn_kernels.hip:

```cpp
#include "tn_kernels.h"
#include "tn_interp.h"

#include <cstdlib>

#include "tn_common.h"

namespace tn {

static inline int fthreads(int F) {
  int t = ((F + 63) / 64) * 64;
  return t > 256 ? 256 : t;
}
static inline int cdiv(int64_t a, int64_t b) { return (int)((a + b - 1) / b); }

__global__ void k_mol_ranges(const int64_t* __restrict__ batch, int N, int B, int* mstart, int* mend, int* counts) {
  int i = blockIdx.x * blockDim.x + threadIdx.x;
  if (i >= N) return;
  int64_t b = batch[i];
  if (b < 0 || b >= B) {
    counts[3] = 1;
    counts[5] = 1;
    return;
  }
  if (i > 0) {
// ... 46 lines not shown
      if (j < i) ++nl;
    }
  }
  g.nlow[i] = nl;
  g.ntot[i] = nt;
}

__global__ __launch_bounds__(1024) void k_scan_counts(Graph g, int N) {
  constexpr int T = 8192, PER = 8;
  __shared__ int la[T], lb[T];
  __shared__ int wsum[2][16];
  __shared__ int carry[2];
  const int tid = threadIdx.x, lane = tid & 63, wave = tid >> 6;
  if (tid == 0) carry[0] = carry[1] = 0;
  for (int base = 0; base < N; base += T) {
#pragma unroll
    for (int r = 0; r < PER; ++r) {
      const int i = base + r * 1024 + tid;
      la[r * 1024 + tid] = i < N ? g.nlow[i] : 0;
      lb[r * 1024 + tid] = i < N ? g.ntot[i] : 0;
    }
    __syncthreads();
    int va[PER], vb[PER], a = 0, b = 0;
#pragma unroll
    for (int r = 0; r < PER; ++r) {
      va[r] = la[tid * PER + r];
      vb[r] = lb[tid * PER + r];
      a += va[r];
      b += vb[r];
    }
    int ia = a, ib = b;
#pragma unroll
    for (int off = 1; off < 64; off <<= 1) {
      int ta = __shfl_up(ia, off, 64), tb = __shfl_up(ib, off, 64);
      if (lane >= off) {
        ia += ta;
        ib += tb;
      }
    }
    if (lane == 63) {
      wsum[0][wave] = ia;
      wsum[1][wave] = ib;
    }
    __syncthreads();
    int oa = carry[0] + ia - a, ob = carry[1] + ib - b;
    for (int w = 0; w < wave; ++w) {
      oa += wsum[0][w];
      ob += wsum[1][w];
    }
#pragma unroll
    for (int r = 0; r < PER; ++r) {
      la[tid * PER + r] = oa;
      lb[tid * PER + r] = ob;
      oa += va[r];
      ob += vb[r];
    }
    __syncthreads();
    if (tid == 1023) {
      carry[0] = oa;
      carry[1] = ob;
    }
#pragma unroll
    for (int r = 0; r < PER; ++r) {
      const int i = base + r * 1024 + tid;
      if (i < N) {
        g.pairptr[i] = la[r * 1024 + tid];
        g.rowptr[i] = lb[r * 1024 + tid];
      }
    }
    __syncthreads();
  }
  if (tid == 0) {
    const int P = carry[0], E = carry[1];
    g.pairptr[N] = P;
    g.rowptr[N] = E;
    g.counts[0] = P;
    g.counts[1] = E;
    g.counts[2] = (E > g.ecap || P > g.pcap || g.counts[5]) ? 1 : 0;
  }
}

__global__ void k_nbr_fill(Graph g, const float* __restrict__ pos, const int64_t* __restrict__ batch, const float* __restrict__ box,
                           int box_mode, int N, float lo2, float up2, int loop) {
  int i = blockIdx.x * blockDim.x + threadIdx.x;
  if (i >= N) return;
  if (g.counts[2]) return;
  const int P = g.counts[0];
  int64_t b = batch[i];
  int j0, j1;
  cand_range(g.mstart, g.mend, g.counts, b, N, j0, j1);
  const float* bx = box_mode == 0 ? nullptr : (box_mode == 1 ? box : box + b * 9);
  int e = g.rowptr[i];
  int p = g.pairptr[i];
  for (int j = j0; j < j1; ++j) {
    if (j == i) {
      if (loop) {
        g.col[e] = i;
        g.epair[e] = P;
        g.esign[e] = 0.f;
        ++e;
      }
      continue;
    }
    if (batch[j] != b) continue;
    float dx, dy, dz;
    float d2 = (j < i) ? pair_delta(pos, i, j, bx, dx, dy, dz) : pair_delta(pos, j, i, bx, dx, dy, dz);
    if (d2 < up2 && d2 >= lo2) {
      g.col[e] = j;
      if (j < i) {
        float d = sqrtf(d2);
        float inv = d > 0.f ? 1.0f / d : 0.f;
        g.pair_i[p] = i;
        g.pair_j[p] = j;
        g.pd[p] = d;
        g.pdelta[p * 3 + 0] = dx;
        g.pdelta[p * 3 + 1] = dy;
        g.pdelta[p * 3 + 2] = dz;
        g.prhat[p * 3 + 0] = dx * inv;
        g.prhat[p * 3 + 1] = dy * inv;
        g.prhat[p * 3 + 2] = dz * inv;
        g.epair[e] = p;
        g.esign[e] = 1.f;
        ++p;
      } else {
        g.epair[e] = -1;
        g.esign[e] = -1.f;
      }
      ++e;
    }
  }
  if (i == 0) g.pd[P] = 0.f;
}

__global__ void k_nbr_link(Graph g, int N) {
  int i = blockIdx.x * blockDim.x + threadIdx.x;
  if (i >= N) return;
  if (g.counts[2]) return;
  int e0 = g.rowptr[i], e1 = g.rowptr[i + 1];
  for (int e = e0; e < e1; ++e) {
    int j = g.col[e];
    if (j <= i) continue;
    int lo = g.rowptr[j], hi = lo + g.nlow[j] - 1, base = lo;
    while (lo < hi) {
      int mid = (lo + hi) >> 1;
      if (g.col[mid] < i) lo = mid + 1; else hi = mid;
    }
    g.epair[e] = g.pairptr[j] + (lo - base);
  }
}

__global__ void k_graph_reset(Graph g, int B) {
  const int i = blockIdx.x * blockDim.x + threadIdx.x;
  if (i < B) g.mstart[i] = g.mend[i] = 0;
  if (i < 8) g.counts[i] = 0;
}

void launch_graph_build_phase1(const Graph& g, const float* pos, const int64_t* batch, const float* box, int box_mode, int N,
                               int B, float lo, float up, bool loop, hipStream_t s) {
  hipLaunchKernelGGL(k_graph_reset, dim3(cdiv(B > 8 ? B : 8, 256)), dim3(256), 0, s, g, B);
  if (N <= 0) return;
  hipLaunchKernelGGL(k_mol_ranges, dim3(cdiv(N, 256)), dim3(256), 0, s, batch, N, B, g.mstart, g.mend, g.counts);
  if (getenv("TMDNET_SCALAR_GRAPH"))
    hipLaunchKernelGGL(k_nbr_count, dim3(cdiv(N, 64)), dim3(64), 0, s, g, pos, batch, box, box_mode, N, lo * lo, up * up, (int)loop);
  else
    launch_nbr_count_wave(g, pos, batch, box, box_mode, N, B, lo, up, loop, s);
  hipLaunchKernelGGL(k_scan_counts, dim3(1), dim3(1024), 0, s, g, N);
}

void launch_scan_counts(const Graph& g, int N, hipStream_t s) {
  hipLaunchKernelGGL(k_scan_counts, dim3(1), dim3(1024), 0, s, g, N);
}

void launch_graph_build_phase2(const Graph& g, const float* pos, const int64_t* batch, const float* box, int box_mode, int N,
                               int B, float lo, float up, bool loop, hipStream_t s) {
  if (N <= 0) return;
  if (getenv("TMDNET_SCALAR_GRAPH")) {
    hipLaunchKernelGGL(k_nbr_fill, dim3(cdiv(N, 64)), dim3(64), 0, s, g, pos, batch, box, box_mode, N, lo * lo, up * up, (int)loop);
    hipLaunchKernelGGL(k_nbr_link, dim3(cdiv(N, 64)), dim3(64), 0, s, g, N);
  } else {
    launch_nbr_fill_link_wave(g, pos, batch, box, box_mode, N, B, lo, up, loop, s);
  }
}

__global__ void k_export_pairs(Graph g, int N, int include_transpose, int loop, int64_t max_pairs, const int* __restrict__ perm,
                               int64_t* neighbors, float* deltas, float* distances, int* num_pairs) {
  const int P = g.counts[0];
  const int64_t total = (int64_t)P * (include_transpose ? 2 : 1) + (loop ? N : 0);
  int64_t idx = (int64_t)blockIdx.x * blockDim.x + threadIdx.x;
  if (idx == 0) num_pairs[0] = (int)total;
  if (idx >= max_pairs) return;
  int64_t a = -1, b = -1;
  float dx = 0.f, dy = 0.f, dz = 0.f, d = 0.f;
  if (idx < total && !g.counts[2]) {
    int64_t k = idx;
    const bool tr = include_transpose && k >= P && k < 2 * (int64_t)P;
    if (k < P || tr) {
      if (tr) k -= P;
      a = g.pair_i[k]; b = g.pair_j[k];
      dx = g.pdelta[k * 3]; dy = g.pdelta[k * 3 + 1]; dz = g.pdelta[k * 3 + 2]; d = g.pd[k];
      if (perm) {
        a = perm[a]; b = perm[b];
      }
      if ((a < b) != tr) {
        const int64_t t = a; a = b; b = t;
        dx = -dx; dy = -dy; dz = -dz;
      }
    } else {
      a = b = k - (int64_t)P * (include_transpose ? 2 : 1);
    }
  }
  neighbors[idx] = a;
  neighbors[max_pairs + idx] = b;
  deltas[idx * 3] = dx; deltas[idx * 3 + 1] = dy; deltas[idx * 3 + 2] = dz;
  distances[idx] = d;
}

void launch_export_pairs(const Graph& g, int N, bool include_transpose, bool loop, int64_t max_pairs, const int* perm,
                         int64_t* neighbors, float* deltas, float* distances, int* num_pairs, hipStream_t s) {
  int64_t n = max_pairs > 0 ? max_pairs : 1;
  hipLaunchKernelGGL(k_export_pairs, dim3(cdiv(n, 256)), dim3(256), 0, s, g, N, (int)include_transpose, (int)loop, max_pairs, perm,
                     neighbors, deltas, distances, num_pairs);
}

__global__ void k_neighbor_grad(const int64_t* __restrict__ nb, const float* __restrict__ deltas, const float* __restrict__ dist,
                                const float* __restrict__ g_delta, const float* __restrict__ g_dist, int64_t M, int N,
                                float* __restrict__ out) {
  const int64_t p = (int64_t)blockIdx.x * blockDim.x + threadIdx.x;
  if (p >= M) return;
  const int64_t i = nb[p], j = nb[M + p];
  const float d = dist[p];
  if (i < 0 || j < 0 || i >= N || j >= N || d == 0.f) return;
  const float gd = g_dist ? g_dist[p] / d : 0.f;
#pragma unroll
  for (int a = 0; a < 3; ++a) {
    const float g = (g_delta ? g_delta[p * 3 + a] : 0.f) + deltas[p * 3 + a] * gd;
    atomicAdd(out + i * 3 + a, g);
    atomicAdd(out + j * 3 + a, -g);
  }
}
void launch_neighbor_grad(const int64_t* nb, const float* deltas, const float* dist, const float* g_delta, const float* g_dist,
                          int64_t M, int N, float* out, hipStream_t s) {
  launch_fill(out, 0.f, (int64_t)N * 3, s);
  if (M <= 0) return;
  hipLaunchKernelGGL(k_neighbor_grad, dim3(cdiv(M, 256)), dim3(256), 0, s, nb, deltas, dist, g_delta, g_dist, M, N, out);
}

__global__ void k_radial(Graph g, int Pcap, RadialParams rp, float* __restrict__ phi, float* __restrict__ dphi, float* __restrict__ C,
                         float* __restrict__ dC) {
  const int P = g.counts[0];
  if (g.counts[2]) return;
  int64_t idx = (int64_t)blockIdx.x * blockDim.x + threadIdx.x;
  int64_t total = (int64_t)(P + 1) * rp.K;
  if (idx >= total) return;
  int p = (int)(idx / rp.K), k = (int)(idx - (int64_t)p * rp.K);
  float d = p < P ? g.pd[p] : 0.f;
  float c0, dc0;
  cosine_cutoff(d, 0.f, rp.up, c0, dc0);
  float alpha = 5.0f / (rp.up - rp.lo);
  float u = expf(-alpha * (d - rp.lo));
  float mu = rp.means[k], beta = rp.betas[k];
  float gk = expf(-beta * (u - mu) * (u - mu));
  phi[idx] = c0 * gk;
  dphi[idx] = dc0 * gk + c0 * gk * (-2.0f * beta * (u - mu)) * (-alpha * u);
  if (k == 0) {
    float c, dc;
    cosine_cutoff(d, rp.lo, rp.up, c, dc);
    C[p] = c;
    dC[p] = dc;
  }
}
void launch_radial(const Graph& g, int P, RadialParams rp, float* phi, float* dphi, float* C, float* dC, hipStream_t s) {
  int64_t total = (int64_t)(P + 1) * rp.K;
  hipLaunchKernelGGL(k_radial, dim3(cdiv(total, 256)), dim3(256), 0, s, g, P, rp, phi, dphi, C, dC);
}

__global__ void k_ztables(const float* __restrict__ emb, const float* __restrict__ WaT, const float* __restrict__ WbT,
                          const float* __restrict__ b2, int Z, int F, float* __restrict__ Utab, float* __restrict__ Vtab) {
  const int z = blockIdx.x;
  for (int f = threadIdx.x; f < F; f += blockDim.x) {
    float u = b2[f], v = 0.f;
    for (int k = 0; k < F; ++k) {
      const float e = emb[(int64_t)z * F + k];
      u += e * WaT[(int64_t)k * F + f];
      v += e * WbT[(int64_t)k * F + f];
    }
    Utab[(int64_t)z * F + f] = u;
    Vtab[(int64_t)z * F + f] = v;
  }
}
void launch_ztables(const float* emb, const float* WaT, const float* WbT, const float* b2, int Z, int F, float* Utab, float* Vtab,
                    hipStream_t s) {
  hipLaunchKernelGGL(k_ztables, dim3(Z), dim3(fthreads(F)), 0, s, emb, WaT, WbT, b2, Z, F, Utab, Vtab);
}

static int embed_split_rows() {
  static const int v = [] {
    const char* e = getenv("TMDNET_SPLIT_ROWS");
    return e ? atoi(e) : 1024;
  }();
  return v;
}
__global__ void k_embed_scatter(Graph g, int N, int F, const int64_t* __restrict__ z, const float* __restrict__ Utab,
                                const float* __restrict__ Vtab, const float* __restrict__ Q, const float* __restrict__ C,
                                float* __restrict__ u0, float* __restrict__ s0n) {
  const int i = xcd_chunk(blockIdx.x, gridDim.x);
  if (g.counts[2]) return;
  const int e0 = g.rowptr[i], e1 = g.rowptr[i + 1];
  const int64_t zi = z[i];
  const int F3 = 3 * F;
  for (int f = threadIdx.x; f < F; f += blockDim.x) {
    const float Ui = Utab[zi * F + f];
    float I0 = 0.f, v0 = 0.f, v1 = 0.f, v2 = 0.f, t00 = 0.f, t01 = 0.f, t02 = 0.f, t11 = 0.f, t12 = 0.f, t22 = 0.f;
    struct In {
      float rx, ry, rz, c, v, q0, q1, q2;
    };
    auto load = [&](int e, In& o) {
      const int j = g.col[e], p = g.epair[e];
      const float sg = g.esign[e];
      const float h0 = g.prhat[p * 3], h1 = g.prhat[p * 3 + 1], h2 = g.prhat[p * 3 + 2];
// ... 1190 lines not shown
```

Measured before the change: 113,000 molecules/s.

## Fuse graph count scan, z prep, type map and bucket scan into fewer kernels

Replaces the single-block count scan with a per-block scan inside the neighbour-count kernel, followed by a multi-block prepare-atoms kernel. That kernel finalises row and pair pointers, clamps z, and builds the type map using a bitset plus a last-block ticket. The separate bucket-scan kernel is folded into the histogram kernel through a last-block ticket, and the histogram kernel now also writes pair scalars so the later pair_scalars launch can be skipped. The aim is to cut launch count and serial single-block work in graph build and the edge-table setup. In exchange it relies on atomic tickets and cross-block memory ordering, which adds correctness risk.

Measured after the change: 113,600 molecules/s, median of 6. About the same (+0.5%).

```diff
diff --git a/torchmd-net_amd/csrc/tn_api.hip b/torchmd-net_amd/csrc/tn_api.hip
--- a/torchmd-net_amd/csrc/tn_api.hip
+++ b/torchmd-net_amd/csrc/tn_api.hip
@@ -228,7 +228,9 @@
   Graph g{};
   const int64_t pcap = ecap / 2 + 1;
   g.small_mols = N <= 96 * (B > 0 ? B : 1) ? 1 : 0;
-  g.counts = c.take<int>(8);
+  g.counts = c.take<int>(GRAPH_ZERO_INTS);
+  g.tick = g.counts ? g.counts + 8 : nullptr;
+  g.zbits = g.counts ? g.counts + 16 : nullptr;
   g.mstart = c.take<int>(B);
   g.mend = c.take<int>(B);
   g.nlow = c.take<int>(N);
@@ -261,6 +263,8 @@
   g.tz = c.take<int>(64);
   g.sort_tmp_bytes = cell_sort_temp_bytes(N);
   g.sort_tmp = c.take<char>((int64_t)g.sort_tmp_bytes);
+  const int64_t nblk = (N + GRAPH_COUNT_ROWS - 1) / GRAPH_COUNT_ROWS;
+  g.btot = c.take<int>(2 * nblk);
   if (total) *total = c.off;
   return g;
 }
@@ -1195,17 +1199,17 @@
   CurScope cur_(m);
   {
     ProfScope ps_(s, CAT_GRAPH, 0.0, (double)n_atoms * 20);
+    const bool type_map = z && m->rb_fwd && n_atoms >= m->rb_min_atoms;
     if (cell) {
-      launch_fill(reinterpret_cast<float*>(g.counts), 0.f, 8, s);
+      launch_fill(reinterpret_cast<float*>(g.counts), 0.f, GRAPH_ZERO_INTS, s);
       launch_cell_phase1(g, pos, batch, box_mode == 1 ? box : nullptr, (int)n_atoms, m->hp.cutoff_lower, m->hp.cutoff_upper, true, s,
                          (int)n_mol);
       launch_scan_counts(g, (int)n_atoms, s);
+      if (z) launch_prepare_atoms(g, z, g.perm, (int)n_atoms, m->hp.max_z, false, type_map, s);
     } else {
       launch_graph_build_phase1(g, pos, batch, box, box_mode, (int)n_atoms, (int)n_mol, m->hp.cutoff_lower, m->hp.cutoff_upper,
-                                true, s);
-    }
-    if (z) launch_prepare_z(g, z, cell ? g.perm : nullptr, (int)n_atoms, m->hp.max_z, s);
-    if (z && m->rb_fwd && n_atoms >= m->rb_min_atoms) launch_type_map(g, (int)n_atoms, m->hp.max_z, s);
+                                true, s, z, m->hp.max_z, type_map);
+    }
   }
   int counts[8] = {0, 0, 0, 0, 0, 0, 0, 0};
   HIP_TRY(m, hipMemcpyAsync(counts, g.counts, sizeof(counts), hipMemcpyDeviceToHost, s));
@@ -1270,11 +1274,11 @@
                          m->hp.max_z, s);
     } else {
       launch_graph_build_phase1(g, pos, batch, box, box_mode, (int)n_atoms, (int)n_mol, m->hp.cutoff_lower, m->hp.cutoff_upper,
-                                true, s);
+                                true, s, z, m->hp.max_z);
       launch_graph_build_phase2(g, pos, batch, box, box_mode, (int)n_atoms, (int)n_mol, m->hp.cutoff_lower, m->hp.cutoff_upper, true,
                                 s);
     }
-    if (z && (cell || !graph_small_ok((int)n_atoms))) launch_prepare_z(g, z, cell ? g.perm : nullptr, (int)n_atoms, m->hp.max_z, s);
+    if (z && cell) launch_prepare_atoms(g, z, g.perm, (int)n_atoms, m->hp.max_z, false, false, s);
   }
   m->lastE = ecap;
   m->last_nt = 0;
@@ -1497,6 +1501,7 @@
   const bool chain_gb = chain_gate && (m->chain_mask & 4) && fm_image(W.L2T) && fm_image(W.L1T);
   m->chain_last = (chain_ro ? 1 : 0) | (chain_gf ? 2 : 0) | (chain_gb ? 4 : 0);
   m->msg_fold_last = 0;
+  bool ps_done = false;
   if (run_fwd) {
     if (use_tab) {
       const float* tabs[8];
@@ -1514,9 +1519,11 @@
         douts[nt_++] = want_forces ? b.dw[l] : nullptr;
       }
       const double rowB = 12.0 * Fd;
+      ps_done = ntp && nt_ > 0 && !edge_interp_direct(P);
       if (nt_ > 0)
         KR(CAT_EDGE_TABLE, (Pd + 1) * (rowB * nt_ * (want_forces ? 2 : 1) + 24) + (double)(m->tabs.T + 2) * 2 * rowB * nt_,
-           (launch_pair_buckets(g, P, hp.cutoff_lower, hp.cutoff_upper, m->tabs.T, b.C, b.dC, b.shist, b.skeys_s, b.svals_s, s),
+           (launch_pair_buckets(g, P, hp.cutoff_lower, hp.cutoff_upper, m->tabs.T, b.C, b.dC, b.shist, b.skeys_s, b.svals_s, s,
+                                ps_done ? b.ps : nullptr),
             launch_edge_interp(g, P, hp.cutoff_lower, hp.cutoff_upper, m->tabs.T, 3 * F, nt_, tabs, outs, douts, b.skeys_s, b.svals_s, s, b.C,
                                b.dC)));
     } else {
@@ -1587,7 +1594,8 @@
     } else {
     if (ntp) {
       KR(CAT_SCATTER, E_ * 12 + Pd * 48 + momB,
-         (launch_pair_scalars(g, P, hp.cutoff_lower, hp.cutoff_upper, b.ps, s), launch_embed_moments(g, N, rbp, ntp, b.ps, b.mom, s)));
+         ((ps_done ? (void)0 : launch_pair_scalars(g, P, hp.cutoff_lower, hp.cutoff_upper, b.ps, s)),
+          launch_embed_moments(g, N, rbp, ntp, b.ps, b.mom, s)));
       KR(CAT_SCATTER, momB + Nd * 10 * Fd * 4, launch_embed_combine(g, N, F, K, ntp, z, W.Utab, W.Vtab, m->rb_fwd, b.mom, b.u0, b.s0n, s));
     } else {
       KR(CAT_SCATTER, Pd * 12 * Fd + E_ * 12 + Nd * 10 * Fd * 4,
@@ -2181,7 +2189,8 @@
       {"pd", g.pd, (g.pcap + 1) * 4},       {"pdelta", g.pdelta, g.pcap * 12},    {"prhat", g.prhat, g.pcap * 12},
       {"perm", g.perm, N * 4},              {"z_c", g.z_c, N * 8},                {"bat_c", g.bat_c, N * 8},
       {"cgrid", g.cgrid, 4 * 4},            {"boxd", g.boxd, 12 * 4},             {"cell_key_sorted", g.cell_key_sorted, N * 4},
-      {"cell_start", g.cell_start, (8 * N + 2) * 4}};
+      {"cell_start", g.cell_start, (8 * N + 2) * 4},                              {"tix", g.tix, N * 4},
+      {"tz", g.tz, 64 * 4}};
   for (const auto& a : arrays) {
     if (std::strcmp(a.name, name)) continue;
     if (bytes != a.bytes) return fail(m, TMDNET_ERR_INVALID, "debug graph size mismatch: expected " + std::to_string(a.bytes) + " bytes");
diff --git a/torchmd-net_amd/csrc/tn_cell.hip b/torchmd-net_amd/csrc/tn_cell.hip
--- a/torchmd-net_amd/csrc/tn_cell.hip
+++ b/torchmd-net_amd/csrc/tn_cell.hip
@@ -120,21 +120,6 @@
 }
 void launch_permute_z(const Graph& g, const int64_t* z, int N, hipStream_t s) {
   hipLaunchKernelGGL(k_permute_z, dim3(cdivc(N, 256)), dim3(256), 0, s, z, g.perm, N, g.z_s);
-}
-__global__ void k_prepare_z(const int64_t* __restrict__ z, const int* __restrict__ perm, int N, int max_z, int64_t* __restrict__ z_c,
-                            int* __restrict__ counts) {
-  int i = blockIdx.x * blockDim.x + threadIdx.x;
-  if (i >= N) return;
-  int64_t v = z[perm ? perm[i] : i];
-  if (v < 0 || v >= max_z) {
-    counts[4] = 1;
-    v = v < 0 ? 0 : max_z - 1;
-  }
-  z_c[i] = v;
-}
-void launch_prepare_z(const Graph& g, const int64_t* z, const int* perm, int N, int max_z, hipStream_t s) {
-  if (N <= 0) return;
-  hipLaunchKernelGGL(k_prepare_z, dim3(cdivc(N, 256)), dim3(256), 0, s, z, perm, N, max_z, g.z_c, g.counts);
 }
 
 __device__ __forceinline__ float cell_d2(const float* __restrict__ pos, int hi, int lo, const float* __restrict__ box, float& dx,
diff --git a/torchmd-net_amd/csrc/tn_common.h b/torchmd-net_amd/csrc/tn_common.h
--- a/torchmd-net_amd/csrc/tn_common.h
+++ b/torchmd-net_amd/csrc/tn_common.h
@@ -278,6 +278,18 @@
   return row_sum(v, 16);
 }
 
+__device__ __forceinline__ bool last_block_ticket(int* ticket, int* s_flag) {
+  asm volatile("s_waitcnt vmcnt(0)" ::: "memory");
+  __syncthreads();
+  if (threadIdx.x == 0) *s_flag = atomicAdd(ticket, 1) == (int)gridDim.x - 1 ? 1 : 0;
+  __syncthreads();
+  return *s_flag != 0;
+}
+template <typename T>
+__device__ __forceinline__ T ticket_load(const T* p) {
+  return __hip_atomic_load(p, __ATOMIC_RELAXED, __HIP_MEMORY_SCOPE_AGENT);
+}
+
 __device__ __forceinline__ void cosine_cutoff(float d, float lo, float up, float& c, float& dc) {
   const float PI = 3.14159265358979323846f;
   if (lo > 0.f) {
diff --git a/torchmd-net_amd/csrc/tn_edge_table.hip b/torchmd-net_amd/csrc/tn_edge_table.hip
--- a/torchmd-net_amd/csrc/tn_edge_table.hip
+++ b/torchmd-net_amd/csrc/tn_edge_table.hip
@@ -130,9 +130,50 @@
   return atomicAdd(&A.cnt[sl], 1);
 }
 
+__device__ __forceinline__ void bucket_scan_block(int* hist, int nb) {
+  constexpr int PER = 8, TILE = 1024 * PER;
+  __shared__ int wsum[16];
+  __shared__ int carry;
+  const int tid = threadIdx.x, lane = tid & 63, wave = tid >> 6;
+  if (tid == 0) carry = 0;
+  __syncthreads();
+  for (int base = 0; base < nb; base += TILE) {
+    int v[PER], sum = 0;
+#pragma unroll
+    for (int r = 0; r < PER; ++r) {
+      const int i = base + tid * PER + r;
+      v[r] = i < nb ? ticket_load(hist + i) : 0;
+      sum += v[r];
+    }
+    int inc = sum;
+#pragma unroll
+    for (int off = 1; off < 64; off <<= 1) {
+      const int t = __shfl_up(inc, off, 64);
+      if (lane >= off) inc += t;
+    }
+    if (lane == 63) wsum[wave] = inc;
+    __syncthreads();
+    int pre = carry + inc - sum;
+    for (int w = 0; w < wave; ++w) pre += wsum[w];
+#pragma unroll
+    for (int r = 0; r < PER; ++r) {
+      const int i = base + tid * PER + r;
+      if (i < nb) hist[i] = pre;
+      pre += v[r];
+    }
+    __syncthreads();
+    if (tid == 1023) carry = pre;
+    __syncthreads();
+  }
+  if (tid == 0) hist[nb] = carry;
+}
+static_assert(BK_THREADS == 1024, "bucket_scan_block");
+
 __global__ __launch_bounds__(BK_THREADS) void k_pair_cutoff_hist(Graph g, int Pcap, float lo, float up, float inv_h, int T,
-                                                                float* __restrict__ C, float* __restrict__ dC, int* __restrict__ hist) {
+                                                                float* __restrict__ C, float* __restrict__ dC, int* hist,
+                                                                float* __restrict__ ps) {
   __shared__ BucketAgg A;
+  __shared__ int s_last;
   bucket_agg_init(A);
   const int p = blockIdx.x * blockDim.x + threadIdx.x;
   const int P = g.counts[0];
@@ -142,49 +183,20 @@
     cosine_cutoff(d, lo, up, c, dc);
     C[p] = c;
     dC[p] = dc;
+    if (ps) {
+      float c0, dc0;
+      cosine_cutoff(d, 0.f, up, c0, dc0);
+      const float alpha = 5.0f / (up - lo);
+      *reinterpret_cast<float4*>(ps + (int64_t)p * 8) = make_float4(c, dc, c0, dc0);
+      *reinterpret_cast<float4*>(ps + (int64_t)p * 8 + 4) = make_float4(expf(-alpha * (d - lo)), 0.f, 0.f, 0.f);
+    }
     const int b = p < P ? interval_of(d, lo, inv_h, T) : T;
     if (bucket_agg_add(A, b) < 0) atomicAdd(hist + b, 1);
   }
   __syncthreads();
   for (int i = threadIdx.x; i < BK_SLOTS; i += blockDim.x)
     if (A.cnt[i] > 0) atomicAdd(hist + A.key[i], A.cnt[i]);
-}
-__global__ __launch_bounds__(1024) void k_bucket_scan(int* __restrict__ hist, int nb) {
-  constexpr int PER = 8, TILE = 1024 * PER;
-  __shared__ int wsum[16];
-  __shared__ int carry;
-  const int tid = threadIdx.x, lane = tid & 63, wave = tid >> 6;
-  if (tid == 0) carry = 0;
-  __syncthreads();
-  for (int base = 0; base < nb; base += TILE) {
-    int v[PER], sum = 0;
-#pragma unroll
-    for (int r = 0; r < PER; ++r) {
-      const int i = base + tid * PER + r;
-      v[r] = i < nb ? hist[i] : 0;
-      sum += v[r];
-    }
-    int inc = sum;
-#pragma unroll
-    for (int off = 1; off < 64; off <<= 1) {
-      const int t = __shfl_up(inc, off, 64);
-      if (lane >= off) inc += t;
-    }
-    if (lane == 63) wsum[wave] = inc;
-    __syncthreads();
-    int pre = carry + inc - sum;
-    for (int w = 0; w < wave; ++w) pre += wsum[w];
-#pragma unroll
-    for (int r = 0; r < PER; ++r) {
-      const int i = base + tid * PER + r;
-      if (i < nb) hist[i] = pre;
-      pre += v[r];
-    }
-    __syncthreads();
-    if (tid == 1023) carry = pre;
-    __syncthreads();
-  }
-  if (tid == 0) hist[nb] = carry;
+  if (last_block_ticket(hist + T + 1, &s_last)) bucket_scan_block(hist, T + 1);
 }
 __global__ __launch_bounds__(BK_THREADS) void k_bucket_scatter(Graph g, int Pcap, float lo, float inv_h, int T, int* __restrict__ cursor,
                                                               unsigned* __restrict__ keys_s, int* __restrict__ vals_s) {
@@ -361,13 +373,12 @@
 }
 
 void launch_pair_buckets(const Graph& g, int Pcap, float lo, float up, int T, float* C, float* dC, int* hist, unsigned* keys_s,
-                         int* vals_s, hipStream_t s) {
+                         int* vals_s, hipStream_t s, float* ps) {
   const int n = Pcap + 1;
   if (edge_interp_direct(Pcap)) return;
   const float h0 = (up - lo) / (float)T, inv_h0 = 1.0f / h0;
   hipLaunchKernelGGL(k_fill_int, dim3(cdive(T + 2, 256)), dim3(256), 0, s, hist, 0, T + 2);
-  hipLaunchKernelGGL(k_pair_cutoff_hist, dim3(cdive(n, BK_THREADS)), dim3(BK_THREADS), 0, s, g, Pcap, lo, up, inv_h0, T, C, dC, hist);
-  hipLaunchKernelGGL(k_bucket_scan, dim3(1), dim3(1024), 0, s, hist, T + 1);
+  hipLaunchKernelGGL(k_pair_cutoff_hist, dim3(cdive(n, BK_THREADS)), dim3(BK_THREADS), 0, s, g, Pcap, lo, up, inv_h0, T, C, dC, hist, ps);
   hipLaunchKernelGGL(k_bucket_scatter, dim3(cdive(n, BK_THREADS)), dim3(BK_THREADS), 0, s, g, Pcap, lo, inv_h0, T, hist, keys_s, vals_s);
 }
 
diff --git a/torchmd-net_amd/csrc/tn_embed_rb.hip b/torchmd-net_amd/csrc/tn_embed_rb.hip
--- a/torchmd-net_amd/csrc/tn_embed_rb.hip
+++ b/torchmd-net_amd/csrc/tn_embed_rb.hip
@@ -11,37 +11,6 @@
 
 __host__ __device__ __forceinline__ int64_t mom_off(int64_t R, int g, int k, int nksb) {
   return (R >> 5) * (10 * (int64_t)nksb * 512) + ((int64_t)(g * nksb + (k >> 4)) * 2 + ((k >> 3) & 1)) * 256 + (R & 31) * 8 + (k & 7);
-}
-
-__global__ __launch_bounds__(1024) void k_type_map(const int64_t* __restrict__ z_c, int N, int max_z, int* __restrict__ tix,
-                                                  int* __restrict__ tz, int* __restrict__ counts) {
-  __shared__ int flag[2048];
-  const int tid = threadIdx.x;
-  if (max_z > 2048) {
-    if (tid == 0) counts[6] = 1 << 20;
-    return;
-  }
-  for (int k = tid; k < max_z; k += 1024) flag[k] = 0;
-  if (tid < 64) tz[tid] = 0;
-  __syncthreads();
-  for (int i = tid; i < N; i += 1024) flag[(int)z_c[i]] = 1;
-  __syncthreads();
-  if (tid == 0) {
-    int nt = 0;
-    for (int k = 0; k < max_z; ++k)
-      if (flag[k]) {
-        if (nt < 64) tz[nt] = k;
-        flag[k] = nt + 1;
-        ++nt;
-      }
-    counts[6] = nt;
-  }
-  __syncthreads();
-  for (int i = tid; i < N; i += 1024) tix[i] = flag[(int)z_c[i]] - 1;
-}
-void launch_type_map(const Graph& g, int N, int max_z, hipStream_t s) {
-  if (N <= 0) return;
-  hipLaunchKernelGGL(k_type_map, dim3(1), dim3(1024), 0, s, g.z_c, N, max_z, g.tix, g.tz, g.counts);
 }
 
 __global__ void k_pair_scalars(Graph g, int Pcap, float lo, float up, float* __restrict__ ps) {
diff --git a/torchmd-net_amd/csrc/tn_graph_wave.hip b/torchmd-net_amd/csrc/tn_graph_wave.hip
--- a/torchmd-net_amd/csrc/tn_graph_wave.hip
+++ b/torchmd-net_amd/csrc/tn_graph_wave.hip
@@ -15,7 +15,7 @@
 template <bool FILL>
 __device__ __forceinline__ void nbr_wave_row(const Graph& g, const float* __restrict__ pos, const int64_t* __restrict__ batch,
                                              const float* __restrict__ box, int box_mode, int N, int B, float lo2, float up2, int loop,
-                                             int i, int lane) {
+                                             int i, int lane, int* cnt_low = nullptr, int* cnt_tot = nullptr) {
   int64_t b = batch[i];
   int j0 = 0, j1 = N;
   if (b < 0 || b >= B) {
@@ -79,6 +79,10 @@
     g.nlow[i] = nl;
     g.ntot[i] = nt;
   }
+  if (!FILL && cnt_low) {
+    *cnt_low = nl;
+    *cnt_tot = nt;
+  }
   if (FILL && i == 0 && lane == 0) g.pd[P] = 0.f;
 }
 
@@ -91,6 +95,164 @@
   if (i >= N) return;
   if (FILL && g.counts[2]) return;
   nbr_wave_row<FILL>(g, pos, batch, box, box_mode, N, B, lo2, up2, loop, i, lane);
+}
+
+static_assert(GRAPH_COUNT_ROWS <= 64, "one wave scans a block's rows");
+__global__ __launch_bounds__(1024) void k_nbr_count_scan(Graph g, const float* __restrict__ pos, const int64_t* __restrict__ batch,
+                                                         const float* __restrict__ box, int box_mode, int N, int B, float lo2,
+                                                         float up2, int loop) {
+  __shared__ int s_nl[GRAPH_COUNT_ROWS], s_nt[GRAPH_COUNT_ROWS];
+  const int tid = threadIdx.x, lane = tid & 63, wave = tid >> 6;
+  const int r0 = blockIdx.x * GRAPH_COUNT_ROWS;
+  for (int r = wave; r < GRAPH_COUNT_ROWS; r += 16) {
+    const int i = r0 + r;
+    int nl = 0, nt = 0;
+    if (i < N) nbr_wave_row<false>(g, pos, batch, box, box_mode, N, B, lo2, up2, loop, i, lane, &nl, &nt);
+    if (lane == 0) {
+      s_nl[r] = nl;
+      s_nt[r] = nt;
+    }
+  }
+  __syncthreads();
+  if (wave == 0) {
+    const int va = lane < GRAPH_COUNT_ROWS ? s_nl[lane] : 0, vb = lane < GRAPH_COUNT_ROWS ? s_nt[lane] : 0;
+    int a = va, b = vb;
+#pragma unroll
+    for (int off = 1; off < 64; off <<= 1) {
+      const int ta = __shfl_up(a, off, 64), tb = __shfl_up(b, off, 64);
+      if (lane >= off) {
+        a += ta;
+        b += tb;
+      }
+    }
+    const int i = r0 + lane;
+    if (lane < GRAPH_COUNT_ROWS && i < N) {
+      g.pairptr[i] = a - va;
+      g.rowptr[i] = b - vb;
+    }
+    if (lane == 63) *reinterpret_cast<int2*>(g.btot + 2 * blockIdx.x) = make_int2(a, b);
+  }
+}
+
+constexpr int PA_THREADS = 1024, PA_CB = PA_THREADS / GRAPH_COUNT_ROWS;
+static_assert(PA_THREADS % GRAPH_COUNT_ROWS == 0 && PA_CB <= 64, "one wave scans a block's count blocks");
+__device__ __forceinline__ int64_t clamp_z(int64_t v, int max_z, bool& bad) {
+  bad = v < 0 || v >= max_z;
+  return bad ? (v < 0 ? 0 : max_z - 1) : v;
+}
+__global__ __launch_bounds__(PA_THREADS) void k_prepare_atoms(Graph g, const int64_t* __restrict__ z, const int* __restrict__ perm,
+                                                              int N, int max_z, int finalise, int type_map) {
+  __shared__ unsigned s_bits[64];
+  __shared__ int s_pre[64], s_last, s_red[2][16], s_base[2][PA_CB];
+  const int tid = threadIdx.x, lane = tid & 63, wave = tid >> 6, i = blockIdx.x * PA_THREADS + tid;
+  const bool tm = type_map && max_z <= 2048;
+  if (tm && tid < 64) s_bits[tid] = 0;
+  if (finalise) {
+    const int k0 = blockIdx.x * PA_CB, nblk = (N + GRAPH_COUNT_ROWS - 1) / GRAPH_COUNT_ROWS;
+    int a = 0, b = 0;
+    for (int j = tid; j < k0; j += PA_THREADS) {
+      const int2 t = *reinterpret_cast<const int2*>(g.btot + 2 * j);
+      a += t.x;
+      b += t.y;
+    }
+#pragma unroll
+    for (int off = 32; off > 0; off >>= 1) {
+      a += __shfl_down(a, off, 64);
+      b += __shfl_down(b, off, 64);
+    }
+    if (lane == 0) {
+      s_red[0][wave] = a;
+      s_red[1][wave] = b;
+    }
+    __syncthreads();
+    if (wave == 0) {
+      int fa = 0, fb = 0;
+#pragma unroll
+      for (int w = 0; w < 16; ++w) {
+        fa += s_red[0][w];
+        fb += s_red[1][w];
+      }
+      const int k = k0 + lane;
+      int2 v = make_int2(0, 0);
+      if (lane < PA_CB && k < nblk) v = *reinterpret_cast<const int2*>(g.btot + 2 * k);
+      int ia = v.x, ib = v.y;
+#pragma unroll
+      for (int off = 1; off < 64; off <<= 1) {
+        const int ta = __shfl_up(ia, off, 64), tb = __shfl_up(ib, off, 64);
+        if (lane >= off) {
+          ia += ta;
+          ib += tb;
+        }
+      }
+      if (lane < PA_CB) {
+        s_base[0][lane] = fa + ia - v.x;
+        s_base[1][lane] = fb + ib - v.y;
+      }
+      if (blockIdx.x == gridDim.x - 1 && lane == 63) {
+        const int P = fa + ia, E = fb + ib;
+        g.pairptr[N] = P;
+        g.rowptr[N] = E;
+        g.counts[0] = P;
+        g.counts[1] = E;
+        g.counts[2] = (E > g.ecap || P > g.pcap || g.counts[5]) ? 1 : 0;
+      }
+    }
+  }
+  if (tm || finalise) __syncthreads();
+  if (i < N) {
+    if (finalise) {
+      g.pairptr[i] += s_base[0][tid / GRAPH_COUNT_ROWS];
+      g.rowptr[i] += s_base[1][tid / GRAPH_COUNT_ROWS];
+    }
+    if (z) {
+      bool bad;
+      const int64_t v = clamp_z(z[perm ? perm[i] : i], max_z, bad);
+      if (bad) g.counts[4] = 1;
+      g.z_c[i] = v;
+      if (tm) atomicOr(s_bits + ((int)v >> 5), 1u << ((int)v & 31));
+    }
+  }
+  if (!type_map) return;
+  if (!tm) {
+    if (i == 0) g.counts[6] = 1 << 20;
+    return;
+  }
+  __syncthreads();
+  if (tid < 64 && s_bits[tid]) atomicOr(reinterpret_cast<unsigned*>(g.zbits) + tid, s_bits[tid]);
+  if (!last_block_ticket(g.tick + 1, &s_last)) return;
+  if (tid < 64) {
+    const unsigned w = (unsigned)ticket_load(g.zbits + tid);
+    const int c = __popc(w);
+    int inc = c;
+#pragma unroll
+    for (int off = 1; off < 64; off <<= 1) {
+      const int t = __shfl_up(inc, off, 64);
+      if (tid >= off) inc += t;
+    }
+    s_bits[tid] = w;
+    s_pre[tid] = inc - c;
+    g.tz[tid] = 0;
+    if (tid == 63) g.counts[6] = inc;
+  }
+  __syncthreads();
+  for (int k = tid; k < max_z; k += PA_THREADS) {
+    const unsigned w = s_bits[k >> 5];
+    if (w & (1u << (k & 31))) {
+      const int t = s_pre[k >> 5] + __popc(w & ((1u << (k & 31)) - 1u));
+      if (t < 64) g.tz[t] = k;
+    }
+  }
+  for (int j = tid; j < N; j += PA_THREADS) {
+    bool bad;
+    const int v = (int)clamp_z(z[perm ? perm[j] : j], max_z, bad);
+    g.tix[j] = s_pre[v >> 5] + __popc(s_bits[v >> 5] & ((1u << (v & 31)) - 1u));
+  }
+}
+void launch_prepare_atoms(const Graph& g, const int64_t* z, const int* perm, int N, int max_z, bool finalise, bool type_map,
+                          hipStream_t s) {
+  if (N <= 0 || (!z && !finalise)) return;
+  hipLaunchKernelGGL(k_prepare_atoms, dim3(cdivw(N, PA_THREADS)), dim3(PA_THREADS), 0, s, g, z, perm, N, max_z, (int)finalise,
+                     (int)(type_map && z != nullptr));
 }
 
 __device__ __forceinline__ void nbr_link_row(const Graph& g, int i, int lane) {
@@ -246,8 +408,8 @@
 
 void launch_nbr_count_wave(const Graph& g, const float* pos, const int64_t* batch, const float* box, int box_mode, int N, int B,
                            float lo, float up, bool loop, hipStream_t s) {
-  hipLaunchKernelGGL(k_nbr_wave<false>, dim3(cdivw(N, 4)), dim3(256), 0, s, g, pos, batch, box, box_mode, N, B, lo * lo, up * up,
-                     (int)loop);
+  hipLaunchKernelGGL(k_nbr_count_scan, dim3(cdivw(N, GRAPH_COUNT_ROWS)), dim3(1024), 0, s, g, pos, batch, box, box_mode, N, B, lo * lo,
+                     up * up, (int)loop);
 }
 void launch_nbr_fill_link_wave(const Graph& g, const float* pos, const int64_t* batch, const float* box, int box_mode, int N, int B,
                                float lo, float up, bool loop, hipStream_t s) {
diff --git a/torchmd-net_amd/csrc/tn_kernels.h b/torchmd-net_amd/csrc/tn_kernels.h
--- a/torchmd-net_amd/csrc/tn_kernels.h
+++ b/torchmd-net_amd/csrc/tn_kernels.h
@@ -22,6 +22,9 @@
   int* counts;
   int* tix;
   int* tz;
+  int* tick;
+  int* zbits;
+  int* btot;
   int64_t ecap, pcap;
   int* perm;
   int* iota;
@@ -51,8 +54,11 @@
   float lo, up;
 };
 
+constexpr int GRAPH_COUNT_ROWS = 32;
+constexpr int GRAPH_ZERO_INTS = 80;
 void launch_graph_build_phase1(const Graph& g, const float* pos, const int64_t* batch, const float* box, int box_mode, int N,
-                               int B, float lo, float up, bool loop, hipStream_t s);
+                               int B, float lo, float up, bool loop, hipStream_t s, const int64_t* z = nullptr, int max_z = 0,
+                               bool type_map = false);
 void launch_graph_build_phase2(const Graph& g, const float* pos, const int64_t* batch, const float* box, int box_mode, int N,
                                int B, float lo, float up, bool loop, hipStream_t s);
 void launch_export_pairs(const Graph& g, int N, bool include_transpose, bool loop, int64_t max_pairs, const int* perm,
@@ -170,13 +176,14 @@
 void launch_graph_small(const Graph& g, const float* pos, const int64_t* batch, const float* box, int box_mode, int N, int B, float lo,
                         float up, bool loop, const int64_t* z, int max_z, hipStream_t s);
 void launch_scan_counts(const Graph& g, int N, hipStream_t s);
+void launch_prepare_atoms(const Graph& g, const int64_t* z, const int* perm, int N, int max_z, bool finalise, bool type_map,
+                          hipStream_t s);
 
 size_t cell_sort_temp_bytes(int64_t n);
 void launch_cell_phase1(const Graph& g, const float* pos, const int64_t* batch, const float* box, int N, float lo, float up, bool loop,
                         hipStream_t s, int B = 0);
 void launch_cell_phase2(const Graph& g, int N, float lo, float up, bool loop, hipStream_t s);
 void launch_permute_z(const Graph& g, const int64_t* z, int N, hipStream_t s);
-void launch_prepare_z(const Graph& g, const int64_t* z, const int* perm, int N, int max_z, hipStream_t s);
 
 void launch_pair_gd(const Graph& g, int Pcap, int F, const float* gMi, const float* Pn, const float* dw, float* gd, hipStream_t s);
 void launch_embed_pair_gd(const Graph& g, int Pcap, int F, const int64_t* z, const float* Utab, const float* Vtab, const float* Q,
@@ -191,12 +198,11 @@
                       const double* rs, const double* rs2, double* C, double* C2, int ldc, hipStream_t s);
 void launch_table_pack(const double* f, const double* sl, int T, int R, double h, float* tab, hipStream_t s);
 void launch_pair_buckets(const Graph& g, int Pcap, float lo, float up, int T, float* C, float* dC, int* hist, unsigned* keys_s,
-                         int* vals_s, hipStream_t s);
+                         int* vals_s, hipStream_t s, float* ps = nullptr);
 bool edge_interp_direct(int Pcap);
 void launch_edge_interp(const Graph& g, int Pcap, float lo, float up, int T, int R, int ntab, const float* const* tabs,
                         float* const* outs, float* const* douts, const unsigned* keys_s, const int* vals_s, hipStream_t s, float* C,
                         float* dC, int out_bf16 = 0);
-void launch_type_map(const Graph& g, int N, int max_z, hipStream_t s);
 bool embed_rb_shape_ok(int F, int K);
 int embed_rb_ntp(int nt);
 int64_t embed_rb_moment_elems(int64_t N, int ntp, int K);
diff --git a/torchmd-net_amd/csrc/tn_kernels.hip b/torchmd-net_amd/csrc/tn_kernels.hip
--- a/torchmd-net_amd/csrc/tn_kernels.hip
+++ b/torchmd-net_amd/csrc/tn_kernels.hip
@@ -222,19 +222,22 @@
 __global__ void k_graph_reset(Graph g, int B) {
   const int i = blockIdx.x * blockDim.x + threadIdx.x;
   if (i < B) g.mstart[i] = g.mend[i] = 0;
-  if (i < 8) g.counts[i] = 0;
+  if (i < GRAPH_ZERO_INTS) g.counts[i] = 0;
 }
 
 void launch_graph_build_phase1(const Graph& g, const float* pos, const int64_t* batch, const float* box, int box_mode, int N,
-                               int B, float lo, float up, bool loop, hipStream_t s) {
-  hipLaunchKernelGGL(k_graph_reset, dim3(cdiv(B > 8 ? B : 8, 256)), dim3(256), 0, s, g, B);
+                               int B, float lo, float up, bool loop, hipStream_t s, const int64_t* z, int max_z, bool type_map) {
+  hipLaunchKernelGGL(k_graph_reset, dim3(cdiv(B > GRAPH_ZERO_INTS ? B : GRAPH_ZERO_INTS, 256)), dim3(256), 0, s, g, B);
   if (N <= 0) return;
   hipLaunchKernelGGL(k_mol_ranges, dim3(cdiv(N, 256)), dim3(256), 0, s, batch, N, B, g.mstart, g.mend, g.counts);
-  if (getenv("TMDNET_SCALAR_GRAPH"))
+  if (getenv("TMDNET_SCALAR_GRAPH")) {
     hipLaunchKernelGGL(k_nbr_count, dim3(cdiv(N, 64)), dim3(64), 0, s, g, pos, batch, box, box_mode, N, lo * lo, up * up, (int)loop);
-  else
+    hipLaunchKernelGGL(k_scan_counts, dim3(1), dim3(1024), 0, s, g, N);
+    if (z) launch_prepare_atoms(g, z, nullptr, N, max_z, false, type_map, s);
+  } else {
     launch_nbr_count_wave(g, pos, batch, box, box_mode, N, B, lo, up, loop, s);
-  hipLaunchKernelGGL(k_scan_counts, dim3(1), dim3(1024), 0, s, g, N);
+    launch_prepare_atoms(g, z, nullptr, N, max_z, true, type_map, s);
+  }
 }
 
 void launch_scan_counts(const Graph& g, int N, hipStream_t s) {
```
